# aleCombi/Hedgehog.jl

Measured on AMD Instinct MI355X. Metric: MC path-steps/sec (Heston Euler-Maruyama, 1e6 paths x 252 steps per GPU), higher is better.
Workload: dtype f64

## Files before the change

hedgehog.jl_amd/_ffi.py:

```python
from __future__ import annotations

import ctypes as C
import os

HH_MAX_PARTIALS = 8
HH_LSM_PHASE_POW, HH_LSM_PHASE_INIT, HH_LSM_PHASE_STEP = 1, 2, 3
HH_TILE_PATHS = 256
HH_ACC_LEN = 16
HH_MAX_MODELS = 16
HH_ACC_SUM, HH_ACC_SUMSQ, HH_ACC_DSUM, HH_ACC_NPATHS = 0, 1, 2, 10

HH_LOGNORMAL, HH_HESTON = 0, 1
HH_EULER_MARUYAMA, HH_EXACT_LAW, HH_BROADIE_KAYA = 0, 1, 2
HH_NOISE_GENERATE, HH_NOISE_REPLAY = 0, 1
HH_REPLAY_TILE_MAJOR, HH_REPLAY_PATH_MAJOR = 0, 1
HH_PATH_SPOT, HH_PATH_LOG = 0, 1
HH_PAYOFF_VANILLA, HH_PAYOFF_ASIAN_ARITH, HH_PAYOFF_ASIAN_GEOM = 0, 1, 2
HH_PAYOFF_BARRIER, HH_PAYOFF_DIGITAL_CASH, HH_PAYOFF_DIGITAL_ASSET = 3, 4, 5
HH_BARRIER_UP_OUT, HH_BARRIER_UP_IN, HH_BARRIER_DOWN_OUT, HH_BARRIER_DOWN_IN = 0, 1, 2, 3
HH_STAT_SUM_S, HH_STAT_SUM_X, HH_STAT_MAX_S, HH_STAT_MIN_S, HH_STAT_S_T = 0, 1, 2, 3, 4
HH_PAYOFF_LOOKBACK_FLOAT, HH_PAYOFF_LOOKBACK_FIXED = 6, 7
HH_STAT_CMAX_S, HH_STAT_CMIN_S = 5, 6
HH_EXTREMES_MONITORED, HH_EXTREMES_BRIDGE = 0, 1
HH_PATH_STATS = 5
HH_PATH_STATS_BRIDGE = 7
HH_MAX_PATH_PAYOFFS = 1024
HH_JUMP_MAX_MEAN = 64.0
HH_JUMP_MAX_COUNT = 255

HH_OK, HH_ERR_INVALID, HH_ERR_UNSUPPORTED, HH_ERR_HIP, HH_ERR_NOMEM, HH_ERR_RCCL, HH_ERR_DEVICE_TIMEOUT = 0, -1, -2, -3, -4, -5, -6
HH_MGPU_AUTO, HH_MGPU_HOST_SUM, HH_MGPU_RCCL = 0, 1, 2
HH_MGPU_REDUCE_HOST, HH_MGPU_REDUCE_RCCL = 0, 1
HH_MGPU_OPT_ENQUEUE = 1
HH_MGPU_ENQUEUE_SERIAL, HH_MGPU_ENQUEUE_THREADS = 0, 1

_dp = C.POINTER(C.c_double)


class hh_model(C.Structure):
    _fields_ = [(n, C.c_double) for n in
                ("S0", "V0", "kappa", "theta", "sigma", "rho", "r_drift", "discount", "T", "strike",
                 "cp")] + \
               [(n, _dp) for n in
                ("dS0", "dV0", "dkappa", "dtheta", "dsigma", "dr_drift", "ddiscount", "dstrike")]


class hh_config(C.Structure):
    _fields_ = [
        ("dynamics", C.c_int32), ("strategy", C.c_int32), ("antithetic", C.c_int32),
        ("em_split", C.c_int32), ("compat_sqrt_alpha", C.c_int32), ("noise_mode", C.c_int32),
        ("replay_layout", C.c_int32), ("seeds_on_device", C.c_int32),
        ("replay_on_device", C.c_int32), ("terminal_on_device", C.c_int32),
        ("n_steps", C.c_uint32), ("n_partials", C.c_uint32),
        ("n_paths", C.c_uint64), ("path_offset", C.c_uint64),
        ("seeds", C.c_void_p), ("replay", C.c_void_p),
        ("bk_n_sigma", C.c_double), ("bk_cf_tol", C.c_double), ("bk_atol", C.c_double),
        ("bk_moment_h", C.c_double),
        ("bk_newton_maxiter", C.c_int32), ("bk_bisect_maxiter", C.c_int32),
        ("bk_root_form", C.c_int32), ("bk_bracket_form", C.c_int32), ("bk_caps", C.c_int32), ("reserved0", C.c_int32),
        ("seeds_len", C.c_uint64), ("replay_len", C.c_uint64),
    ]


class hh_result(C.Structure):
    _fields_ = [
        ("price", C.c_double), ("std_error", C.c_double),
        ("sum_payoff", C.c_double), ("sumsq_payoff", C.c_double),
        ("dprice", C.c_double * HH_MAX_PARTIALS),
        ("n_paths_done", C.c_uint64),
        ("bk_newton_fail", C.c_uint64), ("bk_bisect_fallback", C.c_uint64),
        ("bk_maxguess_fallback", C.c_uint64), ("bk_cf_terms", C.c_uint64),
        ("kernel_ms", C.c_double), ("total_ms", C.c_double),
    ]


class hh_lsm_result(C.Structure):
    _fields_ = [("price", C.c_double), ("std_error", C.c_double), ("n_paths_total", C.c_uint64),
                ("rows_regressed", C.c_uint32), ("rows_skipped", C.c_uint32),
                ("kernel_ms", C.c_double), ("total_ms", C.c_double),
                ("form", C.c_int32), ("persistent_fallbacks", C.c_int32)]


class hh_path_payoff(C.Structure):
    _fields_ = [("kind", C.c_int32), ("barrier_type", C.c_int32), ("strike", C.c_double), ("cp", C.c_double),
                ("barrier", C.c_double), ("rebate", C.c_double), ("cash", C.c_double)]


class hh_jump(C.Structure):
    _fields_ = [("lambda_", C.c_double), ("mu_j", C.c_double), ("sigma_j", C.c_double)]


HH_BK_ROOT_SECANT, HH_BK_ROOT_ORDER2 = 0, 1
HH_BK_BRACKET_MIDPOINT, HH_BK_BRACKET_ROOTS = 0, 1
HH_BK_CAPS_AS_WRITTEN, HH_BK_CAPS_ROOTS_DEFAULT = 0, 1
HH_OPT_LSM_FORM = 1
HH_OPT_BK_TERM_CACHE = 2
HH_OPT_GRID_FORM = 3
HH_OPT_LSM_SPIN_TICKS = 4
HH_OPT_FUSE_REDUCE = 5
HH_OPT_GRID_ORDER = 6
HH_OPT_FINISH_SPIN_TICKS = 7
HH_OPT_FINISH_TILE_FIRST = 8
HH_GRID_FORM_PER_DATE, HH_GRID_FORM_BATCHED = 0, 1
HH_CM_GRAD_LEN = 8
HH_LSM_FORM_PER_DATE, HH_LSM_FORM_PERSISTENT, HH_LSM_FORM_AUTO = 0, 1, 2
HH_CRR_MAX_STEPS, HH_CRR_FORM_A_MAX_STEPS = 32768, 2047
HH_CRR_EUROPEAN, HH_CRR_AMERICAN_FORWARD, HH_CRR_AMERICAN_SPOT = 0, 1, 2
HH_FD_MAX_SPACE, HH_FD_MAX_TIME, HH_FD_FORM_A_MAX_SPACE = 4096, 65536, 1024
HH_FD_EUROPEAN, HH_FD_AMERICAN = 0, 1


class HedgehogMCError(RuntimeError):
    def __init__(self, code: int, msg: str):
        super().__init__(f"hedgehog_mc error {code}: {msg}")
        self.code = code


LIB_PATH = os.environ.get("HEDGEHOG_MC_LIB") or os.path.join(
    os.path.dirname(os.path.abspath(__file__)), "lib", "libhedgehog_mc.so")

_vp = C.c_void_p
SYMBOLS = [
    ("hh_abi_version", C.c_int, []),
    ("hh_ctx_create", C.c_int, [C.POINTER(_vp), C.c_int]),
    ("hh_ctx_destroy", None, [_vp]),
    ("hh_ctx_set_stream", C.c_int, [_vp, _vp]),
    ("hh_ctx_reset_stream", C.c_int, [_vp]),
    ("hh_last_error", C.c_char_p, [_vp]),
    ("hh_ctx_set_option", C.c_int, [_vp, C.c_int32, C.c_int64]),
    ("hh_ctx_check_last", C.c_int, [_vp]),
    ("hh_mc_solve", C.c_int, [_vp, C.POINTER(hh_model), C.POINTER(hh_config), C.POINTER(hh_result), _vp]),
    ("hh_mc_accumulate", C.c_int, [_vp, C.POINTER(hh_model), C.POINTER(hh_config), _vp, _vp]),
    ("hh_mc_solve_multi", C.c_int, [_vp, C.POINTER(hh_model), C.c_uint32, C.POINTER(hh_config), C.POINTER(hh_result), _vp]),
    ("hh_mc_accumulate_multi", C.c_int, [_vp, C.POINTER(hh_model), C.c_uint32, C.POINTER(hh_config), _vp, _vp]),
    ("hh_mc_finalize", C.c_int, [C.POINTER(hh_model), C.POINTER(hh_config), _vp, C.POINTER(hh_result)]),
    ("hh_mc_accumulate_basket", C.c_int, [_vp, C.POINTER(hh_model), C.POINTER(hh_config), _vp, _vp, C.c_uint32, _vp, _vp]),
    ("hh_mc_solve_basket", C.c_int, [_vp, C.POINTER(hh_model), C.POINTER(hh_config), _vp, _vp, C.c_uint32, _vp, _vp]),
    ("hh_carr_madan", C.c_int, [_vp, C.POINTER(hh_model), C.c_int32, C.c_int32, C.c_double, C.c_double, C.POINTER(C.c_double)]),
    ("hh_carr_madan_basket", C.c_int, [_vp, C.POINTER(hh_model), C.c_int32, C.c_int32, C.c_double, C.c_double,
                                       _vp, _vp, _vp, _vp, _vp, C.c_uint32, _vp]),
    ("hh_carr_madan_basket_grad", C.c_int, [_vp, C.POINTER(hh_model), C.c_int32, C.c_int32, C.c_double,
                                            C.c_double, _vp, _vp, _vp, _vp, _vp, C.c_uint32, _vp, _vp]),
    ("hh_crr_solve", C.c_int, [_vp, C.c_int32, C.c_uint32, _vp, _vp, _vp, _vp, _vp, _vp, _vp, C.c_uint32, _vp, _vp]),
    ("hh_fd_solve", C.c_int, [_vp, C.c_int32, C.c_int32, C.c_int32, C.c_uint32, _vp, _vp, _vp, _vp, _vp, _vp, _vp, _vp, _vp, _vp, _vp]),
    ("hh_lsm_grid_elems", C.c_size_t, [C.c_uint64, C.c_uint32, C.c_int32]),
    ("hh_lsm_solve", C.c_int, [_vp, C.POINTER(hh_model), C.POINTER(hh_config), C.c_int32, C.c_double, C.POINTER(hh_lsm_result), _vp, _vp, _vp]),
    ("hh_lsm_solve_grid", C.c_int, [_vp, C.POINTER(hh_model), _vp, C.c_uint64, C.c_uint32, C.c_int32, C.c_double, C.POINTER(hh_lsm_result), _vp, _vp]),
    ("hh_heston_exact_grid", C.c_int, [_vp, C.POINTER(hh_model), C.POINTER(hh_config), _vp, _vp, C.c_int32, C.POINTER(hh_result)]),
    ("hh_euler_grid", C.c_int, [_vp, C.POINTER(hh_model), C.POINTER(hh_config), C.c_int32, _vp, _vp, C.c_int32, C.POINTER(hh_result)]),
    ("hh_lsm_solve_euler", C.c_int, [_vp, C.POINTER(hh_model), C.POINTER(hh_config), C.c_int32, C.c_int32, C.c_double,
                                     C.POINTER(hh_lsm_result), _vp, _vp, _vp]),
    ("hh_mc_path_stats", C.c_int, [_vp, C.POINTER(hh_model), C.POINTER(hh_config), C.c_uint32, C.c_int32, _vp, C.c_int32,
                                   C.POINTER(hh_result)]),
    ("hh_mc_solve_path", C.c_int, [_vp, C.POINTER(hh_model), C.POINTER(hh_config), C.c_uint32, C.c_int32,
                                   C.POINTER(hh_path_payoff), C.c_uint32, C.POINTER(hh_result), _vp, _vp]),
    ("hh_mc_path_stats_ex", C.c_int, [_vp, C.POINTER(hh_model), C.POINTER(hh_config), C.c_uint32, C.c_int32, C.c_int32, _vp,
                                      C.c_int32, C.POINTER(hh_result)]),
    ("hh_mc_solve_path_ex", C.c_int, [_vp, C.POINTER(hh_model), C.POINTER(hh_config), C.c_uint32, C.c_int32, C.c_int32,
                                      C.POINTER(hh_path_payoff), C.c_uint32, C.POINTER(hh_result), _vp, _vp]),
    ("hh_mc_solve_jump", C.c_int, [_vp, C.POINTER(hh_model), C.POINTER(hh_jump), C.POINTER(hh_config), C.POINTER(hh_result),
                                   _vp]),
    ("hh_mc_solve_path_jump", C.c_int, [_vp, C.POINTER(hh_model), C.POINTER(hh_jump), C.POINTER(hh_config), C.c_uint32,
                                        C.c_int32, C.POINTER(hh_path_payoff), C.c_uint32, C.POINTER(hh_result), _vp, _vp]),
    ("hh_carr_madan_jump", C.c_int, [_vp, C.POINTER(hh_model), C.POINTER(hh_jump), C.c_double, C.c_double,
                                     _vp, _vp, _vp, _vp, _vp, C.c_uint32, _vp]),
    ("hh_lsm_shard_xchg_elems", C.c_size_t, [C.c_uint32, C.c_int32]),
    ("hh_lsm_shard_begin", C.c_int, [_vp, C.POINTER(hh_model), C.POINTER(hh_config), C.c_int32, C.c_double, _vp]),
    ("hh_lsm_shard_phase", C.c_int, [_vp, C.c_int32, C.c_uint32, _vp, _vp]),
    ("hh_lsm_shard_finish", C.c_int, [_vp, _vp, _vp, _vp, _vp, C.POINTER(C.c_uint32), C.POINTER(C.c_uint32)]),
    ("hh_lsm_finalize", C.c_int, [_vp, C.POINTER(hh_lsm_result)]),
    ("hh_lsm_debug_read", C.c_int, [_vp, C.c_uint64, C.c_uint32, C.c_int32, _vp]),
    ("hh_replay_elems", C.c_size_t, [C.c_uint64, C.c_uint32, C.c_int32]),
    ("hh_replay_pack", C.c_int, [_vp, C.c_int32, C.c_uint64, C.c_uint32, _vp, C.c_int32, _vp]),
    ("hh_wiener_fill", C.c_int, [_vp, C.c_int32, C.c_double, C.c_double, C.c_uint32, C.c_uint64, _vp, C.c_int32, _vp]),
    ("hh_seeds_fingerprint", C.c_uint64, [_vp, C.c_uint64]),
    ("hh_seeds_cache", C.c_int, [_vp, _vp, C.c_uint64, C.c_uint64, C.POINTER(_vp)]),
    ("hh_seeds_cache_stats", C.c_int, [_vp, C.POINTER(C.c_uint64), C.POINTER(C.c_uint64), C.POINTER(C.c_uint64)]),
    ("hh_device_malloc", C.c_int, [_vp, C.c_size_t, C.POINTER(_vp)]),
    ("hh_device_free", C.c_int, [_vp, _vp]),
    ("hh_memcpy_h2d", C.c_int, [_vp, _vp, _vp, C.c_size_t]),
    ("hh_memcpy_d2h", C.c_int, [_vp, _vp, _vp, C.c_size_t]),
    ("hh_ctx_synchronize", C.c_int, [_vp]),
    ("hh_ctx_enable_timing", C.c_int, [_vp, C.c_int32]),
    ("hh_ctx_read_timings", C.c_int, [_vp, _vp, C.c_int32, C.POINTER(C.c_int32)]),
    ("hh_bk_decisions", C.c_int, [_vp, C.c_uint64, _vp, _vp]),
# ... 347 lines not shown
```

hedgehog.jl_amd/csrc/hh_api.hip:

```cpp
#include <cmath>
#include <cstdarg>
#include <cstdio>
#include <cstring>
#include <mutex>
#include <vector>

#include "hh_kernels.h"

#include "hh_ctx.h"

namespace {

const char* const kNoCtx = "hedgehog_mc: no context";

int ncomp_of(int dynamics) { return dynamics == HH_HESTON ? 2 : 1; }

constexpr uint64_t kMaxPaths = (1ull << 32) - 256;
constexpr uint32_t kMaxEulerSteps = 4u * 65535u;
constexpr uint32_t kMaxGridSteps = 65534u;

static bool bk_law_ok(const hh_model* m, double dt) {
  const double s2 = m->sigma * m->sigma;
  const double d = 4.0 * m->kappa * m->theta / s2;
  if (!(d >= 1e-8 && d <= 1e6)) return false;
// ... 41 lines not shown
    if ((c->bk_root_form != HH_BK_ROOT_SECANT && c->bk_root_form != HH_BK_ROOT_ORDER2) ||
        (c->bk_bracket_form != HH_BK_BRACKET_MIDPOINT && c->bk_bracket_form != HH_BK_BRACKET_ROOTS) ||
        (c->bk_caps != HH_BK_CAPS_AS_WRITTEN && c->bk_caps != HH_BK_CAPS_ROOTS_DEFAULT))
      return fail(ctx, HH_ERR_INVALID, "bk_root_form, bk_bracket_form, bk_caps: 0 or 1 each (hedgehog_mc.h)");
    if (!bk_law_ok(m, m->T))
      return fail(ctx, HH_ERR_INVALID, "HestonBroadieKaya needs 1e-8 <= d = 4 kappa theta / sigma^2 <= 1e6 "
                                       "(Bessel order d/2 - 1 strictly above -1, tables up to order 5e5) and "
                                       "finite transition constants (|kappa T| < 700)");
  }
  const bool euler = c->strategy == HH_EULER_MARUYAMA;
  if (c->noise_mode == HH_NOISE_REPLAY) {
    if (!c->replay) return fail(ctx, HH_ERR_INVALID, "REPLAY needs a replay buffer");
    if (((uintptr_t)c->replay & 15u) != 0)
      return fail(ctx, HH_ERR_INVALID, "replay buffer must be 16-byte aligned");
    if (c->replay_len) {
      uint64_t need = c->n_paths;
      if (c->strategy == HH_BROADIE_KAYA) need = 3 * c->n_paths;
      if (euler)
        need = c->replay_layout == HH_REPLAY_PATH_MAJOR
                   ? c->n_paths * (uint64_t)c->n_steps * (uint64_t)ncomp_of(c->dynamics)
                   : (uint64_t)hh::tiles_for(c->n_paths) * c->n_steps * ncomp_of(c->dynamics) *
                         hh::kTile;
      if (c->replay_len < need)
        return fail(ctx, HH_ERR_INVALID, "replay buffer holds %llu elements, %llu needed",
                    (unsigned long long)c->replay_len, (unsigned long long)need);
    }
  } else if (c->noise_mode == HH_NOISE_GENERATE) {
    if (!c->seeds) return fail(ctx, HH_ERR_INVALID, "GENERATE needs seeds");
    const uint64_t need = euler ? c->n_paths : 1;
    if (c->seeds_len && c->seeds_len < need)
      return fail(ctx, HH_ERR_INVALID, "Number of seeds (%llu) must be >= number of trajectories (%llu)",
                  (unsigned long long)c->seeds_len, (unsigned long long)need);
  } else {
    return fail(ctx, HH_ERR_INVALID, "unknown noise_mode %d", c->noise_mode);
  }
  return HH_OK;
}

int ensure_poisoned(hh_ctx* ctx, size_t need) {
  if (need <= ctx->frecords.cap) return HH_OK;
  int rc = ensure(ctx, ctx->frecords, need);
  if (rc) return rc;
  static_assert((hh::kPoison >> 32) == (hh::kPoison & 0xffffffffull), "hipMemsetD32 writes the pattern");
  HH_HIP(ctx, hipMemsetD32Async((hipDeviceptr_t)ctx->frecords, (int)(hh::kPoison & 0xffffffffull),
                                ctx->frecords.cap * 2, ctx->stream));
  return HH_OK;
}

constexpr uint32_t kFuseAutoMaxRecords = 512, kFuseAutoMinSteps = 32;
bool fuse_for(const hh_ctx* ctx, const hh_config* c) {
  if (ctx->fuse_reduce != 2) return ctx->fuse_reduce == 1;
  return hh::sim_records(*c) <= kFuseAutoMaxRecords || (c->strategy == HH_EULER_MARUYAMA && c->n_steps >= kFuseAutoMinSteps);
}

void fused_controls(const hh_ctx* ctx, hh::DevicePtrs& p) {
  p.finish_state = ctx->finish_state;
  p.finish_spin_ticks = ctx->finish_spin_ticks;
  p.finish_tile_first = ctx->finish_tile_first;
}

int recover_finish(hh_ctx* ctx) {
  unsigned int state = 0;
  HH_HIP(ctx, hipStreamSynchronize(ctx->stream));
  HH_HIP(ctx, hipMemcpy(&state, ctx->finish_state, sizeof(state), hipMemcpyDeviceToHost));
  if (state == 0u) return HH_OK;
  if (ctx->frecords.cap)
    HH_HIP(ctx, hipMemsetD32Async((hipDeviceptr_t)ctx->frecords, (int)(hh::kPoison & 0xffffffffull),
                                  ctx->frecords.cap * 2, ctx->stream));
  HH_HIP(ctx, hipMemsetAsync(ctx->finish_state, 0, 2 * sizeof(unsigned int), ctx->stream));
  HH_HIP(ctx, hipStreamSynchronize(ctx->stream));
  const long long ticks = ctx->finish_spin_ticks < 0 ? (long long)hh::kFinishSpinTicksDefault : ctx->finish_spin_ticks;
  return fail(ctx, HH_ERR_DEVICE_TIMEOUT,
              "the record reduction inside a simulation kernel gave up: a workgroup's record had not arrived after %lld "
              "ticks of the 100 MHz clock (a queue preempted for that long, or a workgroup that died); the sums of that "
              "solve, and of solves queued behind it, are lost — the context's record buffer has been reset and the "
              "context can be used again", ticks);
}

int finalize_failed(hh_ctx* ctx, int rc) {
  const int rf = recover_finish(ctx);
  return rf ? rf : fail(ctx, rc, "finalize failed: the accumulator holds no trajectories");
}

size_t replay_elems(uint64_t n_paths, uint32_t n_steps, int dynamics) {
  return (size_t)hh::tiles_for(n_paths) * n_steps * ncomp_of(dynamics) * hh::kTile;
}

int solve_times(hh_ctx* ctx, const WallClock& clock, double* kernel_ms, double* total_ms) {
  float ms = 0.f;
  HH_HIP(ctx, hipEventElapsedTime(&ms, ctx->ev0, ctx->ev1));
  *kernel_ms = ms;
  *total_ms = clock.ms();
  return HH_OK;
}

void payoff_moments(const double* acc, double n, double* mean, double* var) {
  *mean = acc[HH_ACC_SUM] / n;
  *var = n > 1.0 ? (acc[HH_ACC_SUMSQ] - n * *mean * *mean) / (n - 1.0) : 0.0;
  if (!(*var > 0.0)) *var = 0.0;
}

}

extern "C" {

int hh_abi_version(void) { return HH_ABI_VERSION; }

int hh_ctx_create(hh_ctx** out, int device_id) {
  if (!out) return HH_ERR_INVALID;
  *out = nullptr;
  int n = 0;
  if (hipGetDeviceCount(&n) != hipSuccess || n <= 0) return HH_ERR_HIP;
  if (device_id < 0 || device_id >= n) return HH_ERR_INVALID;
  hh_ctx* ctx = new (std::nothrow) hh_ctx();
  if (!ctx) return HH_ERR_NOMEM;
  ctx->device = device_id;
  if (hipSetDevice(device_id) != hipSuccess ||
      hipStreamCreateWithFlags(&ctx->own_stream, hipStreamNonBlocking) != hipSuccess ||
      hipEventCreate(&ctx->ev0) != hipSuccess || hipEventCreate(&ctx->ev1) != hipSuccess ||
      hipEventCreateWithFlags(&ctx->ev_switch, hipEventDisableTiming) != hipSuccess ||
      hipEventCreateWithFlags(&ctx->ev_stage, hipEventDisableTiming) != hipSuccess ||
      hipMalloc((void**)&ctx->accum, HH_ACC_LEN * sizeof(double)) != hipSuccess ||
      hipMalloc((void**)&ctx->finish_state, 2 * sizeof(unsigned int)) != hipSuccess ||
      hipMemset(ctx->finish_state, 0, 2 * sizeof(unsigned int)) != hipSuccess ||
      hipHostMalloc((void**)&ctx->accum_host, (HH_ACC_LEN + 8) * sizeof(double), hipHostMallocDefault) !=
          hipSuccess) {
    hh_ctx_destroy(ctx);
    return HH_ERR_HIP;
  }
  ctx->stream = ctx->own_stream;
  *out = ctx;
  return HH_OK;
}

void hh_ctx_destroy(hh_ctx* ctx) {
  if (!ctx) return;
  (void)hipSetDevice(ctx->device);
  if (ctx->own_stream) (void)hipStreamSynchronize(ctx->own_stream);
  (void)hipDeviceSynchronize();
  for (auto& e : ctx->seed_cache)
    if (e.dev) (void)hipFree(e.dev);
  if (ctx->accum) (void)hipFree(ctx->accum);
  if (ctx->finish_state) (void)hipFree(ctx->finish_state);
  if (ctx->accum_host) (void)hipHostFree(ctx->accum_host);
  for (auto& pr : ctx->tev)
    for (auto& e : pr)
      if (e) (void)hipEventDestroy(e);
  if (ctx->ev_switch) (void)hipEventDestroy(ctx->ev_switch);
  if (ctx->ev_stage) (void)hipEventDestroy(ctx->ev_stage);
  if (ctx->ev0) (void)hipEventDestroy(ctx->ev0);
  if (ctx->ev1) (void)hipEventDestroy(ctx->ev1);
  if (ctx->own_stream) (void)hipStreamDestroy(ctx->own_stream);
  delete ctx;
}

static int switch_stream(hh_ctx* ctx, hipStream_t next) {
  if (next == ctx->stream) return HH_OK;
  HH_HIP(ctx, hipSetDevice(ctx->device));
  HH_HIP(ctx, hipEventRecord(ctx->ev_switch, ctx->stream));
  HH_HIP(ctx, hipStreamWaitEvent(next, ctx->ev_switch, 0));
  ctx->stream = next;
  return HH_OK;
}

int hh_ctx_set_stream(hh_ctx* ctx, void* hip_stream) {
  if (!ctx) return HH_ERR_INVALID;
  std::lock_guard<std::recursive_mutex> lock__(ctx->mu);
  return switch_stream(ctx, (hipStream_t)hip_stream);
}

int hh_ctx_reset_stream(hh_ctx* ctx) {
  if (!ctx) return HH_ERR_INVALID;
  std::lock_guard<std::recursive_mutex> lock__(ctx->mu);
  return switch_stream(ctx, ctx->own_stream);
}

const char* hh_last_error(const hh_ctx* ctx) { return ctx ? ctx->err : kNoCtx; }

int hh_ctx_set_option(hh_ctx* ctx, int32_t option, int64_t value) {
  if (!ctx) return HH_ERR_INVALID;
  std::lock_guard<std::recursive_mutex> lock__(ctx->mu);
  switch (option) {
    case HH_OPT_LSM_FORM:
      if (value != HH_LSM_FORM_PER_DATE && value != HH_LSM_FORM_PERSISTENT && value != HH_LSM_FORM_AUTO)
        return fail(ctx, HH_ERR_INVALID, "HH_OPT_LSM_FORM: 0 (launch per date), 1 (one launch) or 2 (auto)");
      ctx->lsm_form = (int)value;
      return HH_OK;
    case HH_OPT_BK_TERM_CACHE:
      if (value < 8 || value > 1024)
        return fail(ctx, HH_ERR_INVALID, "HH_OPT_BK_TERM_CACHE: 8 .. 1024 series terms per trajectory");
      ctx->bk_term_cache = (int)value;
      return HH_OK;
    case HH_OPT_LSM_SPIN_TICKS:
      if (value < -1) return fail(ctx, HH_ERR_INVALID, "HH_OPT_LSM_SPIN_TICKS: ticks of the 100 MHz clock, 0 = give up at once, -1 = default");
      ctx->lsm_spin_ticks = value;
      return HH_OK;
    case HH_OPT_GRID_FORM:
      if (value != HH_GRID_FORM_PER_DATE && value != HH_GRID_FORM_BATCHED)
        return fail(ctx, HH_ERR_INVALID, "HH_OPT_GRID_FORM: 0 (one chain per date) or 1 (dates batched)");
      ctx->grid_form = (int)value;
      return HH_OK;
    case HH_OPT_GRID_ORDER:
      if (value != 0 && value != 1)
        return fail(ctx, HH_ERR_INVALID, "HH_OPT_GRID_ORDER: 0 (a chain's pairs in their natural order) or 1 (sorted by their Bessel arguments)");
      ctx->grid_order = (int)value;
      return HH_OK;
    case HH_OPT_FINISH_SPIN_TICKS:
      if (value < -1) return fail(ctx, HH_ERR_INVALID, "HH_OPT_FINISH_SPIN_TICKS: ticks of the 100 MHz clock, 0 = give up at once, -1 = default");
      ctx->finish_spin_ticks = value;
      return HH_OK;
    case HH_OPT_FINISH_TILE_FIRST:
      if (value != 0 && value != 1) return fail(ctx, HH_ERR_INVALID, "HH_OPT_FINISH_TILE_FIRST: 0 (the last tile's workgroup adds the records) or 1 (the first one's)");
      ctx->finish_tile_first = (int)value;
      return HH_OK;
    case HH_OPT_FUSE_REDUCE:
      if (value < 0 || value > 2)
        return fail(ctx, HH_ERR_INVALID, "HH_OPT_FUSE_REDUCE: 0 (a second kernel reduces the records), 1 (the simulation kernel does) or 2 (by size)");
      ctx->fuse_reduce = (int)value;
      return HH_OK;
    default:
      return fail(ctx, HH_ERR_INVALID, "unknown option %d", option);
  }
}

int hh_ctx_synchronize(hh_ctx* ctx) {
  if (!ctx) return HH_ERR_INVALID;
  std::lock_guard<std::recursive_mutex> lock__(ctx->mu);
  HH_HIP(ctx, hipSetDevice(ctx->device));
  HH_HIP(ctx, hipStreamSynchronize(ctx->stream));
  return HH_OK;
}

size_t hh_replay_elems(uint64_t n_paths, uint32_t n_steps, int32_t dynamics) {
  return replay_elems(n_paths, n_steps, dynamics);
}

int hh_replay_pack(hh_ctx* ctx, int32_t dynamics, uint64_t n_paths, uint32_t n_steps,
                   const double* src, int32_t src_on_device, double* dst) {
  if (!ctx) return HH_ERR_INVALID;
  std::lock_guard<std::recursive_mutex> lock__(ctx->mu);
  if (!src || !dst || n_paths == 0 || n_steps == 0 || n_paths > kMaxPaths || n_steps > kMaxEulerSteps)
    return fail(ctx, HH_ERR_INVALID, "hh_replay_pack: bad arguments");
  HH_HIP(ctx, hipSetDevice(ctx->device));
  const int nc = ncomp_of(dynamics);
  const double* src_dev = src;
  if (!src_on_device) {
    const size_t n = (size_t)n_paths * n_steps * nc;
    const int rc = stage_host(ctx, ctx->replay_src, n, src, n, &src_dev);
    if (rc) return rc;
  }
  HH_HIP(ctx, hh::launch_replay_pack(nc, n_paths, n_steps, src_dev, dst, ctx->stream));
  return release_host_operands(ctx);
}

int hh_wiener_fill(hh_ctx* ctx, int32_t dynamics, double rho, double T, uint32_t n_steps,
                   uint64_t n_paths, const uint64_t* seeds, int32_t seeds_on_device, double* dst) {
  if (!ctx) return HH_ERR_INVALID;
  std::lock_guard<std::recursive_mutex> lock__(ctx->mu);
  if (!seeds || !dst || n_paths == 0 || n_steps == 0 || !(T > 0.0) || !(std::fabs(rho) <= 1.0) ||
      n_paths > kMaxPaths || n_steps > kMaxEulerSteps)
    return fail(ctx, HH_ERR_INVALID, "hh_wiener_fill: bad arguments");
  HH_HIP(ctx, hipSetDevice(ctx->device));
  const uint64_t* seeds_dev = seeds;
  if (!seeds_on_device) {
    const int rc = stage_host(ctx, ctx->seeds, (size_t)n_paths, seeds, (size_t)n_paths, &seeds_dev);
    if (rc) return rc;
  }
  const double dt = T / (double)n_steps;
  HH_HIP(ctx, hh::launch_wiener_fill(dynamics, rho, std::sqrt(dt), n_steps, n_paths, seeds_dev, dst,
                                     ctx->stream));
  return release_host_operands(ctx);
}

static int stage_noise(hh_ctx* ctx, const hh_config* c, hh::DevicePtrs& p, bool tile_major_only) {
  int rc = HH_OK;
  const bool bk = c->strategy == HH_BROADIE_KAYA;
  if (c->noise_mode == HH_NOISE_GENERATE) {
    const size_t need = (c->strategy == HH_EULER_MARUYAMA) ? (size_t)c->n_paths : 1;
    if (c->seeds_on_device)
      p.seeds = c->seeds;
    else if ((rc = stage_host(ctx, ctx->seeds, need, c->seeds, need, &p.seeds)))
      return rc;
  } else if (bk) {
    const size_t n3 = (size_t)3 * c->n_paths;
    if (c->replay_on_device)
      p.replay = c->replay;
    else if ((rc = stage_host(ctx, ctx->replay, n3, c->replay, n3, &p.replay)))
      return rc;
  } else {
    const uint32_t steps = (c->strategy == HH_EULER_MARUYAMA) ? c->n_steps : 1;
    const int dyn = (c->strategy == HH_EULER_MARUYAMA) ? c->dynamics : HH_LOGNORMAL;
    const size_t tile_elems = replay_elems(c->n_paths, steps, dyn);
    if (c->replay_layout == HH_REPLAY_PATH_MAJOR && c->strategy == HH_EULER_MARUYAMA && !tile_major_only &&
        hh::replay_direct_path_major(steps, ncomp_of(dyn))) {
      const size_t n = (size_t)c->n_paths * steps * ncomp_of(dyn);
      if (c->replay_on_device)
        p.replay = c->replay;
      else if ((rc = stage_host(ctx, ctx->replay_src, n, c->replay, n, &p.replay)))
        return rc;
      p.replay_path_major = true;
    } else if (c->replay_layout == HH_REPLAY_PATH_MAJOR) {
      rc = ensure(ctx, ctx->replay, tile_elems);
      if (rc) return rc;
      rc = hh_replay_pack(ctx, dyn, c->n_paths, steps, c->replay, c->replay_on_device, ctx->replay);
      if (rc) return rc;
      p.replay = ctx->replay;
    } else if (c->replay_layout == HH_REPLAY_TILE_MAJOR) {
      if (c->replay_on_device) {
        p.replay = c->replay;
      } else {
        const size_t host_elems =
            (c->strategy == HH_EULER_MARUYAMA) ? tile_elems : (size_t)c->n_paths;
        rc = stage_host(ctx, ctx->replay, tile_elems, c->replay, host_elems, &p.replay);
        if (rc) return rc;
      }
    } else {
      return fail(ctx, HH_ERR_INVALID, "unknown replay_layout %d", c->replay_layout);
    }
  }

  return HH_OK;
}

static int run_simulation(hh_ctx* ctx, const hh_model* m, const hh_config* c, double* terminal,
                          bool need_terminal_dev, double** terminal_dev_out, double* accum_dev = nullptr,
                          bool* reduced = nullptr) {
  int rc = HH_OK;
  const uint32_t n_tiles = hh::tiles_for(c->n_paths);
  const bool bk = c->strategy == HH_BROADIE_KAYA;
  rc = ensure(ctx, ctx->records, (size_t)(bk ? hh::bk_record_count(c->n_paths) : n_tiles) * hh::kRecStride);
  if (rc) return rc;

  hh::DevicePtrs p{};
  p.records = ctx->records;
  const bool fuse = accum_dev && !bk && fuse_for(ctx, c);
  if (fuse) {
    if ((rc = ensure_poisoned(ctx, (size_t)n_tiles * hh::kRecStride))) return rc;
    p.records = ctx->frecords;
    p.accum = accum_dev;
    fused_controls(ctx, p);
  }
  if (reduced) *reduced = fuse || bk;
  if (bk) {
    rc = ensure_bk_scratch(ctx, hh::bk_scratch_bytes(c->n_paths, ctx->bk_term_cache));
    if (rc) return rc;
    p.accum = accum_dev ? accum_dev : ctx->accum;
    p.bk_scratch = ctx->bk_scratch;
    p.bk_table_key = &ctx->bk_table_key;
    p.bk_term_cache = ctx->bk_term_cache;
    ctx->bk_last_n = c->n_paths;
    ctx->bk_last_cache = ctx->bk_term_cache;
  }

  if ((rc = stage_noise(ctx, c, p, false))) return rc;

  const size_t n_term = (size_t)c->n_paths * (c->antithetic ? 2 : 1);
  if (terminal && c->terminal_on_device) {
    p.terminal = terminal;
  } else if (terminal || need_terminal_dev) {
    rc = ensure(ctx, ctx->terminal, n_term);
    if (rc) return rc;
    p.terminal = ctx->terminal;
  }
  const int n_active = c->n_partials ? hh::count_active_partials(*m, *c) : 0;
  if (need_terminal_dev && n_active) {
    rc = ensure(ctx, ctx->terminal_d, n_term * (size_t)hh::pad_partials((uint32_t)n_active));
    if (rc) return rc;
    p.terminal_d = ctx->terminal_d;
  }
  if (terminal_dev_out) *terminal_dev_out = p.terminal;

  if (ctx->timing) HH_HIP(ctx, hipEventRecord(ctx->tev[ctx->t_count % hh_ctx::kTimingSlots][0], ctx->stream));
  if (c->strategy == HH_BROADIE_KAYA)
    HH_HIP(ctx, hh::launch_bk(*m, *c, p, ctx->stream));
  else
    HH_HIP(ctx, hh::launch_simulation(*m, *c, p, ctx->stream));
  return HH_OK;
}

static int end_timing(hh_ctx* ctx) {
  if (ctx->timing) {
    HH_HIP(ctx, hipEventRecord(ctx->tev[ctx->t_count % hh_ctx::kTimingSlots][1], ctx->stream));
    ++ctx->t_count;
  }
  return HH_OK;
}

static int copy_back_terminal(hh_ctx* ctx, const hh_config* c, double* terminal) {
  if (terminal && !c->terminal_on_device) {
    const size_t n_term = (size_t)c->n_paths * (c->antithetic ? 2 : 1);
    HH_HIP(ctx, hipMemcpyAsync(terminal, ctx->terminal, n_term * sizeof(double),
                               hipMemcpyDeviceToHost, ctx->stream));
    HH_HIP(ctx, hipStreamSynchronize(ctx->stream));
  }
  return HH_OK;
}

int hh_mc_accumulate(hh_ctx* ctx, const hh_model* m, const hh_config* c, double* accum_dev,
                     double* terminal) {
  if (!ctx) return HH_ERR_INVALID;
  std::lock_guard<std::recursive_mutex> lock__(ctx->mu);
  int rc = validate(ctx, m, c);
  if (rc) return rc;
  if (!accum_dev) return fail(ctx, HH_ERR_INVALID, "accum_dev is NULL");
  HH_HIP(ctx, hipSetDevice(ctx->device));
  bool reduced = false;
  rc = run_simulation(ctx, m, c, terminal, false, nullptr, accum_dev, &reduced);
  if (rc) return rc;
  if (!reduced)
    HH_HIP(ctx, hh::launch_reduce_records(ctx->records, hh::sim_records(*c), (double)c->n_paths, accum_dev, ctx->stream, 1, m, c));
  if ((rc = end_timing(ctx))) return rc;
  if ((rc = release_host_operands(ctx))) return rc;
  return copy_back_terminal(ctx, c, terminal);
}

static int next_pass(int remaining) {
  if (remaining <= hh::kMaxModelsPerPass) return remaining;
  return remaining == hh::kMaxModelsPerPass + 1 ? hh::kMaxModelsPerPass - 1 : hh::kMaxModelsPerPass;
}

int hh_mc_accumulate_multi(hh_ctx* ctx, const hh_model* models, uint32_t n_models, const hh_config* c,
                           double* accum_dev, double* const* terminals) {
  if (!ctx) return HH_ERR_INVALID;
  std::lock_guard<std::recursive_mutex> lock__(ctx->mu);
  if (!models || n_models == 0 || n_models > HH_MAX_MODELS)
    return fail(ctx, HH_ERR_INVALID, "hh_mc_accumulate_multi: 1 .. %d models", HH_MAX_MODELS);
  if (!accum_dev) return fail(ctx, HH_ERR_INVALID, "accum_dev is NULL");
  int rc;
  for (uint32_t k = 0; k < n_models; ++k)
    if ((rc = validate(ctx, &models[k], c))) return rc;
  if (c->n_partials)
    return fail(ctx, HH_ERR_UNSUPPORTED, "several models in one pass carry no dual partials (n_partials must be 0)");
  if (n_models == 1) return hh_mc_accumulate(ctx, models, c, accum_dev, terminals ? terminals[0] : nullptr);
  HH_HIP(ctx, hipSetDevice(ctx->device));
  if (c->strategy == HH_BROADIE_KAYA) {
    const uint32_t count = hh::bk_record_count(c->n_paths);
    if ((rc = ensure(ctx, ctx->records, 2 * (size_t)count * hh::kRecStride))) return rc;
    std::vector<int> leader(n_models, -1);
    for (uint32_t k = 0; k < n_models; ++k)
      for (uint32_t j = 0; j < k; ++j)
        if (leader[j] < 0 && hh::bk_same_chain(models[j], models[k])) {
          leader[k] = (int)j;
          break;
        }
    for (uint32_t k = 0; k < n_models; ++k) {
      if (leader[k] >= 0) continue;
      if ((rc = hh_mc_accumulate(ctx, &models[k], c, accum_dev + (size_t)k * HH_ACC_LEN, terminals ? terminals[k] : nullptr)))
        return rc;
      for (uint32_t f = k + 1; f < n_models; ++f) {
        if (leader[f] != (int)k) continue;
        double* terminal = terminals ? terminals[f] : nullptr;
        hh::DevicePtrs p{};
        p.records = ctx->records + (size_t)count * hh::kRecStride;
        p.bk_scratch = ctx->bk_scratch;
        p.bk_term_cache = ctx->bk_term_cache;
        if (terminal && c->terminal_on_device) {
          p.terminal = terminal;
        } else if (terminal) {
          if ((rc = ensure(ctx, ctx->terminal, (size_t)c->n_paths))) return rc;
          p.terminal = ctx->terminal;
        }
        if (ctx->timing) HH_HIP(ctx, hipEventRecord(ctx->tev[ctx->t_count % hh_ctx::kTimingSlots][0], ctx->stream));
        HH_HIP(ctx, hh::launch_bk_refinish(models[f], *c, p, ctx->records, ctx->stream));
        HH_HIP(ctx, hh::launch_reduce_records(p.records, count, (double)c->n_paths, accum_dev + (size_t)f * HH_ACC_LEN,
                                              ctx->stream, 1, &models[f], c, false,
                                              hh::bk_live_records(ctx->bk_scratch, c->n_paths)));
        if ((rc = end_timing(ctx))) return rc;
        if ((rc = copy_back_terminal(ctx, c, terminal))) return rc;
      }
    }
    return HH_OK;
  }
  const uint32_t n_tiles = hh::tiles_for(c->n_paths);
  const size_t rec_elems = (size_t)n_tiles * hh::kRecStride;
  const bool fuse = fuse_for(ctx, c);
  if (fuse) rc = ensure_poisoned(ctx, (size_t)n_models * rec_elems);
  else rc = ensure(ctx, ctx->records, (size_t)n_models * rec_elems);
  if (rc) return rc;
  hh::DevicePtrs base{};
  if (fuse) fused_controls(ctx, base);
  if ((rc = stage_noise(ctx, c, base, true))) return rc;
  const size_t n_term = (size_t)c->n_paths * (c->antithetic ? 2 : 1);
  bool any_host_terminal = false;
  if (terminals && !c->terminal_on_device) {
    for (uint32_t k = 0; k < n_models; ++k) any_host_terminal = any_host_terminal || terminals[k] != nullptr;
    if (any_host_terminal && (rc = ensure(ctx, ctx->terminal, (size_t)n_models * n_term))) return rc;
  }
  std::vector<hh::DevicePtrs> p(n_models, base);
  for (uint32_t k = 0; k < n_models; ++k) {
    p[k].records = (fuse ? ctx->frecords : ctx->records) + (size_t)k * rec_elems;
    p[k].accum = fuse ? accum_dev + (size_t)k * HH_ACC_LEN : nullptr;
    double* t = terminals ? terminals[k] : nullptr;
    p[k].terminal = !t ? nullptr : c->terminal_on_device ? t : ctx->terminal + (size_t)k * n_term;
  }
  if (ctx->timing) HH_HIP(ctx, hipEventRecord(ctx->tev[ctx->t_count % hh_ctx::kTimingSlots][0], ctx->stream));
  for (uint32_t k0 = 0; k0 < n_models;) {
    const int take = next_pass((int)(n_models - k0));
    HH_HIP(ctx, hh::launch_simulation_multi(models + k0, take, *c, p.data() + k0, ctx->stream));
    if (!fuse)
      for (int k = 0; k < take; ++k)
        HH_HIP(ctx, hh::launch_reduce_records(p[k0 + k].records, hh::sim_records(*c), (double)c->n_paths,
                                              accum_dev + (size_t)(k0 + k) * HH_ACC_LEN, ctx->stream, 1, &models[k0 + k], c));
    k0 += (uint32_t)take;
  }
  if ((rc = end_timing(ctx))) return rc;
  if ((rc = release_host_operands(ctx))) return rc;
  if (any_host_terminal) {
    for (uint32_t k = 0; k < n_models; ++k)
      if (terminals[k])
        HH_HIP(ctx, hipMemcpyAsync(terminals[k], p[k].terminal, n_term * sizeof(double), hipMemcpyDeviceToHost, ctx->stream));
    HH_HIP(ctx, hipStreamSynchronize(ctx->stream));
  }
  return HH_OK;
}

int hh_mc_solve_multi(hh_ctx* ctx, const hh_model* models, uint32_t n_models, const hh_config* c, hh_result* out,
                      double* const* terminals) {
  if (!ctx) return HH_ERR_INVALID;
  std::lock_guard<std::recursive_mutex> lock__(ctx->mu);
  if (!out || !models || n_models == 0 || n_models > HH_MAX_MODELS)
    return fail(ctx, HH_ERR_INVALID, "hh_mc_solve_multi: 1 .. %d models and their results", HH_MAX_MODELS);
  const WallClock clock;
  HH_HIP(ctx, hipSetDevice(ctx->device));
  const size_t n_acc = (size_t)n_models * HH_ACC_LEN;
  int rc = ensure(ctx, ctx->basket_accum, n_acc);
  if (rc) return rc;
  HH_HIP(ctx, hipEventRecord(ctx->ev0, ctx->stream));
  if ((rc = hh_mc_accumulate_multi(ctx, models, n_models, c, ctx->basket_accum, terminals))) return rc;
  HH_HIP(ctx, hipEventRecord(ctx->ev1, ctx->stream));
  double host[HH_MAX_MODELS * HH_ACC_LEN];
  HH_HIP(ctx, hipMemcpyAsync(host, ctx->basket_accum, n_acc * sizeof(double), hipMemcpyDeviceToHost, ctx->stream));
  HH_HIP(ctx, hipStreamSynchronize(ctx->stream));
  double kernel_ms, total_ms;
  if ((rc = solve_times(ctx, clock, &kernel_ms, &total_ms))) return rc;
  rc = finalize_results(models, 1, c, host, n_models, kernel_ms, total_ms, out);
  return rc ? finalize_failed(ctx, rc) : HH_OK;
}

int hh_mc_accumulate_basket(hh_ctx* ctx, const hh_model* m, const hh_config* c,
                            const double* strikes, const double* cps, uint32_t n_payoffs,
                            double* accum_dev, double* terminal) {
  if (!ctx) return HH_ERR_INVALID;
  std::lock_guard<std::recursive_mutex> lock__(ctx->mu);
  int rc = validate(ctx, m, c);
  if (rc) return rc;
  if (!accum_dev || !strikes || !cps || n_payoffs == 0 || n_payoffs > 65535)
    return fail(ctx, HH_ERR_INVALID, "hh_mc_accumulate_basket: bad arguments");
  for (uint32_t k = 0; k < n_payoffs; ++k)
    if (cps[k] != 1.0 && cps[k] != -1.0) return fail(ctx, HH_ERR_INVALID, "cp must be +1 or -1");
  if (m->dstrike)
    return fail(ctx, HH_ERR_UNSUPPORTED, "strike partials are not carried through a basket");
  HH_HIP(ctx, hipSetDevice(ctx->device));
  double* term_dev = nullptr;
  rc = run_simulation(ctx, m, c, terminal, true, &term_dev);
  if (rc) return rc;

  hh::BasketArgs b{};
  b.n_paths = c->n_paths;
  b.n_chunks = hh::basket_chunks(c->n_paths);
  b.antithetic = c->antithetic;
  std::vector<double> payoffs(strikes, strikes + n_payoffs);
  payoffs.insert(payoffs.end(), cps, cps + n_payoffs);
  const double* payoffs_dev = nullptr;
  rc = stage_host(ctx, ctx->payoffs, payoffs.size(), payoffs.data(), payoffs.size(), &payoffs_dev);
  if (rc) return rc;
  rc = ensure(ctx, ctx->basket_records, (size_t)n_payoffs * b.n_chunks * hh::kRecStride);
  if (rc) return rc;
  b.terminal = term_dev;
  const int n_active = c->n_partials ? hh::count_active_partials(*m, *c) : 0;
  b.terminal_d = n_active ? ctx->terminal_d : nullptr;
  b.strikes = payoffs_dev;
  b.cps = payoffs_dev + n_payoffs;
  b.records = ctx->basket_records;
  HH_HIP(ctx, hh::launch_basket_payoffs(b, n_payoffs, (uint32_t)n_active, ctx->stream));
  HH_HIP(ctx, hh::launch_reduce_records(ctx->basket_records, b.n_chunks, (double)c->n_paths,
                                        accum_dev, ctx->stream, n_payoffs, m, c, true));
  if (c->strategy == HH_BROADIE_KAYA)
    HH_HIP(ctx, hh::launch_copy_bk_counters(ctx->accum, accum_dev, n_payoffs, ctx->stream));
  if ((rc = end_timing(ctx))) return rc;
  if ((rc = release_host_operands(ctx))) return rc;
  return copy_back_terminal(ctx, c, terminal);
}

int hh_mc_solve_basket(hh_ctx* ctx, const hh_model* m, const hh_config* c, const double* strikes,
                       const double* cps, uint32_t n_payoffs, hh_result* out, double* terminal) {
  if (!ctx) return HH_ERR_INVALID;
  std::lock_guard<std::recursive_mutex> lock__(ctx->mu);
  if (!out) return fail(ctx, HH_ERR_INVALID, "result is NULL");
  const WallClock clock;
  HH_HIP(ctx, hipSetDevice(ctx->device));
  const size_t n_acc = (size_t)n_payoffs * HH_ACC_LEN;
  int rc = ensure(ctx, ctx->basket_accum, n_acc);
  if (rc) return rc;
  HH_HIP(ctx, hipEventRecord(ctx->ev0, ctx->stream));
  rc = hh_mc_accumulate_basket(ctx, m, c, strikes, cps, n_payoffs, ctx->basket_accum, terminal);
  if (rc) return rc;
  HH_HIP(ctx, hipEventRecord(ctx->ev1, ctx->stream));
  std::vector<double> host(n_acc);
  HH_HIP(ctx, hipMemcpyAsync(host.data(), ctx->basket_accum, n_acc * sizeof(double),
                             hipMemcpyDeviceToHost, ctx->stream));
  HH_HIP(ctx, hipStreamSynchronize(ctx->stream));
  double kernel_ms, total_ms;
  if ((rc = solve_times(ctx, clock, &kernel_ms, &total_ms))) return rc;
  rc = finalize_results(m, 0, c, host.data(), n_payoffs, kernel_ms, total_ms, out);
  return rc ? finalize_failed(ctx, rc) : HH_OK;
}

int hh_mc_finalize(const hh_model* m, const hh_config* c, const double* acc, hh_result* out) {
  if (!m || !c || !acc || !out) return HH_ERR_INVALID;
  const double n = acc[HH_ACC_NPATHS];
  if (!(n >= 1.0)) return HH_ERR_INVALID;
  double mean, var;
  payoff_moments(acc, n, &mean, &var);
  out->sum_payoff = acc[HH_ACC_SUM];
  out->sumsq_payoff = acc[HH_ACC_SUMSQ];
  out->price = m->discount * mean;
  out->std_error = m->discount * std::sqrt(var / n);
  for (uint32_t k = 0; k < HH_MAX_PARTIALS; ++k) {
    double d = 0.0;
    if (k < c->n_partials) {
      const double dD = m->ddiscount ? m->ddiscount[k] : 0.0;
      d = dD * mean + m->discount * (acc[HH_ACC_DSUM + k] / n);
    }
    out->dprice[k] = d;
  }
  out->n_paths_done = (uint64_t)n;
  out->bk_newton_fail = (uint64_t)acc[HH_ACC_BK_NEWTON_FAIL];
  out->bk_bisect_fallback = (uint64_t)acc[HH_ACC_BK_BISECT];
  out->bk_maxguess_fallback = (uint64_t)acc[HH_ACC_BK_MAXGUESS];
  out->bk_cf_terms = (uint64_t)acc[HH_ACC_BK_CF_TERMS];
  return HH_OK;
}

int hh_mc_solve(hh_ctx* ctx, const hh_model* m, const hh_config* c, hh_result* out,
                double* terminal) {
  if (!ctx) return HH_ERR_INVALID;
  std::lock_guard<std::recursive_mutex> lock__(ctx->mu);
  if (!out) return fail(ctx, HH_ERR_INVALID, "result is NULL");
  const WallClock clock;
  std::memset(out, 0, sizeof(*out));
  HH_HIP(ctx, hipSetDevice(ctx->device));
  HH_HIP(ctx, hipEventRecord(ctx->ev0, ctx->stream));
  int rc = hh_mc_accumulate(ctx, m, c, ctx->accum, terminal);
  if (rc) return rc;
  HH_HIP(ctx, hipEventRecord(ctx->ev1, ctx->stream));
  HH_HIP(ctx, hipMemcpyAsync(ctx->accum_host, ctx->accum, HH_ACC_LEN * sizeof(double),
                             hipMemcpyDeviceToHost, ctx->stream));
  HH_HIP(ctx, hipStreamSynchronize(ctx->stream));
  rc = hh_mc_finalize(m, c, ctx->accum_host, out);
  if (rc) return finalize_failed(ctx, rc);
  return solve_times(ctx, clock, &out->kernel_ms, &out->total_ms);
}

int hh_ctx_check_last(hh_ctx* ctx) {
  if (!ctx) return HH_ERR_INVALID;
  std::lock_guard<std::recursive_mutex> lock__(ctx->mu);
  HH_HIP(ctx, hipSetDevice(ctx->device));
  return recover_finish(ctx);
}

int hh_bk_decisions(hh_ctx* ctx, uint64_t n_paths, uint32_t* decisions, uint32_t* series_len) {
  if (!ctx) return HH_ERR_INVALID;
  std::lock_guard<std::recursive_mutex> lock__(ctx->mu);
  if (!ctx->bk_scratch || ctx->bk_last_n == 0 || n_paths != ctx->bk_last_n)
    return fail(ctx, HH_ERR_INVALID, "hh_bk_decisions: the last Broadie-Kaya solve of this context had %llu trajectories",
                (unsigned long long)ctx->bk_last_n);
  HH_HIP(ctx, hipSetDevice(ctx->device));
  const uint32_t *dec = nullptr, *len = nullptr;
  hh::bk_diag_ptrs(ctx->bk_scratch, n_paths, ctx->bk_last_cache, &dec, &len);
  if (decisions)
    HH_HIP(ctx, hipMemcpyAsync(decisions, dec, n_paths * sizeof(uint32_t), hipMemcpyDeviceToHost, ctx->stream));
  if (series_len)
    HH_HIP(ctx, hipMemcpyAsync(series_len, len, n_paths * sizeof(uint32_t), hipMemcpyDeviceToHost, ctx->stream));
  HH_HIP(ctx, hipStreamSynchronize(ctx->stream));
  return HH_OK;
}

#define HH_CM_BOUND_MSG "%s: bound/alpha must be <= 196608 (1024 sub-panels of half-width 0.75 alpha per lane)"
static_assert(hh::kCarrMadanMaxSubpanels * 192 == 196608, "HH_CM_BOUND_MSG names the limit");

int hh_carr_madan(hh_ctx* ctx, const hh_model* m, int32_t dynamics, int32_t compat_sqrt_alpha,
                  double alpha, double bound, double* price_out) {
  if (!ctx) return HH_ERR_INVALID;
  std::lock_guard<std::recursive_mutex> lock__(ctx->mu);
  if (!m || !price_out) return fail(ctx, HH_ERR_INVALID, "hh_carr_madan: NULL argument");
  if (dynamics != HH_LOGNORMAL && dynamics != HH_HESTON)
    return fail(ctx, HH_ERR_INVALID, "unknown dynamics %d", dynamics);
  if (!(m->S0 > 0.0) || !(m->strike > 0.0) || !(m->T > 0.0) || !(alpha > 0.0) || !(bound > 0.0) ||
      (m->cp != 1.0 && m->cp != -1.0) || (dynamics == HH_HESTON && m->sigma == 0.0))
    return fail(ctx, HH_ERR_INVALID, "hh_carr_madan: bad scalars");
  if (!hh::carr_madan_subpanels(alpha, bound)) return fail(ctx, HH_ERR_INVALID, HH_CM_BOUND_MSG, "hh_carr_madan");
  HH_HIP(ctx, hipSetDevice(ctx->device));
  HH_HIP(ctx, hh::launch_carr_madan(*m, dynamics, compat_sqrt_alpha, alpha, bound, ctx->accum,
                                    ctx->stream));
  HH_HIP(ctx, hipMemcpyAsync(ctx->accum_host, ctx->accum, sizeof(double), hipMemcpyDeviceToHost,
                             ctx->stream));
  HH_HIP(ctx, hipStreamSynchronize(ctx->stream));
  const double call = ctx->accum_host[0];
  *price_out = m->cp > 0.0 ? call : call - m->S0 + m->strike * m->discount;
  return HH_OK;
}

static int cm_upload_payoffs(hh_ctx* ctx, const char* who, const double* strikes, const double* cps, const double* Ts,
                             const double* r_drifts, const double* discounts, size_t n, size_t out_len,
                             std::vector<double>& host) {
  for (size_t k = 0; k < n; ++k) {
    if (!(strikes[k] > 0.0) || !(Ts[k] > 0.0) || (cps[k] != 1.0 && cps[k] != -1.0) ||
        !std::isfinite(r_drifts[k]) || !(discounts[k] > 0.0))
      return fail(ctx, HH_ERR_INVALID, "%s: payoff %zu: strike, T, discount > 0, cp = +-1", who, k);
    host[k] = std::log(strikes[k]);
    host[n + k] = Ts[k];
    host[2 * n + k] = r_drifts[k];
    host[3 * n + k] = discounts[k];
  }
  HH_HIP(ctx, hipSetDevice(ctx->device));
  int rc = ensure(ctx, ctx->payoffs, 4 * n + out_len);
  if (rc) return rc;
  HH_HIP(ctx, hipMemcpyAsync(ctx->payoffs, host.data(), 4 * n * sizeof(double), hipMemcpyHostToDevice,
                             ctx->stream));
  return HH_OK;
}

int hh_carr_madan_basket(hh_ctx* ctx, const hh_model* m, int32_t dynamics, int32_t compat_sqrt_alpha,
                         double alpha, double bound, const double* strikes, const double* cps,
                         const double* Ts, const double* r_drifts, const double* discounts,
                         uint32_t n_payoffs, double* prices_out) {
  if (!ctx) return HH_ERR_INVALID;
  std::lock_guard<std::recursive_mutex> lock__(ctx->mu);
  if (!m || !strikes || !cps || !Ts || !r_drifts || !discounts || !prices_out)
    return fail(ctx, HH_ERR_INVALID, "hh_carr_madan_basket: NULL argument");
  if (dynamics != HH_LOGNORMAL && dynamics != HH_HESTON)
    return fail(ctx, HH_ERR_INVALID, "unknown dynamics %d", dynamics);
  if (n_payoffs == 0 || n_payoffs > (1u << 20))
    return fail(ctx, HH_ERR_INVALID, "hh_carr_madan_basket: 1 .. 2^20 payoffs per call");
// ... 885 lines not shown
```

hedgehog.jl_amd/csrc/hh_bk.hip:

```cpp
#include <algorithm>
#include <atomic>
#include <cmath>

#include "hh_bessel.h"
#include "hh_kernels.h"
#include "hh_math.h"
#include "hh_reduce.h"
#include "hh_rng.h"

namespace hh {

namespace {

constexpr double kPi = kBesselPi;
constexpr double kTwoPi = kBesselTwoPi, kInvTwoPi = 0.15915494309189533577;
constexpr double kInvPi = 0.31830988618379067154, kTwoOverPi = 0.63661977236758134308;

#ifndef HH_BK_COMPLEX_SETUP
#define HH_BK_COMPLEX_SETUP 0
#endif
#ifndef HH_BK_SERIAL_LADDER
#define HH_BK_SERIAL_LADDER 0
#endif

// ... 971 lines not shown
    if (stage == kLadderLo) {
      fa = f;
      x = xb;
      stage = kLadderHi;
      continue;
    }
    if (stage == kLadderHi) {
      fb = f;
      if (fa * fb > 0.0) {
        acc[4] += 1.0;
        dec |= kDecMaxGuess;
        break;
      }
      acc[3] += 1.0;
      dec |= kDecBisect;
      x = roots_bisect ? roots_middle(xa, xb) : 0.5 * (xa + xb);
      if (cap_bisect <= 0 || (roots_bisect && !(xa < x && x < xb))) break;
      stage = kBisect;
      continue;
    }
    ++iters;
    bool stop;
    if (roots_bisect) {
      if (f == 0.0) {
        out_set = true;
      } else if (sign_of(fa) * sign_of(f) < 0) {
        xb = x;
        fb = f;
      } else {
        xa = x;
        fa = f;
      }
      const double mid = roots_middle(xa, xb);
      stop = out_set || (int)iters >= cap_bisect || !(xa < mid && mid < xb);
      if (!out_set) x = stop ? mid : mid;
    } else {
      if (f == 0.0) {
        xa = xb = x;
      } else if ((f < 0.0) == (fa < 0.0)) {
        xa = x;
        fa = f;
      } else {
        xb = x;
      }
      x = 0.5 * (xa + xb);
      stop = f == 0.0 || xb - xa <= p.atol || (int)iters >= cap_bisect;
    }
    if (stop) {
      dec |= (iters & 0xffu) << kDecItersShift;
      break;
    }
  }
  if (roots_bisect && (dec & kDecBisect) && !out_set) x = fabs(fa) < fabs(fb) ? xa : xb;
  const double IV = x;
  p.diag[path] = dec;
  p.diag[p.draw_stride + path] = (uint32_t)s.cache.j_stop;
  acc[5] += n_terms;
  const double pay = bk_finish_path(p, path, IV);
  acc[0] += pay;
  acc[1] = fma(pay, pay, acc[1]);
}

template <class Fn>
__device__ __forceinline__ void for_long_tiles(const unsigned long long* __restrict__ long_mask, uint32_t n_tiles,
                                               uint32_t b, Fn&& fn) {
  __shared__ unsigned char hit[kTile];
  for (uint32_t t0 = b; t0 < n_tiles; t0 += (uint32_t)kHeavyGrid * kTile) {
    const uint32_t t = t0 + threadIdx.x * (uint32_t)kHeavyGrid;
    unsigned long long any = 0ull;
    if (t < n_tiles) {
#pragma unroll
      for (int w = 0; w < kTile / 64; ++w) any |= long_mask[(size_t)t * (kTile / 64) + w];
    }
    __syncthreads();
    hit[threadIdx.x] = any != 0ull;
    __syncthreads();
    for (uint32_t i = 0; i < (uint32_t)kTile; ++i)
      if (hit[i]) fn(t0 + i * (uint32_t)kHeavyGrid);
  }
}

__global__ __launch_bounds__(kTile) void bk_tail_kernel(const BkArgs* __restrict__ args, const BkTables* __restrict__ tabs,
                                                        uint32_t n_tiles, double n_paths, double* __restrict__ accum,
                                                        uint32_t* __restrict__ cnt, const double* __restrict__ records) {
  const uint32_t b = blockIdx.x, tid = threadIdx.x;
  __shared__ double sm[257];
  const uint32_t n_long_v = __hip_atomic_load(cnt, __ATOMIC_RELAXED, __HIP_MEMORY_SCOPE_AGENT);
  double out = 0.0;
  if (b < (uint32_t)kRecStride) out = sum_slot(records, n_tiles, (int)b, sm);
  const uint32_t n_long = (uint32_t)__builtin_amdgcn_readfirstlane((int)n_long_v);
  uint32_t n_rec = n_tiles;
  if (n_long != 0u) {
    const BkArgs& p = *args;
    double acc[6] = {0, 0, 0, 0, 0, 0};
    for_long_tiles(p.long_mask, n_tiles, b, [&](uint32_t tile) {
      const uint64_t path = (uint64_t)tile * kTile + tid;
      if ((p.long_mask[(size_t)tile * (kTile / 64) + (tid >> 6)] >> (tid & 63u)) & 1ull)
        tail_whole_trajectory(p, tabs->t, tabs->coef, path, acc);
    });
    bk_store_record(acc, p.records + (size_t)(n_tiles + b) * kRecStride);
    __syncthreads();
    if (tid == 0) {
      __builtin_amdgcn_fence(__ATOMIC_RELEASE, "agent");
      asm volatile("s_waitcnt vmcnt(0)" ::: "memory");
      __hip_atomic_fetch_add(cnt + 2, 1u, __ATOMIC_RELAXED, __HIP_MEMORY_SCOPE_AGENT);
    }
    if (b >= (uint32_t)kRecStride) return;
    if (tid == 0) {
      while (__hip_atomic_load(cnt + 2, __ATOMIC_RELAXED, __HIP_MEMORY_SCOPE_AGENT) != (uint32_t)kHeavyGrid)
        __builtin_amdgcn_s_sleep(8);
      __builtin_amdgcn_fence(__ATOMIC_ACQUIRE, "agent");
      asm volatile("s_waitcnt vmcnt(0)" ::: "memory");
      if (__hip_atomic_fetch_add(cnt + 3, 1u, __ATOMIC_RELAXED, __HIP_MEMORY_SCOPE_AGENT) == (uint32_t)kRecStride - 1u) {
        __hip_atomic_store(cnt, 0u, __ATOMIC_RELAXED, __HIP_MEMORY_SCOPE_AGENT);
        __hip_atomic_store(cnt + 2, 0u, __ATOMIC_RELAXED, __HIP_MEMORY_SCOPE_AGENT);
        __hip_atomic_store(cnt + 3, 0u, __ATOMIC_RELAXED, __HIP_MEMORY_SCOPE_AGENT);
      }
    }
    __syncthreads();
    n_rec = n_tiles + (uint32_t)kHeavyGrid;
    out = sum_slot(records, n_rec, (int)b, sm);
  } else if (b >= (uint32_t)kRecStride) {
    return;
  }
  if (tid == 0) {
    accum[b] = b == (uint32_t)HH_ACC_NPATHS ? n_paths : out;
    if (b == 0u) cnt[1] = n_rec;
  }
}

__global__ __launch_bounds__(kTile) void bk_refinish_kernel(const BkArgs p, const double* __restrict__ rec0, uint32_t n_tiles) {
  const uint32_t b = blockIdx.x, tid = threadIdx.x;
  if (b >= p.counters[1]) return;
  double acc[6] = {0, 0, 0, 0, 0, 0};
  if (b < n_tiles) {
    const uint64_t path = (uint64_t)b * kTile + tid;
    const bool left = (p.long_mask[(size_t)b * (kTile / 64) + (tid >> 6)] >> (tid & 63u)) & 1ull;
    if (path < p.n_paths && !left) {
      const double pay = bk_finish_path(p, path, p.iv_keep[path]);
      acc[0] = pay;
      acc[1] = pay * pay;
    }
  } else {
    for_long_tiles(p.long_mask, n_tiles, b - n_tiles, [&](uint32_t tile) {
      const uint64_t path = (uint64_t)tile * kTile + tid;
      if ((p.long_mask[(size_t)tile * (kTile / 64) + (tid >> 6)] >> (tid & 63u)) & 1ull) {
        const double pay = bk_finish_path(p, path, p.iv_keep[path]);
        acc[0] += pay;
        acc[1] = fma(pay, pay, acc[1]);
      }
    });
  }
  double* rec = p.records + (size_t)b * kRecStride;
  bk_store_record(acc, rec);
  if (tid == 0) {
    const double* r0 = rec0 + (size_t)b * kRecStride;
    rec[HH_ACC_BK_NEWTON_FAIL] = r0[HH_ACC_BK_NEWTON_FAIL];
    rec[HH_ACC_BK_BISECT] = r0[HH_ACC_BK_BISECT];
    rec[HH_ACC_BK_MAXGUESS] = r0[HH_ACC_BK_MAXGUESS];
    rec[HH_ACC_BK_CF_TERMS] = r0[HH_ACC_BK_CF_TERMS];
  }
}

__global__ __launch_bounds__(64) void bk_tables_kernel(const BkBessel t, BkTables* __restrict__ dst, double kappa,
                                                        double sigma2, double T, double eta_k, double zeta_k) {
  for (int j = (int)threadIdx.x; j <= kCoefTerms; j += 64) dst->coef[j] = kTwoOverPi / (double)j;
  if (threadIdx.x != 0) return;
  dst->zero = chf_zero(kappa, sigma2, T, eta_k, zeta_k);
  const double* src = reinterpret_cast<const double*>(&t);
  double* out = reinterpret_cast<double*>(dst->t);
  static_assert(sizeof(BkBessel) == sizeof(dst->t), "the Bessel tables of BkTables");
#pragma unroll
  for (size_t i = 0; i < sizeof(BkBessel) / sizeof(double); ++i) out[i] = src[i];
}

__global__ __launch_bounds__(256) void fill_rows_kernel(double* __restrict__ spot0,
                                                        double* __restrict__ var0, uint64_t n,
                                                        double S0, double V0) {
  const uint64_t i = (uint64_t)blockIdx.x * 256 + threadIdx.x;
  if (i < n) {
    spot0[i] = S0;
    var0[i] = V0;
  }
}

constexpr int kSortWaves = kTile / 64;
static_assert(kSortRun % 64 == 0, "whole rounds of a wave");

__global__ __launch_bounds__(kTile) void grid_sort_count_kernel(const uint8_t* __restrict__ keys, uint32_t n, uint32_t n_runs,
                                                                uint32_t* __restrict__ counts) {
  __shared__ uint32_t hist[kSortWaves][256];
  const uint32_t wave = threadIdx.x >> 6, lane = threadIdx.x & 63u, run = blockIdx.x * kSortWaves + wave;
  for (uint32_t d = lane; d < 256u; d += 64u) hist[wave][d] = 0u;
  __syncthreads();
  if (run < n_runs) {
    const uint32_t base = run * (uint32_t)kSortRun;
    constexpr int kRounds = kSortRun / 64;
    uint32_t key[kRounds];
#pragma unroll
    for (int r = 0; r < kRounds; ++r) {
      const uint32_t i = base + (uint32_t)r * 64u + lane;
      key[r] = i < n ? (uint32_t)keys[i] : 256u;
    }
#pragma unroll
    for (int r = 0; r < kRounds; ++r)
      if (key[r] < 256u) atomicAdd(&hist[wave][key[r]], 1u);
  }
  __syncthreads();
  if (run < n_runs)
// ... 123 lines not shown
  a.kappa = m.kappa; a.theta = m.theta; a.sigma = m.sigma; a.sigma2 = m.sigma * m.sigma; a.inv_sigma2 = 1.0 / a.sigma2;
  a.rho = m.rho; a.V0 = m.V0; a.T = m.T; a.logS0 = log(m.S0); a.r = m.r_drift;
  a.strike = m.strike; a.cp = m.cp;
  const double em1 = -expm1(-m.kappa * m.T);
  a.d = 4.0 * m.kappa * m.theta / a.sigma2;
  a.lam_num = 4.0 * m.kappa * exp(-m.kappa * m.T);
  a.lam_den = a.sigma2 * em1;
  a.cscale = a.sigma2 * em1 / (4.0 * m.kappa);
  a.nu = 0.5 * a.d - 1.0;
  a.zeta_k = em1 / m.kappa;
  a.eta_k = m.kappa * (1.0 + exp(-m.kappa * m.T)) / em1;
  a.nuk_factor = 4.0 * m.kappa * exp(-0.5 * m.kappa * m.T) / a.sigma2 / em1;
  if (!(a.d > 0.0) || !std::isfinite(a.d) || !(a.lam_num * m.V0 / a.lam_den >= 0.0))
    return (int)hipErrorInvalidValue;
  a.n_int = a.nu >= 1.0 ? (int)floor(a.nu) : 0;
  a.n_sigma = c.bk_n_sigma > 0.0 ? c.bk_n_sigma : 5.0;
  a.cf_tol = c.bk_cf_tol > 0.0 ? c.bk_cf_tol : 1e-3;
  a.atol = c.bk_atol > 0.0 ? c.bk_atol : 1e-4;
  a.moment_h = c.bk_moment_h > 0.0 ? c.bk_moment_h : 1e-2;
  a.newton_maxiter = c.bk_newton_maxiter > 0 ? c.bk_newton_maxiter : 10;
  a.bisect_maxiter = c.bk_bisect_maxiter > 0 ? c.bk_bisect_maxiter : 100;
  a.root_form = c.bk_root_form;
  a.bracket_form = c.bk_bracket_form;
  a.caps = c.bk_caps;
  a.n_paths = n_chain;
  a.path_offset = c.path_offset;
  a.seeds = ptr.seeds;
  a.terminal = ptr.terminal;
  a.records = ptr.records;
  const BkScratch at = bk_scratch_at(n_chain, ptr.bk_term_cache);
  unsigned char* base = reinterpret_cast<unsigned char*>(ptr.bk_scratch);
  a.long_mask = reinterpret_cast<unsigned long long*>(base + at.long_mask);
  L.n_tiles = at.n_tiles;
  a.slot_busy = reinterpret_cast<uint32_t*>(base + at.slot_lines);
  a.counters = reinterpret_cast<uint32_t*>(base + at.counters);
  a.args_dev = base + at.args;
  L.tabs_dev = reinterpret_cast<BkTables*>(base + at.tables);
  a.tabs_dev = L.tabs_dev;
  a.n_tiles = at.n_tiles;
  a.cache_cap = at.cache_cap;
  a.phi_cache = reinterpret_cast<double*>(base + at.phi_cache);
  a.cache_stride = at.cache_columns;
  a.static_slots = at.n_tiles <= (uint32_t)kSlots ? 1u : 0u;
  a.draws = reinterpret_cast<double*>(base + at.draws);
  a.iv_store = reinterpret_cast<double*>(base + at.iv);
  a.diag = reinterpret_cast<uint32_t*>(base + at.diag);
  a.draw_stride = at.lanes;
  return 0;
}

int bk_tables(const BkArgs& a, const BkLayout& L, const DevicePtrs& ptr, hipStream_t s, bool upload_tables) {
  if (ptr.bk_table_key)
    upload_tables = !(ptr.bk_table_key->where == L.tabs_dev && ptr.bk_table_key->nu == a.nu &&
                      ptr.bk_table_key->kappa == a.kappa && ptr.bk_table_key->sigma2 == a.sigma2 &&
                      ptr.bk_table_key->T == a.T);
  if (upload_tables) {
    (void)hipMemsetAsync(a.slot_busy, 0, bk_scratch_at(a.n_paths, 0).zeroed_bytes, s);
    BkBessel tabs;
    if (!bessel_table(a.nu, tabs.t[0]) || !bessel_table(a.nu - a.n_int, tabs.t[1]))
      return (int)hipErrorInvalidValue;
    hipLaunchKernelGGL(bk_tables_kernel, dim3(1), dim3(64), 0, s, tabs, L.tabs_dev, a.kappa, a.sigma2, a.T, a.eta_k,
                       a.zeta_k);
    if (ptr.bk_table_key) *ptr.bk_table_key = BkTableKey{L.tabs_dev, a.nu, a.kappa, a.sigma2, a.T};
  }
  return 0;
}

uint32_t cf_resident_workgroups() {
  static std::atomic<uint32_t> cache[64];
  int dev = 0;
  if (hipGetDevice(&dev) != hipSuccess || dev < 0 || dev >= 64) return 0u;
  uint32_t v = cache[dev].load(std::memory_order_relaxed);
  if (v == 0u) {
    int cus = 0, per_cu = 0;
    if (hipDeviceGetAttribute(&cus, hipDeviceAttributeMultiprocessorCount, dev) != hipSuccess ||
        hipOccupancyMaxActiveBlocksPerMultiprocessor(&per_cu, bk_cf_kernel<0, 1>, kTile, 0) != hipSuccess || cus <= 0 || per_cu <= 0)
      return 0u;
    v = (uint32_t)cus * (uint32_t)per_cu;
    cache[dev].store(v, std::memory_order_relaxed);
  }
  return v;
}

void bk_chain(const BkArgs& a0, const BkLayout& L, hipStream_t s, double* accum, double n_acc, int draw = 0) {
  BkArgs a = a0;
  const uint32_t resident = cf_resident_workgroups();
  a.drain_tile = resident != 0u && L.n_tiles > resident ? L.n_tiles - resident : 0xffffffffu;
  const dim3 b(kTile), g(L.n_tiles);
  const BkTables* tabs = static_cast<const BkTables*>(L.tabs_dev);
  if (a.order)
    hipLaunchKernelGGL(bk_cf_kernel<1>, g, b, 0, s, a, tabs);
  else if (draw == 1)
    hipLaunchKernelGGL((bk_cf_kernel<0, 1>), g, b, 0, s, a, tabs);
  else if (draw == 2)
    hipLaunchKernelGGL((bk_cf_kernel<0, 2>), g, b, 0, s, a, tabs);
  else
    hipLaunchKernelGGL(bk_cf_kernel<0>, g, b, 0, s, a, tabs);
  hipLaunchKernelGGL(bk_tail_kernel, dim3(kHeavyGrid), b, 0, s, static_cast<const BkArgs*>(a.args_dev), tabs, L.n_tiles,
                     n_acc, accum, a.counters, static_cast<const double*>(a.records));
}

}

int launch_bk(const hh_model& m, const hh_config& c, const DevicePtrs& ptr, hipStream_t s,
              const BkTransition* tr, bool upload_tables) {
  if (!ptr.accum) return (int)hipErrorInvalidValue;
  BkArgs a{};
  BkLayout L{};
  if (tr) {
    a.in_spot = tr->in_spot; a.in_var = tr->in_var;
    a.out_spot = tr->out_spot; a.out_var = tr->out_var;
    a.step = tr->step;
  }
  int rc = bk_prepare(m, c, ptr, c.n_paths, a, L);
  if (rc) return rc;
  a.replay = c.noise_mode == HH_NOISE_REPLAY ? ptr.replay : nullptr;
  if (!tr) a.iv_keep = a.iv_store;
  if ((rc = bk_tables(a, L, ptr, s, upload_tables))) return rc;
  int draw = a.replay ? 2 : 1;
  if (a.in_var) {
    if (a.replay) return (int)hipErrorInvalidValue;
    hipLaunchKernelGGL(bk_draw_kernel, dim3(L.n_tiles), dim3(kTile), 0, s, a);
    draw = 0;
  }
  bk_chain(a, L, s, ptr.accum, (double)c.n_paths, draw);
  return (int)hipGetLastError();
}

bool bk_same_chain(const hh_model& a, const hh_model& b) {
  return a.kappa == b.kappa && a.theta == b.theta && a.sigma == b.sigma && a.V0 == b.V0 && a.T == b.T;
}

int launch_bk_refinish(const hh_model& m, const hh_config& c, const DevicePtrs& ptr, const double* rec0, hipStream_t s) {
  BkArgs a{};
  BkLayout L{};
  const int rc = bk_prepare(m, c, ptr, c.n_paths, a, L);
  if (rc) return rc;
  a.iv_keep = a.iv_store;
  hipLaunchKernelGGL(bk_refinish_kernel, dim3(L.n_tiles + (uint32_t)kHeavyGrid), dim3(kTile), 0, s, a, rec0, L.n_tiles);
  return (int)hipGetLastError();
}

uint32_t bk_grid_dates_per_chain(uint64_t n_paths, uint32_t n_steps) {
  const uint64_t pairs_max = (uint64_t)1 << 22;
  const uint64_t per = n_paths ? pairs_max / n_paths : 1;
  if (per <= 1) return 1;
  const uint64_t chains = (n_steps + per - 1) / per;
  return (uint32_t)((n_steps + chains - 1) / chains);
}

void bk_diag_ptrs(const void* scratch, uint64_t n_paths, int term_cache, const uint32_t** decisions,
                  const uint32_t** series_len) {
  const BkScratch at = bk_scratch_at(n_paths, term_cache);
  const uint32_t* diag = reinterpret_cast<const uint32_t*>(static_cast<const unsigned char*>(scratch) + at.diag);
  *decisions = diag;
  *series_len = diag + at.lanes;
}

size_t bk_grid_sort_bytes(uint64_t n_chain) { return BkSortScratch(n_chain).total; }

int launch_bk_grid(const hh_model& m, const hh_config& c, const DevicePtrs& ptr, hipStream_t s,
                   double* spot_rows, double* var_rows, uint32_t k0, uint32_t n_dates, bool upload_tables) {
  if (!ptr.accum) return (int)hipErrorInvalidValue;
  BkArgs a{};
  BkLayout L{};
  const uint64_t n_row = c.n_paths, n_chain = n_row * n_dates;
  int rc = bk_prepare(m, c, ptr, n_chain, a, L);
  if (rc) return rc;
  a.in_var = var_rows;
  a.step = k0;
  a.iv_out = a.iv_store;
  if ((rc = bk_tables(a, L, ptr, s, upload_tables))) return rc;
  const dim3 rows(tiles_for(n_row)), b(kTile);
  const bool ordered = ptr.bk_sort && n_chain >= kGridOrderMinPairs && n_chain < (1ull << 31);
  const BkSortScratch sort(n_chain);
  unsigned char* sort_base = static_cast<unsigned char*>(ptr.bk_sort);
  uint32_t* perm = reinterpret_cast<uint32_t*>(sort_base + sort.perm);
  uint32_t* counts = reinterpret_cast<uint32_t*>(sort_base + sort.counts);
  uint32_t* totals = reinterpret_cast<uint32_t*>(sort_base + sort.totals);
  uint8_t* keys = sort_base + sort.keys;
  hipLaunchKernelGGL(bk_draw_grid_kernel, rows, b, 0, s, a, n_row, k0, n_dates, var_rows, ordered ? keys : nullptr);
  if (ordered) {
    const dim3 sort_grid((sort.n_runs + kSortWaves - 1) / kSortWaves);
    hipLaunchKernelGGL(grid_sort_count_kernel, sort_grid, b, 0, s, static_cast<const uint8_t*>(keys), (uint32_t)n_chain,
                       sort.n_runs, counts);
    hipLaunchKernelGGL(grid_sort_scan_kernel, dim3(256), b, 0, s, counts, sort.n_runs, totals);
    hipLaunchKernelGGL(grid_sort_scatter_kernel, sort_grid, b, 0, s, static_cast<const uint8_t*>(keys), (uint32_t)n_chain,
                       sort.n_runs, static_cast<const uint32_t*>(counts), static_cast<const uint32_t*>(totals), perm);
    BkArgs o = a;
    o.order = perm;
    bk_chain(o, L, s, ptr.accum, (double)n_chain);
  } else {
    bk_chain(a, L, s, ptr.accum, (double)n_chain);
  }
  hipLaunchKernelGGL(bk_grid_spots_kernel, rows, b, 0, s, a, n_row, n_dates,
                     static_cast<const double*>(var_rows), spot_rows);
  return (int)hipGetLastError();
}

}
```

hedgehog.jl_amd/csrc/hh_ctx.h:

```cpp
#pragma once
#include <chrono>
#include <cstdarg>
#include <cstdio>
#include <cstring>
#include <mutex>

#include "hh_kernels.h"

template <class T>
struct DevBuf {
  T* p = nullptr;
  size_t cap = 0;
  DevBuf() = default;
  DevBuf(const DevBuf&) = delete;
  DevBuf& operator=(const DevBuf&) = delete;
  ~DevBuf() { if (p) (void)hipFree(p); }
  operator T*() const { return p; }
};

struct hh_ctx {
  int device = 0;
  hipStream_t own_stream = nullptr;
  hipStream_t stream = nullptr;
  hipEvent_t ev0 = nullptr, ev1 = nullptr, ev_switch = nullptr;
  hipEvent_t ev_stage = nullptr;
  bool staged_host = false;
  DevBuf<double> records;
  DevBuf<uint64_t> seeds;
  DevBuf<double> replay;
  DevBuf<double> replay_src;
  DevBuf<double> terminal;
  DevBuf<double> terminal_d;
  DevBuf<double> payoffs;
  DevBuf<double> basket_records;
  DevBuf<double> basket_accum;
  DevBuf<unsigned char> bk_scratch;
  hh::BkTableKey bk_table_key{};
  DevBuf<double> lsm_grid;
  DevBuf<double> heston_var;
  DevBuf<double> path_stats;
  DevBuf<double> path_values;
  DevBuf<hh_path_payoff> path_payoffs;
  DevBuf<double> lsm_val;
  DevBuf<int32_t> lsm_tau;
  DevBuf<double> lsm_scratch;
  struct {
    bool active = false;
    hh_model m{};
    uint64_t ntot = 0;
    uint32_t n_steps = 0;
    int32_t degree = 0;
    double step_discount = 1.0;
  } shard;
  int lsm_form = hh::kLsmFormAuto;
  int bk_term_cache = 0;
  uint64_t bk_last_n = 0;
  int bk_last_cache = 0;
  int grid_form = HH_GRID_FORM_BATCHED;
  int grid_order = 1;
  DevBuf<unsigned char> bk_sort;
  uint64_t lsm_persistent_fallbacks = 0;
  long long lsm_spin_ticks = -1;
  DevBuf<double> frecords;
  int fuse_reduce = 2;
  unsigned int* finish_state = nullptr;
  long long finish_spin_ticks = -1;
  int finish_tile_first = 0;
  struct SeedEntry {
    uint64_t* dev = nullptr;
    uint64_t n = 0, fingerprint = 0, head = 0, tail = 0, stamp = 0;
  };
  static constexpr int kSeedEntries = HH_SEED_CACHE_ENTRIES;
  SeedEntry seed_cache[kSeedEntries];
  uint64_t seed_clock = 0, seed_hits = 0, seed_uploads = 0, seed_evictions = 0;
  double* accum = nullptr;
  double* accum_host = nullptr;
  static constexpr int kTimingSlots = 256;
  bool timing = false;
  hipEvent_t tev[kTimingSlots][2] = {};
  int t_count = 0;
  char err[512] = {0};
  std::recursive_mutex mu;
};

namespace {

[[maybe_unused]] int fail(hh_ctx* ctx, int code, const char* fmt, ...) {
  if (ctx) {
    va_list ap;
    va_start(ap, fmt);
    vsnprintf(ctx->err, sizeof(ctx->err), fmt, ap);
    va_end(ap);
  }
  return code;
}

#define HH_HIP(ctx, expr)                                                                   \
  do {                                                                                      \
    hipError_t e__ = (hipError_t)(expr);                                                    \
    if (e__ != hipSuccess)                                                                  \
      return fail(ctx, HH_ERR_HIP, "%s failed: %s (%s:%d)", #expr, hipGetErrorString(e__),  \
                  __FILE__, __LINE__);                                                      \
  } while (0)

template <class T>
int ensure(hh_ctx* ctx, DevBuf<T>& buf, size_t need) {
  if (need <= buf.cap) return HH_OK;
  if (buf.p) HH_HIP(ctx, hipFree(buf.p));
  buf.p = nullptr;
  buf.cap = 0;
  hipError_t e = hipMalloc((void**)&buf.p, need * sizeof(T));
  if (e != hipSuccess)
    return fail(ctx, HH_ERR_NOMEM, "hipMalloc(%zu bytes) failed: %s", need * sizeof(T),
                hipGetErrorString(e));
  buf.cap = need;
  return HH_OK;
}

[[maybe_unused]] inline int note_host_copy(hh_ctx* ctx) {
  HH_HIP(ctx, hipEventRecord(ctx->ev_stage, ctx->stream));
  ctx->staged_host = true;
  return HH_OK;
}
template <class T>
int stage_host(hh_ctx* ctx, DevBuf<T>& buf, size_t need, const T* src, size_t n, const T** dev) {
  int rc = ensure(ctx, buf, need);
  if (rc) return rc;
  HH_HIP(ctx, hipMemcpyAsync(buf, src, n * sizeof(T), hipMemcpyHostToDevice, ctx->stream));
  if ((rc = note_host_copy(ctx))) return rc;
  *dev = buf;
  return HH_OK;
}
[[maybe_unused]] inline int release_host_operands(hh_ctx* ctx) {
  if (!ctx->staged_host) return HH_OK;
  ctx->staged_host = false;
  HH_HIP(ctx, hipEventSynchronize(ctx->ev_stage));
  return HH_OK;
}

[[maybe_unused]] inline int ensure_bk_scratch(hh_ctx* ctx, size_t need) {
  const size_t before = ctx->bk_scratch.cap;
  const int rc = ensure(ctx, ctx->bk_scratch, need);
  if (ctx->bk_scratch.cap != before) ctx->bk_table_key = hh::BkTableKey{};
  return rc;
}

struct WallClock {
  std::chrono::steady_clock::time_point t0 = std::chrono::steady_clock::now();
  double ms() const { return std::chrono::duration<double, std::milli>(std::chrono::steady_clock::now() - t0).count(); }
};

[[maybe_unused]] int finalize_results(const hh_model* models, size_t model_stride, const hh_config* c,
                                      const double* acc, uint32_t k, double kernel_ms, double total_ms,
                                      hh_result* out) {
  for (uint32_t i = 0; i < k; ++i) {
    std::memset(&out[i], 0, sizeof(hh_result));
    const int rc = hh_mc_finalize(&models[i * model_stride], c, acc + (size_t)i * HH_ACC_LEN, &out[i]);
    if (rc) return rc;
    out[i].kernel_ms = kernel_ms;
    out[i].total_ms = total_ms;
  }
  return HH_OK;
}

}
```

hedgehog.jl_amd/csrc/hh_kernels.h:

```cpp
#pragma once
#include <hip/hip_runtime.h>
#include <stdint.h>

#include "../../include/hedgehog_mc.h"
#include "hh_layout.h"

namespace hh {

constexpr int kRecStride = HH_ACC_LEN;
constexpr unsigned long long kPoison = 0x7FF8C0DE7FF8C0DEull;
constexpr unsigned long long kFinishSpinTicksDefault = 500000000ull;
constexpr int kRecItmS = 11;

template <int P>
struct DualT {
  double v;
  double d[P > 0 ? P : 1];
};

constexpr int kMaxBasis = 4;
enum { kBasisV0 = 0, kBasisKappa = 1, kBasisTheta = 2, kBasisSigma = 3 };
struct PartialMap {
  int sim;
  int n;
  int n_active;
  int basis[kMaxBasis];
  double w[HH_MAX_PARTIALS][kMaxBasis];
  double xdT[HH_MAX_PARTIALS];
  double dK[HH_MAX_PARTIALS];
};
template <int P>
struct SimArgs {
  DualT<P> x0;
  DualT<P> v0;
  DualT<P> kappa, theta, sigma;
  DualT<P> r;
  DualT<P> gdrift;
  DualT<P> strike;
  DualT<P> law_mu, law_sd;
  double dt, sqrt_dt, rho, rho_c, cp;
  uint64_t n_paths;
  uint64_t path_offset;
  uint32_t n_steps;
  uint32_t n_tiles;
  uint32_t tail_from;
  const uint64_t* seeds;
  const double* replay;
  double* terminal;
  double* terminal_d;
  double* records;
  double* accum;
  double acc_n_paths;
  unsigned int* finish_state;
  unsigned long long finish_spin_ticks;
  uint32_t reducer_tile;
  PartialMap map;
};

struct DevicePtrs {
  const uint64_t* seeds;
  const double* replay;
  double* terminal;
  double* terminal_d;
  double* records;
  double* accum;
  unsigned int* finish_state;
  long long finish_spin_ticks = -1;
  int finish_tile_first = 0;
  void* bk_scratch;
  struct BkTableKey* bk_table_key;
  int bk_term_cache;
  void* bk_sort;
  bool replay_path_major;
};
inline bool replay_direct_path_major(uint32_t n_steps, int ncomp) { return ((uint64_t)n_steps * ncomp) % 2 == 0; }
struct BkTableKey {
  const void* where;
  double nu;
  double kappa, sigma2, T;
};

constexpr int kBasketChunk = 4096;
struct BasketArgs {
  const double* terminal;
  const double* terminal_d;
  const double* strikes;
  const double* cps;
  uint64_t n_paths;
  uint32_t n_chunks;
  int antithetic;
  double* records;
};
inline uint32_t basket_chunks(uint64_t n_paths) {
  return (uint32_t)((n_paths + kBasketChunk - 1) / kBasketChunk);
}

constexpr int kExactPairs = 8, kExactPairsHuge = 64;
constexpr int kExactPairsSmall = 4;
int exact_pairs_per_lane(uint64_t n_paths);
inline uint32_t exact_records(uint64_t n_paths) {
  const uint64_t per = 512ull * (uint64_t)exact_pairs_per_lane(n_paths);
  return (uint32_t)((n_paths + per - 1) / per);
}
inline uint32_t sim_records(const hh_config& c) {
  return c.strategy == HH_EXACT_LAW ? exact_records(c.n_paths) : tiles_for(c.n_paths);
}
inline int pad_partials(uint32_t p) { return p <= 4 ? (int)p : 4; }

int launch_simulation(const hh_model& m, const hh_config& c, const DevicePtrs& p, hipStream_t s);
int launch_simulation_multi(const hh_model* models, int n_models, const hh_config& c, const DevicePtrs* p,
                            hipStream_t s);
constexpr int kMaxModelsPerPass = 4;
SimArgs<0> make_args0(const hh_model& m, const hh_config& c, const DevicePtrs& p);
struct BkTransition {
  const double* in_spot;
  const double* in_var;
  double* out_spot;
  double* out_var;
  uint32_t step;
};
bool bk_same_chain(const hh_model& a, const hh_model& b);
int launch_bk_refinish(const hh_model& m, const hh_config& c, const DevicePtrs& p, const double* rec0, hipStream_t s);
int launch_bk(const hh_model& m, const hh_config& c, const DevicePtrs& p, hipStream_t s,
              const BkTransition* tr = nullptr, bool upload_tables = true);
int launch_bk_grid(const hh_model& m, const hh_config& c, const DevicePtrs& p, hipStream_t s,
                   double* spot_rows, double* var_rows, uint32_t k0, uint32_t n_dates, bool upload_tables);
uint32_t bk_grid_dates_per_chain(uint64_t n_paths, uint32_t n_steps);
size_t bk_grid_sort_bytes(uint64_t n_chain);
size_t bk_scratch_bytes(uint64_t n_paths, int term_cache = 0);
void bk_diag_ptrs(const void* scratch, uint64_t n_paths, int term_cache, const uint32_t** decisions,
                  const uint32_t** series_len);
uint32_t bk_record_count(uint64_t n_paths);
const uint32_t* bk_live_records(const void* scratch, uint64_t n_paths);
int launch_copy_bk_counters(const double* src, double* accum, uint32_t n_groups, hipStream_t s);
int launch_fill_rows(double* spot0, double* var0, uint64_t n, double S0, double V0, hipStream_t s);
int launch_reduce_records(const double* records, uint32_t n_records, double n_paths, double* accum,
                          hipStream_t s, uint32_t n_groups = 1, const hh_model* m = nullptr,
                          const hh_config* c = nullptr, bool basket = false,
                          const uint32_t* n_records_dev = nullptr);
int count_active_partials(const hh_model& m, const hh_config& c);
int launch_basket_payoffs(const BasketArgs& b, uint32_t n_payoffs, uint32_t n_active_partials,
                          hipStream_t s);
constexpr uint32_t kCarrMadanMaxSubpanels = 1024;
uint32_t carr_madan_subpanels(double alpha, double bound);
int launch_carr_madan(const hh_model& m, int dynamics, int compat_sqrt_alpha, double alpha,
                      double bound, double* out_dev, hipStream_t s);
int launch_carr_madan_grad(const hh_model& m, int dynamics, int compat_sqrt_alpha, double alpha,
                           double bound, const double* per_payoff_dev, uint32_t n_payoffs,
                           double* out_dev, hipStream_t s);
int launch_carr_madan_basket(const hh_model& m, int dynamics, int compat_sqrt_alpha, double alpha,
                             double bound, const double* per_payoff_dev, uint32_t n_payoffs,
                             double* out_dev, hipStream_t s);
struct CrrTree {
  double F, K, cp, u, p, q, disc;
  int32_t style;
  uint32_t row;
};
int launch_crr(const CrrTree* trees_dev, const double* spot_factors_dev, int steps, uint32_t n_trees,
               double* out_dev, hipStream_t s);
struct FdOption {
  double S0, K, cp, r, T;
  double h, x0;
  double lo, di, up;
  int32_t style;
  int32_t pad_;
};
int launch_fd(const FdOption* opts_dev, int space_steps, int time_steps, int rannacher_steps, uint32_t n_options,
              double* out_dev, hipStream_t s);
uint32_t lsm_chunks(uint64_t ntot);
size_t lsm_scratch_doubles(uint64_t ntot, uint32_t n_steps, int degree);
enum { kLsmPhaseStats = 0, kLsmPhasePow = 1, kLsmPhaseInit = 2, kLsmPhaseStep = 3, kLsmPhaseFinal = 4 };
int launch_lsm_phase(int phase, uint32_t t, const double* grid, uint64_t ntot, uint32_t n_steps,
                     double strike, double cp, double step_discount, int degree, int32_t* tau,
                     double* val, double* scratch, double* records, const double* vec_in,
                     double* vec_out, hipStream_t s);
int launch_gbm_grid(const uint64_t* seeds_dev, uint64_t n_paths, uint32_t n_steps, double S0,
                    double r, double sigma, double T, int anti, double* grid, hipStream_t s);
int launch_euler_grid(const hh_model& m, const hh_config& c, const uint64_t* seeds_dev, bool log_state,
                      double* grid, double* var_grid, hipStream_t s);
int launch_path_stats(const hh_model& m, const hh_config& c, const uint64_t* seeds_dev, uint32_t monitor_every,
                      bool include_start, bool bridge, double* stats, hipStream_t s);
struct PathPayoffArgs {
  const double* stats;
  const hh_path_payoff* payoffs;
  double* values;
  double* records;
  double n_mon;
  uint64_t n_paths;
  uint32_t n_chunks;
  int antithetic;
  int extremes;
};
int launch_path_payoffs(const PathPayoffArgs& b, uint32_t n_payoffs, hipStream_t s);
double merton_compensator(const hh_jump& jump);
constexpr int kMertonPerLane = 8;
inline uint32_t merton_records(uint64_t n_paths) {
  const uint64_t per = (uint64_t)kTile * kMertonPerLane;
  return (uint32_t)((n_paths + per - 1) / per);
}
int launch_merton_exact(const hh_model& m, const hh_config& c, const hh_jump& jump, const DevicePtrs& p, hipStream_t s);
int launch_jump_stats(const hh_model& m, const hh_config& c, const hh_jump& jump, const uint64_t* seeds_dev,
                      uint32_t monitor_every, bool include_start, double* stats, hipStream_t s);
int launch_carr_madan_jump(const hh_model& m, const hh_jump& jump, double alpha, double bound,
                           const double* per_payoff_dev, uint32_t n_payoffs, double* out_dev, hipStream_t s);
enum { kLsmFormPerDate = 0, kLsmFormPersistent = 1, kLsmFormAuto = 2 };
int launch_lsm(const double* grid, uint64_t ntot, uint32_t n_steps, double strike, double cp,
               double step_discount, int degree, int32_t* tau, double* val, double* scratch,
               double* records, hipStream_t s, int form, int* form_used,
               unsigned long long spin_ticks = 100000000ull );
const unsigned int* lsm_persistent_status(const double* scratch, const LsmScratch& at);
int launch_wiener_fill(int dynamics, double rho, double sqrt_dt, uint32_t n_steps, uint64_t n_paths,
                       const uint64_t* seeds_dev, double* dst, hipStream_t s);
int launch_replay_pack(int ncomp, uint64_t n_paths, uint32_t n_steps, const double* src_dev,
                       double* dst_dev, hipStream_t s);

}
```

hedgehog.jl_amd/csrc/hh_kernels.hip:

```cpp
#include <type_traits>

#include "hh_sim.h"

namespace hh {



constexpr int kReplayChunk = 4;
constexpr int kReplayMaxWaves = 2;
constexpr int kReplayMaxWavesDual = 3;
constexpr int kReplayMaxWavesAnti = 8;

constexpr int replay_max_waves(bool replay, bool anti, int p) {
  return !replay ? 8 : anti ? kReplayMaxWavesAnti : p > 0 ? kReplayMaxWavesDual : kReplayMaxWaves;
}
template <class M, int P, bool REPLAY, bool ANTI>
__global__ __launch_bounds__(kTile)
__attribute__((amdgpu_waves_per_eu(1, replay_max_waves(REPLAY, ANTI, P)))) void euler_kernel(const SimArgs<P> a) {
  constexpr int NC = M::NCOMP;
  using State = typename M::State;

  const uint32_t tile = blockIdx.x;
  const uint32_t tid = threadIdx.x;
  const uint64_t path = (uint64_t)tile * kTile + tid;
// ... 188 lines not shown
      if constexpr (ANTI) M::step(sa, a, -d.x, -d.y);
    } else {
      M::step(st, a, d.x, 0.0);
      if constexpr (ANTI) M::step(sa, a, -d.x, 0.0);
      M::step(st, a, d.y, 0.0);
      if constexpr (ANTI) M::step(sa, a, -d.y, 0.0);
    }
  };

  if (n_chunks > 0) issue(0, true);
  for (int k = 0; k < n_chunks; ++k) {
    V2 d[NP];
#pragma unroll
    for (int j = 0; j < NP; ++j)
      d[j] = *reinterpret_cast<const V2*>(my_img + (((uint32_t)j ^ sw) << 4));
    asm volatile("s_waitcnt lgkmcnt(0)" ::: "memory");
    __builtin_amdgcn_sched_barrier(0);
    const bool full = k >= 1 && k <= k_full_end;
    if (k + 1 < n_chunks) issue(k + 1, !(k + 1 <= k_full_end));
    if (full) {
#pragma unroll
      for (int j = 0; j < NP; ++j) advance(d[j]);
    } else {
#pragma unroll
      for (int j = 0; j < NP; ++j) {
        const int t = NP * k - o + j;
        if (t >= 0 && t < T) advance(d[j]);
      }
    }
  }

  double acc[4 + P];
#pragma unroll
  for (int i = 0; i < 4 + P; ++i) acc[i] = 0.0;
  finish_path<P, ANTI>(st, sa, a, path, acc);
  block_reduce_publish<4 + P, kTile / 64, 2>(acc, a.records + (size_t)tile * kRecStride, a.accum != nullptr, a.map.n > 0);
  if (a.accum && reduces_records(tile, a)) finish_records<kTile, P>(a);
}


template <int P>
struct ExactState {
  DualT<P> x;
};

template <int P, bool REPLAY, bool ANTI, int PAIRS>
__global__ __launch_bounds__(kTile) void exact_gbm_kernel(const SimArgs<P> a) {
  const uint32_t chunk = blockIdx.x;
  const uint32_t tid = threadIdx.x;

  double acc[4 + P];
#pragma unroll
  for (int i = 0; i < 4 + P; ++i) acc[i] = 0.0;

#pragma unroll 2
  for (int jp = 0; jp < PAIRS; ++jp) {
    const uint64_t path0 = ((uint64_t)chunk * PAIRS + jp) * (2 * kTile) + (uint64_t)tid * 2;
    double z[2];
    exact_pair_normals<REPLAY>(a, path0, z);
#pragma unroll
    for (int j = 0; j < 2; ++j) {
      ExactState<P> st, sa;
      st.x.v = fma(a.law_sd.v, z[j], a.law_mu.v);
      if constexpr (ANTI) sa.x.v = 2 * a.law_mu.v - st.x.v;
      if constexpr (P > 0) {
#pragma unroll
        for (int k = 0; k < P; ++k) {
          st.x.d[k] = fma(a.law_sd.d[k], z[j], a.law_mu.d[k]);
          if constexpr (ANTI) sa.x.d[k] = 2 * a.law_mu.d[k] - st.x.d[k];
        }
      }
      finish_path<P, ANTI>(st, sa, a, path0 + j, acc);
    }
  }
  block_reduce_publish<4 + P, kTile / 64, 2>(acc, a.records + (size_t)chunk * kRecStride, a.accum != nullptr, a.map.n > 0);
  if (a.accum && reduces_records(chunk, a)) finish_records<kTile, P>(a);
}


__global__ __launch_bounds__(256) void reduce_records_kernel(const double* __restrict__ rec,
                                                              uint32_t n, double n_paths,
                                                              double* __restrict__ accum,
                                                              const PartialMap map,
                                                              const uint32_t* __restrict__ n_dev) {
  __shared__ double sm[257];
  const int slot = blockIdx.x;
  rec += (size_t)blockIdx.y * n * kRecStride;
  if (n_dev) n = min(n, *n_dev);
  accum += (size_t)blockIdx.y * kRecStride;
  double out;
  const int k = slot - HH_ACC_DSUM;
  if (map.n > 0 && k >= 0 && k < HH_MAX_PARTIALS) {
    out = 0.0;
    if (k < map.n) {
      for (int j = 0; j < map.n_active; ++j)
        if (map.w[k][j] != 0.0) out = fma(map.w[k][j], sum_slot(rec, n, HH_ACC_DSUM + j, sm), out);
      if (map.xdT[k] != 0.0) out = fma(map.xdT[k], sum_slot(rec, n, kRecItmS, sm), out);
      if (map.dK[k] != 0.0) out -= map.dK[k] * sum_slot(rec, n, kRecItmS + 1, sm);
    }
  } else if (map.sim && (slot == kRecItmS || slot == kRecItmS + 1)) {
    out = 0.0;
  } else {
    out = sum_slot(rec, n, slot, sm);
  }
  if (threadIdx.x == 0) accum[slot] = (slot == HH_ACC_NPATHS) ? n_paths : out;
}


constexpr int kFillSteps = 16;

template <int NC>
__global__ __launch_bounds__(kTile) void wiener_fill_kernel(double rho, double rho_c,
                                                            double sqrt_dt, uint32_t n_steps,
                                                            uint64_t n_paths,
                                                            const uint64_t* __restrict__ seeds,
                                                            double* __restrict__ dst) {
  const uint32_t tile = blockIdx.x;
  const uint32_t s0 = blockIdx.y * kFillSteps;
  const uint64_t path = (uint64_t)tile * kTile + threadIdx.x;
  const bool live = path < n_paths;
  const uint64_t key = live ? seeds[path] : 0ull;
  double* out = dst + (size_t)tile * n_steps * NC * kTile + threadIdx.x;
  for (uint32_t s = s0; s < s0 + kFillSteps && s < n_steps; ++s) {
    double z1, z2;
    if constexpr (NC == 2) {
      normal_pair(key, s, 0u, 0u, kDomEuler, z1, z2);
      const double d1 = sqrt_dt * z1;
      const double d2 = sqrt_dt * fma(rho, z1, rho_c * z2);
      out[((size_t)s * 2 + 0) * kTile] = live ? d1 : 0.0;
      out[((size_t)s * 2 + 1) * kTile] = live ? d2 : 0.0;
    } else {
      normal_pair(key, s >> 1, 0u, 0u, kDomEuler, z1, z2);
      const double d = sqrt_dt * ((s & 1u) ? z2 : z1);
      out[(size_t)s * kTile] = live ? d : 0.0;
    }
  }
}

constexpr int kPackSteps = 4;

template <int NC>
__global__ __launch_bounds__(256) void replay_pack_kernel(uint64_t n_paths, uint32_t n_steps,
                                                          const double* __restrict__ src,
                                                          double* __restrict__ dst) {
  constexpr int COLS = kPackSteps * NC;
  __shared__ double sm[kTile][COLS + 1];
  const uint32_t tile = blockIdx.x;
  const uint32_t s0 = blockIdx.y * kPackSteps;
  const int tid = threadIdx.x;
  const int col = tid % COLS, row0 = tid / COLS;
  constexpr int ROWS_PER_IT = 256 / COLS;
  for (int row = row0; row < kTile; row += ROWS_PER_IT) {
    const uint64_t path = (uint64_t)tile * kTile + row;
    const uint32_t s = s0 + col / NC;
    double v = 0.0;
    if (path < n_paths && s < n_steps) v = src[((size_t)path * n_steps + s0) * NC + col];
    sm[row][col] = v;
  }
  __syncthreads();
  double* out = dst + (size_t)tile * n_steps * NC * kTile + tid;
  for (int c = 0; c < COLS; ++c) {
    const uint32_t s = s0 + c / NC;
    if (s < n_steps) out[((size_t)s * NC + (c % NC)) * kTile] = sm[tid][c];
  }
}


static inline double seed_of(const double* p, uint32_t k, uint32_t n) {
  return (p && k < n) ? p[k] : 0.0;
}

static const double* basis_seeds(const hh_model& m, int b) {
  return b == kBasisV0 ? m.dV0 : b == kBasisKappa ? m.dkappa : b == kBasisTheta ? m.dtheta : m.dsigma;
}

static PartialMap classify_partials(const hh_model& m, const hh_config& c) {
  PartialMap pm{};
  const uint32_t np = c.n_partials < HH_MAX_PARTIALS ? c.n_partials : HH_MAX_PARTIALS;
  pm.n = (int)np;
  const bool euler = c.strategy == HH_EULER_MARUYAMA;
  const bool heston = c.dynamics == HH_HESTON;
  const double dt = m.T / (double)(c.n_steps ? c.n_steps : 1);
  const double sqT = sqrt(m.T), tmul = c.compat_sqrt_alpha ? sqT : m.T;
  for (int b = 0; b < kMaxBasis; ++b) {
    if (b != kBasisSigma && !(heston && euler)) continue;
    bool used = false;
    for (uint32_t k = 0; k < np; ++k) used = used || seed_of(basis_seeds(m, b), k, np) != 0.0;
    if (used) pm.basis[pm.n_active++] = b;
  }
  for (uint32_t k = 0; k < np; ++k) {
    for (int j = 0; j < pm.n_active; ++j) pm.w[k][j] = seed_of(basis_seeds(m, pm.basis[j]), k, np);
    pm.dK[k] = seed_of(m.dstrike, k, np);
    const double dr = seed_of(m.dr_drift, k, np);
    double xd = seed_of(m.dS0, k, np) / m.S0;
    if (euler) {
      if (dr != 0.0)
        for (uint32_t s = 0; s < c.n_steps; ++s) xd = fma(dt, dr, xd);
    } else {
      xd = xd + dr * tmul;
    }
    pm.xdT[k] = xd;
  }
  return pm;
}

int exact_pairs_per_lane(uint64_t n_paths) {
  return n_paths >= (uint64_t)2048 * 512 * kExactPairsHuge ? kExactPairsHuge
         : n_paths >= (uint64_t)2048 * 512 * kExactPairs   ? kExactPairs
                                                           : kExactPairsSmall;
}

int count_active_partials(const hh_model& m, const hh_config& c) {
  return classify_partials(m, c).n_active;
}

template <int P>
static SimArgs<P> make_args(const hh_model& m, const hh_config& c, const DevicePtrs& p,
                            const PartialMap& pm) {
  SimArgs<P> a{};
  const double sig2h = 0.5 * m.sigma * m.sigma;
  a.x0.v = log(m.S0);
  a.v0.v = m.V0;
  a.kappa.v = m.kappa;
  a.theta.v = m.theta;
  a.sigma.v = m.sigma;
  a.r.v = m.r_drift;
  a.gdrift.v = m.r_drift - sig2h;
  a.strike.v = m.strike;
  const double sqT = sqrt(m.T);
  const double tmul = c.compat_sqrt_alpha ? sqT : m.T;
  a.law_mu.v = a.x0.v + a.gdrift.v * tmul;
  a.law_sd.v = m.sigma * sqT;
  for (int j = 0; j < P && j < pm.n_active; ++j) {
    const int b = pm.basis[j];
    const double dsig = b == kBasisSigma ? 1.0 : 0.0;
    a.v0.d[j] = b == kBasisV0 ? 1.0 : 0.0;
    a.kappa.d[j] = b == kBasisKappa ? 1.0 : 0.0;
    a.theta.d[j] = b == kBasisTheta ? 1.0 : 0.0;
    a.sigma.d[j] = dsig;
    a.gdrift.d[j] = -m.sigma * dsig;
    a.law_mu.d[j] = a.gdrift.d[j] * tmul;
    a.law_sd.d[j] = dsig * sqT;
  }
  a.dt = m.T / (double)(c.n_steps ? c.n_steps : 1);
  a.sqrt_dt = sqrt(a.dt);
  a.rho = m.rho;
  a.rho_c = sqrt(1.0 - m.rho * m.rho);
  a.cp = m.cp;
  a.n_paths = c.n_paths;
  a.path_offset = c.path_offset;
  a.n_steps = c.n_steps;
  a.n_tiles = sim_records(c);
  a.seeds = p.seeds;
  a.replay = p.replay;
  a.terminal = p.terminal;
  a.terminal_d = p.terminal_d;
  a.records = p.records;
  a.accum = p.accum;
  a.acc_n_paths = (double)c.n_paths;
  a.finish_state = p.finish_state;
  a.finish_spin_ticks = p.finish_spin_ticks < 0 ? kFinishSpinTicksDefault : (unsigned long long)p.finish_spin_ticks;
  a.reducer_tile = p.finish_tile_first ? 0u : a.n_tiles - 1u;
  a.map = pm;
  return a;
}

SimArgs<0> make_args0(const hh_model& m, const hh_config& c, const DevicePtrs& p) {
  hh_config c0 = c;
  c0.n_partials = 0;
  return make_args<0>(m, c0, p, classify_partials(m, c0));
}

template <class M, int P, bool REPLAY, bool ANTI>
static int launch_euler_t(const SimArgs<P>& a, hipStream_t s) {
  hipLaunchKernelGGL((euler_kernel<M, P, REPLAY, ANTI>), dim3(a.n_tiles), dim3(kTile), 0, s, a);
  return (int)hipGetLastError();
}

template <class M, int P>
static int launch_euler_pm(const SimArgs<P>& a, bool anti, hipStream_t s) {
  auto kernel = anti ? euler_pm_kernel<M, P, true> : euler_pm_kernel<M, P, false>;
  hipLaunchKernelGGL(kernel, dim3(a.n_tiles), dim3(kTile), 0, s, a);
  return (int)hipGetLastError();
}

template <class M, int P>
static int launch_euler_m(const SimArgs<P>& a, bool replay, bool anti, hipStream_t s, bool path_major = false) {
  if (replay && path_major) return launch_euler_pm<M, P>(a, anti, s);
  if (replay) return anti ? launch_euler_t<M, P, true, true>(a, s) : launch_euler_t<M, P, true, false>(a, s);
  return anti ? launch_euler_t<M, P, false, true>(a, s) : launch_euler_t<M, P, false, false>(a, s);
}

template <int P>
static int launch_sim_p(const hh_model& m, const hh_config& c, const DevicePtrs& p,
                        const PartialMap& pm, hipStream_t s) {
  const SimArgs<P> a = make_args<P>(m, c, p, pm);
  const bool anti = c.antithetic != 0;
  const bool replay = c.noise_mode == HH_NOISE_REPLAY;
  if (c.strategy == HH_EXACT_LAW) {
    auto pick = [&](auto replay_c, auto anti_c) {
      constexpr bool R = decltype(replay_c)::value, A = decltype(anti_c)::value;
      const int pairs = exact_pairs_per_lane(c.n_paths);
      return pairs == kExactPairsHuge ? exact_gbm_kernel<P, R, A, kExactPairsHuge>
             : pairs == kExactPairs   ? exact_gbm_kernel<P, R, A, kExactPairs>
                                      : exact_gbm_kernel<P, R, A, kExactPairsSmall>;
    };
    using T = std::true_type;
    using F = std::false_type;
    auto kernel = replay ? (anti ? pick(T{}, T{}) : pick(T{}, F{})) : (anti ? pick(F{}, T{}) : pick(F{}, F{}));
    hipLaunchKernelGGL(kernel, dim3(a.n_tiles), dim3(kTile), 0, s, a);
    return (int)hipGetLastError();
  }
  const bool direct = replay && p.replay_path_major;
  if (c.dynamics == HH_LOGNORMAL) return launch_euler_m<GbmModel<P>, P>(a, replay, anti, s, direct);
  if (c.em_split) return launch_euler_m<HestonModel<P, true>, P>(a, replay, anti, s, direct);
  return launch_euler_m<HestonModel<P, false>, P>(a, replay, anti, s, direct);
}

int launch_simulation(const hh_model& m, const hh_config& c, const DevicePtrs& p, hipStream_t s) {
  const PartialMap pm = classify_partials(m, c);
  switch (pad_partials((uint32_t)pm.n_active)) {
    case 0: return launch_sim_p<0>(m, c, p, pm, s);
    case 1: return launch_sim_p<1>(m, c, p, pm, s);
    case 2: return launch_sim_p<2>(m, c, p, pm, s);
    case 3: return launch_sim_p<3>(m, c, p, pm, s);
    default: return launch_sim_p<4>(m, c, p, pm, s);
  }
}

int launch_reduce_records(const double* records, uint32_t n_records, double n_paths, double* accum,
                          hipStream_t s, uint32_t n_groups, const hh_model* m, const hh_config* c,
                          bool basket, const uint32_t* n_records_dev) {
  PartialMap pm{};
  if (m && c && (basket || c->strategy != HH_BROADIE_KAYA)) {
    if (c->n_partials) pm = classify_partials(*m, *c);
    pm.sim = 1;
    if (basket)
      for (double& d : pm.dK) d = 0.0;
  }
  hipLaunchKernelGGL(reduce_records_kernel, dim3(kRecStride, n_groups), dim3(256), 0, s, records,
                     n_records, n_paths, accum, pm, n_records_dev);
  return (int)hipGetLastError();
}


constexpr int kBasketKB = 4;

template <int P>
__global__ __launch_bounds__(256) void basket_payoff_kernel(const BasketArgs b, const uint32_t n_payoffs) {
  const uint32_t per_xcd = (b.n_chunks + 7u) / 8u;
  const uint32_t xcd = blockIdx.x & 7u, idx = blockIdx.x >> 3;
  const uint32_t grp = idx / per_xcd, chunk = (idx % per_xcd) * 8u + xcd;
  if (chunk >= b.n_chunks) return;
  const uint32_t k0 = grp * kBasketKB;
  double strike[kBasketKB], cp[kBasketKB];
#pragma unroll
  for (int g = 0; g < kBasketKB; ++g) {
    const uint32_t k = min(k0 + g, n_payoffs - 1);
    strike[g] = b.strikes[k];
    cp[g] = b.cps[k];
  }
  const uint64_t n_total = b.antithetic ? 2 * b.n_paths : b.n_paths;
  double acc[kBasketKB][4 + P];
#pragma unroll
  for (int g = 0; g < kBasketKB; ++g)
#pragma unroll
    for (int i = 0; i < 4 + P; ++i) acc[g][i] = 0.0;
  const uint64_t i0 = (uint64_t)chunk * kBasketChunk;
  for (uint32_t j = threadIdx.x; j < (uint32_t)kBasketChunk; j += 256) {
    const uint64_t i = i0 + j;
    if (i >= b.n_paths) break;
    const double S = b.terminal[i];
    double Sa = 0.0, d[P > 0 ? P : 1], da[P > 0 ? P : 1];
    if constexpr (P > 0) {
#pragma unroll
      for (int q = 0; q < P; ++q) d[q] = b.terminal_d[(uint64_t)q * n_total + i];
    }
    if (b.antithetic) {
      Sa = b.terminal[b.n_paths + i];
      if constexpr (P > 0) {
#pragma unroll
        for (int q = 0; q < P; ++q) da[q] = b.terminal_d[(uint64_t)q * n_total + b.n_paths + i];
      }
    }
#pragma unroll
    for (int g = 0; g < kBasketKB; ++g) {
      const double m = cp[g] * (S - strike[g]);
      const bool itm = m > 0.0;
      double p = itm ? m : 0.0;
      double wS = itm ? cp[g] * S : 0.0, wN = itm ? cp[g] : 0.0;
      double pd[P > 0 ? P : 1];
      if constexpr (P > 0) {
#pragma unroll
        for (int q = 0; q < P; ++q) pd[q] = itm ? cp[g] * d[q] : 0.0;
      }
      if (b.antithetic) {
        const double ma = cp[g] * (Sa - strike[g]);
        const bool itma = ma > 0.0;
        p = (p + (itma ? ma : 0.0)) / 2;
        wS = (wS + (itma ? cp[g] * Sa : 0.0)) / 2;
        wN = (wN + (itma ? cp[g] : 0.0)) / 2;
        if constexpr (P > 0) {
#pragma unroll
          for (int q = 0; q < P; ++q) pd[q] = (pd[q] + (itma ? cp[g] * da[q] : 0.0)) / 2;
        }
      }
      acc[g][0] += p;
      acc[g][1] = fma(p, p, acc[g][1]);
      if constexpr (P > 0) {
#pragma unroll
        for (int q = 0; q < P; ++q) acc[g][2 + q] += pd[q];
      }
      acc[g][2 + P] += wS;
      acc[g][3 + P] += wN;
    }
  }
#pragma unroll
  for (int g = 0; g < kBasketKB; ++g) {
    if (k0 + g >= n_payoffs) break;
    if (g) __syncthreads();
    block_reduce_store<4 + P, 4, 2>(acc[g], b.records + ((size_t)(k0 + g) * b.n_chunks + chunk) * kRecStride);
  }
}

// ... 56 lines not shown
```

hedgehog.jl_amd/csrc/hh_layout.h:

```cpp
#pragma once
#include "../../include/hedgehog_mc.h"

namespace hh {

constexpr int kTile = HH_TILE_PATHS;
inline uint32_t tiles_for(uint64_t n_paths) { return (uint32_t)((n_paths + kTile - 1) / kTile); }

struct LayoutCursor {
  size_t at = 0;
  size_t take(size_t n, size_t a = 1) {
    at = ((at + a - 1) & ~(a - 1)) + n;
    return at - n;
  }
};


constexpr int kLsmWg = 512;
constexpr int kLsmQSmall = 1024 / kLsmWg, kLsmQLarge = 8192 / kLsmWg;
constexpr uint64_t kLsmQ1Max = 1ull << 18;
constexpr int kLsmMaxResident = 256;
constexpr int kLsmRing = 16;
constexpr int kLsmStampSlots = 8;

inline int lsm_q(uint64_t ntot) {
  int q = kLsmQSmall;
  for (uint64_t cap = kLsmQ1Max; q < kLsmQLarge && ntot > cap; cap <<= 1) q <<= 1;
  return q;
}
inline uint32_t lsm_nch(uint64_t ntot) {
  const uint64_t per = (uint64_t)kLsmWg * lsm_q(ntot);
  return (uint32_t)((ntot + per - 1) / per);
}

struct LsmScratch {
  size_t sync, ring, rec_stats, rowstat, rec_pow, P, recB, disc_pow, counters, stamps, total;
  uint32_t rows, nch;
  int q;
  LsmScratch(uint64_t ntot, uint32_t n_steps, int degree) : rows(n_steps + 1), nch(lsm_nch(ntot)), q(lsm_q(ntot)) {
    const size_t r = rows, ch = nch, nv = 2 * (size_t)degree + 1;
    LayoutCursor c;
    sync = c.take(2);
    ring = c.take((size_t)kLsmRing * kLsmMaxResident * 32 * 2);
    rec_stats = c.take(r * ch * 3);
    rowstat = c.take(r * 3);
    rec_pow = c.take(r * ch * nv);
    P = c.take(r * nv);
    recB = c.take(r * ch * (degree + 1));
    disc_pow = c.take(r);
    counters = c.take(2);
    stamps = c.take(kLsmStampSlots);
    total = c.at;
  }
};


struct PathStatsLayout {
  size_t n_total, total;
  constexpr PathStatsLayout(uint64_t n_paths, bool antithetic, int rows = HH_PATH_STATS)
      : n_total((size_t)n_paths * (antithetic ? 2 : 1)), total((size_t)rows * n_total) {}
  constexpr size_t row(int stat) const { return (size_t)stat * n_total; }
};


constexpr int kSlots = 1536;
constexpr int kHeavyGrid = 64;
static_assert(kHeavyGrid <= kSlots, "the tail kernel's workgroup b uses slot b");
constexpr int kXcds = 8, kSlotLineWords = 16, kSlotLineBytes = 8 * kSlotLineWords;
constexpr int kBkTermCacheDefault = 256;
constexpr int kSortRun = 1024;

struct BkScratch {
  size_t long_mask, slot_lines, counters, args, tables, phi_cache, draws, iv, diag, total;
  size_t zeroed_bytes;
  size_t cache_columns, lanes;
  int cache_cap;
  uint32_t n_tiles;
  BkScratch(uint64_t n_chain, int term_cache, size_t sizeof_args, size_t sizeof_tables)
      : cache_cap(term_cache > 0 ? term_cache : kBkTermCacheDefault), n_tiles(tiles_for(n_chain)) {
    const size_t slots = n_tiles < (uint32_t)kHeavyGrid ? kHeavyGrid : n_tiles < (uint32_t)kSlots ? n_tiles : kSlots;
    cache_columns = slots * kTile;
    lanes = (size_t)n_tiles * kTile;
    LayoutCursor c;
    long_mask = c.take((size_t)n_tiles * (kTile / 64) * sizeof(uint64_t));
    slot_lines = c.take(kXcds * kSlotLineBytes, kSlotLineBytes);
    counters = c.take(kSlotLineBytes);
    zeroed_bytes = c.at - slot_lines;
    args = c.take(sizeof_args, 256);
    tables = c.take(sizeof_tables, 256);
    phi_cache = c.take(cache_columns * (size_t)cache_cap * sizeof(double), 256);
    draws = c.take(4 * lanes * sizeof(double));
    iv = c.take(lanes * sizeof(double));
    diag = c.take(2 * lanes * sizeof(uint32_t));
    total = c.at;
  }
};

// ... 16 lines not shown
```

hedgehog.jl_amd/csrc/hh_mgpu.hip:

```cpp
#include <dlfcn.h>

#include <array>
#include <atomic>
#include <chrono>
#include <condition_variable>
#include <cstdlib>
#include <cstring>
#include <functional>
#include <memory>
#include <thread>
#include <vector>

#include "hh_ctx.h"

namespace {

typedef struct ncclComm* rccl_comm_t;
constexpr int kNcclSuccess = 0, kNcclSum = 0, kNcclDouble = 8;

struct RcclApi {
  void* lib = nullptr;
  int (*CommInitAll)(rccl_comm_t*, int, const int*) = nullptr;
  int (*CommDestroy)(rccl_comm_t) = nullptr;
  int (*CommAbort)(rccl_comm_t) = nullptr;
  int (*GetVersion)(int*) = nullptr;
  char path[512] = {0};
  int from_env = 0;
  int (*AllReduce)(const void*, void*, size_t, int, int, rccl_comm_t, hipStream_t) = nullptr;
  int (*GroupStart)() = nullptr;
  int (*GroupEnd)() = nullptr;
  const char* (*GetErrorString)(int) = nullptr;
  char why[256] = {0};
  bool ok = false;
};

RcclApi& rccl() {
  static RcclApi api;
  static std::once_flag once;
  std::call_once(once, [] {
    const char* env = std::getenv("HEDGEHOG_MC_RCCL");
    if (env && *env) {
      api.lib = dlopen(env, RTLD_NOW | RTLD_LOCAL);
      api.from_env = api.lib != nullptr;
    }
    const char* loaded[] = {"librccl.so", "librccl.so.1"};
    for (const char* n : loaded)
      if (!api.lib) api.lib = dlopen(n, RTLD_NOW | RTLD_LOCAL | RTLD_NOLOAD);
    const char* names[] = {"librccl.so.1", "librccl.so", "/opt/rocm/lib/librccl.so.1"};
    for (const char* n : names)
      if (!api.lib) api.lib = dlopen(n, RTLD_NOW | RTLD_LOCAL);
    if (!api.lib) {
      snprintf(api.why, sizeof(api.why), "librccl not found (%s)", dlerror());
      return;
    }
    api.CommInitAll = (decltype(api.CommInitAll))dlsym(api.lib, "ncclCommInitAll");
    api.CommDestroy = (decltype(api.CommDestroy))dlsym(api.lib, "ncclCommDestroy");
    api.CommAbort = (decltype(api.CommAbort))dlsym(api.lib, "ncclCommAbort");
    api.AllReduce = (decltype(api.AllReduce))dlsym(api.lib, "ncclAllReduce");
    api.GroupStart = (decltype(api.GroupStart))dlsym(api.lib, "ncclGroupStart");
    api.GroupEnd = (decltype(api.GroupEnd))dlsym(api.lib, "ncclGroupEnd");
    api.GetErrorString = (decltype(api.GetErrorString))dlsym(api.lib, "ncclGetErrorString");
    api.GetVersion = (decltype(api.GetVersion))dlsym(api.lib, "ncclGetVersion");
    Dl_info info{};
    if (api.AllReduce && dladdr((void*)api.AllReduce, &info) && info.dli_fname)
      snprintf(api.path, sizeof(api.path), "%s", info.dli_fname);
    api.ok = api.CommInitAll && api.CommDestroy && api.CommAbort && api.AllReduce && api.GroupStart &&
             api.GroupEnd && api.GetErrorString;
    if (!api.ok) snprintf(api.why, sizeof(api.why), "librccl lacks an expected symbol");
  });
  return api;
}

}

struct hh_worker {
  std::thread th;
  std::mutex m;
  std::condition_variable cv;
  std::atomic<uint64_t> posted{0}, finished{0};
  std::atomic<int> parked{0}, stop{0};
  int rc = 0;
};

struct hh_mgpu {
  int n = 0;
  int flags = HH_MGPU_AUTO;
  int mode = HH_MGPU_REDUCE_HOST;
  bool rccl_lost = false;
  bool stuck = false;
  std::vector<int> devices;
  std::vector<hh_ctx*> ctx;
  std::vector<double*> acc, red;
  std::vector<size_t> acc_cap;
  std::vector<rccl_comm_t> comms;
  double* host = nullptr;
  size_t host_cap = 0;
  std::vector<double*> xchg;
  std::vector<size_t> xchg_cap;
  int enqueue = HH_MGPU_ENQUEUE_THREADS;
  std::vector<std::unique_ptr<hh_worker>> workers;
  const std::function<int(int)>* job = nullptr;
  std::vector<int> rcs;
  std::vector<std::array<char, 320>> derr;
  std::vector<double> enq_us;
  double enq_phase_us = 0.0;
  std::vector<hipEvent_t> pre;
  std::vector<hipEvent_t> fence;
  struct Retired {
    int device;
    hipStream_t s;
  };
  std::vector<Retired> retired;
  char err[512] = {0};
  std::mutex mu;
};

namespace {

using clk = std::chrono::steady_clock;
inline double us_since(clk::time_point t0) {
  return std::chrono::duration<double, std::micro>(clk::now() - t0).count();
}
inline void cpu_relax() {
#if defined(__x86_64__) && !defined(__HIP_DEVICE_COMPILE__)
  __builtin_ia32_pause();
#endif
}

int mfail(hh_mgpu* mg, int code, const char* fmt, ...) {
  if (mg) {
    va_list ap;
    va_start(ap, fmt);
    vsnprintf(mg->err, sizeof(mg->err), fmt, ap);
    va_end(ap);
  }
  return code;
}

int mfinalize_failed(hh_mgpu* mg, int rc) {
  for (int g = 0; g < mg->n; ++g)
    if (hh_ctx_check_last(mg->ctx[g]) == HH_ERR_DEVICE_TIMEOUT)
      rc = mfail(mg, HH_ERR_DEVICE_TIMEOUT, "device %d: %s", g, hh_last_error(mg->ctx[g]));
  return rc == HH_ERR_DEVICE_TIMEOUT ? rc : mfail(mg, rc, "finalize failed: the accumulator holds no trajectories");
}

#define HH_MHIP(mg, expr)                                                                     \
  do {                                                                                        \
    hipError_t e__ = (hipError_t)(expr);                                                      \
    if (e__ != hipSuccess)                                                                    \
      return mfail(mg, HH_ERR_HIP, "%s failed: %s (%s:%d)", #expr, hipGetErrorString(e__),    \
                   __FILE__, __LINE__);                                                       \
  } while (0)

#define HH_DHIP(mg, g, expr)                                                                       \
  do {                                                                                             \
    hipError_t e__ = (hipError_t)(expr);                                                           \
    if (e__ != hipSuccess) {                                                                       \
      snprintf(mg->derr[g].data(), mg->derr[g].size(), "%s failed: %s (%s:%d)", #expr,             \
               hipGetErrorString(e__), __FILE__, __LINE__);                                        \
      return HH_ERR_HIP;                                                                           \
    }                                                                                              \
  } while (0)

void shard_range(uint64_t n_paths, int n_dev, int g, bool tile_aligned, uint64_t* start, uint64_t* stop) {
  uint64_t per = (n_paths + (uint64_t)n_dev - 1) / (uint64_t)n_dev;
  if (tile_aligned) per = (per + hh::kTile - 1) / hh::kTile * hh::kTile;
  const uint64_t a = std::min(n_paths, (uint64_t)g * per);
  *start = a;
  *stop = std::min(n_paths, a + per);
}


constexpr double kSpinWindowUs = 150.0;

void worker_main(hh_mgpu* mg, int g) {
  hh_worker& w = *mg->workers[g - 1];
  (void)hipSetDevice(mg->devices[g]);
  uint64_t seen = 0;
  for (;;) {
    const auto idle0 = clk::now();
    while (w.posted.load() == seen && !w.stop.load()) {
      if (us_since(idle0) < kSpinWindowUs) {
// ... 98 lines not shown
    mg->host_cap = n_acc * (size_t)mg->n;
  }
  return HH_OK;
}

int drain(hh_mgpu* mg, int rc) {
  for (int g = 0; g < mg->n; ++g) {
    (void)hipSetDevice(mg->devices[g]);
    (void)hipStreamSynchronize(mg->ctx[g]->stream);
    mg->ctx[g]->shard.active = false;
  }
  return rc;
}
#define HH_MHIP_DRAIN(mg, expr)                                                                       \
  do {                                                                                                \
    hipError_t e__ = (hipError_t)(expr);                                                              \
    if (e__ != hipSuccess)                                                                            \
      return drain(mg, mfail(mg, HH_ERR_HIP, "%s failed: %s (%s:%d)", #expr, hipGetErrorString(e__), \
                             __FILE__, __LINE__));                                                    \
  } while (0)


int all_reduce_group(hh_mgpu* mg, double* const* send, double* const* recv, size_t n) {
  RcclApi& api = rccl();
  int e = api.GroupStart();
  for (int g = 0; g < mg->n && e == kNcclSuccess; ++g)
    e = api.AllReduce(send[g], recv[g], n, kNcclDouble, kNcclSum, mg->comms[g], mg->ctx[g]->stream);
  const int e2 = api.GroupEnd();
  return e == kNcclSuccess ? e2 : e;
}

bool rccl_give_up(hh_mgpu* mg) {
  RcclApi& api = rccl();
  for (rccl_comm_t c : mg->comms)
    if (c) (void)api.CommAbort(c);
  mg->comms.clear();
  mg->mode = HH_MGPU_REDUCE_HOST;
  mg->rccl_lost = true;
  bool all_moved = true;
  for (int g = 0; g < mg->n; ++g) {
    hh_ctx* c = mg->ctx[g];
    std::lock_guard<std::recursive_mutex> lock__(c->mu);
    c->shard.active = false;
    hipStream_t fresh = nullptr;
    (void)hipSetDevice(mg->devices[g]);
    if (c->stream != c->own_stream || hipStreamCreateWithFlags(&fresh, hipStreamNonBlocking) != hipSuccess) {
      all_moved = false;
      continue;
    }
    if (mg->fence[g]) (void)hipStreamWaitEvent(fresh, mg->fence[g], 0);
    mg->retired.push_back({mg->devices[g], c->own_stream});
    c->own_stream = c->stream = fresh;
  }
  mg->stuck = mg->stuck || !all_moved;
  return all_moved;
}

void wait_fences(hh_mgpu* mg) {
  for (int g = 0; g < mg->n; ++g)
    if (mg->fence[g]) {
      (void)hipSetDevice(mg->devices[g]);
      (void)hipEventSynchronize(mg->fence[g]);
    }
}

struct Basket {
  const double *strikes, *cps;
  uint32_t n_payoffs;
  uint32_t n_models = 0;
};

int run_shards(hh_mgpu* mg, const hh_model* m, const hh_config* cfgs, const Basket* basket,
               double* const* terminals, double* kernel_ms) {
  const bool multi = basket && basket->n_models > 0;
  const size_t n_acc = (size_t)HH_ACC_LEN * (multi ? basket->n_models : basket ? basket->n_payoffs : 1u);
  if (mg->stuck)
    return mfail(mg, HH_ERR_RCCL, "a collective failed and a shard could not be moved off the stream it was enqueued on "
                                  "(a stream lent with hh_ctx_set_stream, or no new stream): create a new context");
  if (mg->flags == HH_MGPU_RCCL && mg->rccl_lost)
    return drain(mg, mfail(mg, HH_ERR_RCCL, "the RCCL communicators of this context were aborted after a failed "
                                            "collective (HH_MGPU_RCCL does not fall back): create a new one"));
  int rc = ensure_acc(mg, n_acc);
  if (rc) return drain(mg, rc);
  const auto t_enq = clk::now();
  rc = for_each_device(mg, [&](int g) -> int {
    const auto t0 = clk::now();
    hh_ctx* c = mg->ctx[g];
    HH_DHIP(mg, g, hipSetDevice(mg->devices[g]));
    HH_DHIP(mg, g, hipEventRecord(c->ev0, c->stream));
    if (cfgs[g].n_paths == 0) {
      HH_DHIP(mg, g, hipMemsetAsync(mg->acc[g], 0, n_acc * sizeof(double), c->stream));
    } else {
      double* term = terminals ? terminals[g] : nullptr;
      const int r = multi    ? hh_mc_accumulate_multi(c, m, basket->n_models, &cfgs[g], mg->acc[g], nullptr)
                    : basket ? hh_mc_accumulate_basket(c, m, &cfgs[g], basket->strikes, basket->cps,
                                                       basket->n_payoffs, mg->acc[g], term)
                             : hh_mc_accumulate(c, m, &cfgs[g], mg->acc[g], term);
      if (r) {
        snprintf(mg->derr[g].data(), mg->derr[g].size(), "%s", hh_last_error(c));
        return r;
      }
    }
    HH_DHIP(mg, g, hipEventRecord(c->ev1, c->stream));
    mg->fence[g] = c->ev1;
    mg->enq_us[g] = us_since(t0);
    return HH_OK;
  });
  mg->enq_phase_us = us_since(t_enq);
  if (rc) return drain(mg, rc);
  bool reduced = false;
  if (mg->mode == HH_MGPU_REDUCE_RCCL) {
    const int e = all_reduce_group(mg, mg->acc.data(), mg->red.data(), n_acc);
    if (e == kNcclSuccess) {
      HH_MHIP_DRAIN(mg, hipSetDevice(mg->devices[0]));
      HH_MHIP_DRAIN(mg, hipMemcpyAsync(mg->host, mg->red[0], n_acc * sizeof(double), hipMemcpyDeviceToHost,
                                       mg->ctx[0]->stream));
      reduced = true;
    } else {
      mfail(mg, HH_ERR_RCCL, "ncclAllReduce failed: %s — communicators aborted, accumulators are summed on the host",
            rccl().GetErrorString(e));
      const bool moved = rccl_give_up(mg);
      if (mg->flags == HH_MGPU_RCCL || !moved) {
        wait_fences(mg);
        return HH_ERR_RCCL;
      }
    }
  }
  if (!reduced) {
    for (int g = 0; g < mg->n; ++g) {
      HH_MHIP_DRAIN(mg, hipSetDevice(mg->devices[g]));
      HH_MHIP_DRAIN(mg, hipMemcpyAsync(mg->host + (size_t)g * n_acc, mg->acc[g], n_acc * sizeof(double),
                                       hipMemcpyDeviceToHost, mg->ctx[g]->stream));
    }
  }
  for (int g = 0; g < mg->n; ++g) {
    HH_MHIP_DRAIN(mg, hipSetDevice(mg->devices[g]));
    HH_MHIP_DRAIN(mg, hipStreamSynchronize(mg->ctx[g]->stream));
  }
  if (!reduced) {
    for (int g = 1; g < mg->n; ++g)
      for (size_t i = 0; i < n_acc; ++i) mg->host[i] += mg->host[(size_t)g * n_acc + i];
  }
  double worst = 0.0;
  for (int g = 0; g < mg->n; ++g) {
    float ms = 0.f;
    HH_MHIP(mg, hipSetDevice(mg->devices[g]));
    HH_MHIP(mg, hipEventElapsedTime(&ms, mg->ctx[g]->ev0, mg->ctx[g]->ev1));
    if (ms > worst) worst = ms;
  }
  *kernel_ms = worst;
  return HH_OK;
}

int ncomp(int dynamics) { return dynamics == HH_HESTON ? 2 : 1; }

}

extern "C" {

void hh_mgpu_shard_range(uint64_t n_paths, int n_devices, int g, int tile_aligned, uint64_t* start,
                         uint64_t* stop) {
  uint64_t a = 0, b = 0;
  if (n_devices > 0 && g >= 0 && g < n_devices) shard_range(n_paths, n_devices, g, tile_aligned != 0, &a, &b);
  if (start) *start = a;
  if (stop) *stop = b;
}

int hh_mgpu_create(hh_mgpu** out, const int* device_ids, int n_devices, int flags) {
  if (!out) return HH_ERR_INVALID;
  *out = nullptr;
  if (!device_ids || n_devices < 1 || n_devices > 64) return HH_ERR_INVALID;
  if (flags != HH_MGPU_AUTO && flags != HH_MGPU_HOST_SUM && flags != HH_MGPU_RCCL) return HH_ERR_INVALID;
  int n_hip = 0;
  if (hipGetDeviceCount(&n_hip) != hipSuccess || n_hip <= 0) return HH_ERR_HIP;
  for (int g = 0; g < n_devices; ++g)
    if (device_ids[g] < 0 || device_ids[g] >= n_hip) return HH_ERR_INVALID;
  hh_mgpu* mg = new (std::nothrow) hh_mgpu();
  if (!mg) return HH_ERR_NOMEM;
  mg->n = n_devices;
  mg->flags = flags;
  mg->devices.assign(device_ids, device_ids + n_devices);
  mg->ctx.assign(n_devices, nullptr);
  mg->acc.assign(n_devices, nullptr);
  mg->red.assign(n_devices, nullptr);
  mg->acc_cap.assign(n_devices, 0);
  mg->xchg.assign(n_devices, nullptr);
  mg->xchg_cap.assign(n_devices, 0);
  mg->rcs.assign(n_devices, 0);
  mg->derr.resize(n_devices);
  mg->enq_us.assign(n_devices, 0.0);
  mg->pre.assign(n_devices, nullptr);
  mg->fence.assign(n_devices, nullptr);
  for (int g = 0; g < n_devices; ++g) {
    int rc = hh_ctx_create(&mg->ctx[g], device_ids[g]);
    if (!rc && hipEventCreateWithFlags(&mg->pre[g], hipEventDisableTiming) != hipSuccess) rc = HH_ERR_HIP;
    if (rc) {
      hh_mgpu_destroy(mg);
      return rc;
    }
  }
  const bool want = flags == HH_MGPU_RCCL || (flags == HH_MGPU_AUTO && n_devices > 1);
  if (want) {
    RcclApi& api = rccl();
    int e = -1;
    if (api.ok) {
      mg->comms.assign(n_devices, nullptr);
      e = api.CommInitAll(mg->comms.data(), n_devices, device_ids);
      if (e != kNcclSuccess) {
        mg->comms.clear();
        mfail(mg, HH_ERR_RCCL, "ncclCommInitAll failed: %s — accumulators are summed on the host",
              api.GetErrorString(e));
      }
    } else {
      mfail(mg, HH_ERR_RCCL, "RCCL unavailable: %s — accumulators are summed on the host", api.why);
    }
    if (e == kNcclSuccess) {
      mg->mode = HH_MGPU_REDUCE_RCCL;
    } else if (flags == HH_MGPU_RCCL) {
      hh_mgpu_destroy(mg);
      return HH_ERR_RCCL;
    }
  }
  *out = mg;
  return HH_OK;
}

void hh_mgpu_destroy(hh_mgpu* mg) {
  if (!mg) return;
  stop_workers(mg);
  std::vector<char> busy(mg->n, mg->stuck ? 1 : 0);
  for (const auto& r : mg->retired) {
    (void)hipSetDevice(r.device);
    if (hipStreamQuery(r.s) == hipSuccess) {
      (void)hipStreamDestroy(r.s);
    } else {
      for (int g = 0; g < mg->n; ++g)
        if (mg->devices[g] == r.device) busy[g] = 1;
    }
  }
  for (int g = 0; g < mg->n; ++g) {
    if (!mg->ctx[g] || busy[g]) continue;
    (void)hipSetDevice(mg->devices[g]);
    (void)hipStreamSynchronize(mg->ctx[g]->stream);
  }
  for (rccl_comm_t c : mg->comms)
    if (c) (void)rccl().CommDestroy(c);
  for (int g = 0; g < mg->n; ++g) {
    if (busy[g]) continue;
    if (mg->pre[g]) (void)hipEventDestroy(mg->pre[g]);
    if (!mg->ctx[g]) continue;
    (void)hipSetDevice(mg->devices[g]);
    if (mg->acc[g]) (void)hipFree(mg->acc[g]);
    if (mg->red[g]) (void)hipFree(mg->red[g]);
    if (mg->xchg[g]) (void)hipFree(mg->xchg[g]);
    if (mg->ctx[g]) hh_ctx_destroy(mg->ctx[g]);
  }
  bool any_busy = false;
  for (char b : busy) any_busy = any_busy || b;
  if (mg->host && !any_busy) (void)hipHostFree(mg->host);
  delete mg;
}

const char* hh_mgpu_last_error(const hh_mgpu* mg) { return mg ? mg->err : "hedgehog_mc: no multi-GPU context"; }
int hh_mgpu_n_devices(const hh_mgpu* mg) { return mg ? mg->n : 0; }
int hh_mgpu_reduce_mode(const hh_mgpu* mg) { return mg ? mg->mode : HH_MGPU_REDUCE_HOST; }
hh_ctx* hh_mgpu_ctx(hh_mgpu* mg, int i) { return (mg && i >= 0 && i < mg->n) ? mg->ctx[i] : nullptr; }

int hh_mgpu_selftest(hh_mgpu* mg, int32_t* ranks_out, int32_t* reduce_mode_out) {
  if (!mg) return HH_ERR_INVALID;
  std::lock_guard<std::mutex> lock__(mg->mu);
  if (!ranks_out) return mfail(mg, HH_ERR_INVALID, "hh_mgpu_selftest: ranks_out is NULL");
  if (mg->stuck) return mfail(mg, HH_ERR_RCCL, "stuck context (see hh_mgpu_last_error of the failed call)");
  int rc = ensure_acc(mg, HH_ACC_LEN);
  if (rc) return rc;
  std::vector<double> ones(HH_ACC_LEN, 1.0);
  for (int g = 0; g < mg->n; ++g) {
    HH_MHIP_DRAIN(mg, hipSetDevice(mg->devices[g]));
    HH_MHIP_DRAIN(mg, hipMemcpyAsync(mg->acc[g], ones.data(), HH_ACC_LEN * sizeof(double), hipMemcpyHostToDevice,
                                     mg->ctx[g]->stream));
    HH_MHIP_DRAIN(mg, hipMemsetAsync(mg->red[g], 0, HH_ACC_LEN * sizeof(double), mg->ctx[g]->stream));
    HH_MHIP_DRAIN(mg, hipEventRecord(mg->pre[g], mg->ctx[g]->stream));
    mg->fence[g] = mg->pre[g];
  }
  for (int g = 0; g < mg->n; ++g) {
    HH_MHIP_DRAIN(mg, hipSetDevice(mg->devices[g]));
    HH_MHIP_DRAIN(mg, hipStreamSynchronize(mg->ctx[g]->stream));
  }
  double total = 0.0;
  if (mg->mode == HH_MGPU_REDUCE_RCCL) {
    const int e = all_reduce_group(mg, mg->acc.data(), mg->red.data(), HH_ACC_LEN);
    if (e != kNcclSuccess) {
      mfail(mg, HH_ERR_RCCL, "ncclAllReduce failed in the self-test: %s — communicators aborted", rccl().GetErrorString(e));
      (void)rccl_give_up(mg);
      wait_fences(mg);
      return HH_ERR_RCCL;
    }
    for (int g = 0; g < mg->n; ++g) {
      HH_MHIP_DRAIN(mg, hipSetDevice(mg->devices[g]));
      HH_MHIP_DRAIN(mg, hipMemcpyAsync(mg->host + (size_t)g * HH_ACC_LEN, mg->red[g], HH_ACC_LEN * sizeof(double),
                                       hipMemcpyDeviceToHost, mg->ctx[g]->stream));
    }
    for (int g = 0; g < mg->n; ++g) {
      HH_MHIP_DRAIN(mg, hipSetDevice(mg->devices[g]));
      HH_MHIP_DRAIN(mg, hipStreamSynchronize(mg->ctx[g]->stream));
    }
    total = mg->host[0];
    for (size_t i = 0; i < (size_t)mg->n * HH_ACC_LEN; ++i)
      if (mg->host[i] != total) {
        mfail(mg, HH_ERR_RCCL, "self-test: the ranks disagree on the all-reduced count (%g vs %g) — communicators aborted",
              mg->host[i], total);
        (void)rccl_give_up(mg);
        wait_fences(mg);
        return HH_ERR_RCCL;
      }
  } else {
    for (int g = 0; g < mg->n; ++g) {
      HH_MHIP_DRAIN(mg, hipSetDevice(mg->devices[g]));
      HH_MHIP_DRAIN(mg, hipMemcpyAsync(mg->host + (size_t)g * HH_ACC_LEN, mg->acc[g], HH_ACC_LEN * sizeof(double),
                                       hipMemcpyDeviceToHost, mg->ctx[g]->stream));
    }
    for (int g = 0; g < mg->n; ++g) {
      HH_MHIP_DRAIN(mg, hipSetDevice(mg->devices[g]));
      HH_MHIP_DRAIN(mg, hipStreamSynchronize(mg->ctx[g]->stream));
    }
    for (int g = 0; g < mg->n; ++g) total += mg->host[(size_t)g * HH_ACC_LEN];
  }
  *ranks_out = (int32_t)(total + 0.5);
  if (reduce_mode_out) *reduce_mode_out = mg->mode;
  return HH_OK;
}

int hh_mgpu_rccl_info(const hh_mgpu* mg, char* path_out, size_t cap, int32_t* version_out, int32_t* from_env_out) {
  (void)mg;
  RcclApi& api = rccl();
  if (path_out && cap) snprintf(path_out, cap, "%s", api.lib ? api.path : "");
  int v = 0;
  if (api.lib && api.GetVersion && api.GetVersion(&v) != kNcclSuccess) v = 0;
  if (version_out) *version_out = v;
  if (from_env_out) *from_env_out = api.from_env;
  return api.ok ? HH_OK : HH_ERR_RCCL;
}

int hh_mgpu_set_option(hh_mgpu* mg, int32_t option, int64_t value) {
  if (!mg) return HH_ERR_INVALID;
  std::lock_guard<std::mutex> lock__(mg->mu);
  switch (option) {
    case HH_MGPU_OPT_ENQUEUE:
      if (value != HH_MGPU_ENQUEUE_SERIAL && value != HH_MGPU_ENQUEUE_THREADS)
        return mfail(mg, HH_ERR_INVALID, "HH_MGPU_OPT_ENQUEUE: 0 (one shard after the other) or 1 (a thread per device)");
      if (value == HH_MGPU_ENQUEUE_SERIAL) stop_workers(mg);
      mg->enqueue = (int)value;
      return HH_OK;
    default:
      return mfail(mg, HH_ERR_INVALID, "unknown option %d", option);
  }
}

int hh_mgpu_enqueue_stats(hh_mgpu* mg, double* shard_us, double* phase_us) {
  if (!mg) return HH_ERR_INVALID;
  std::lock_guard<std::mutex> lock__(mg->mu);
  if (shard_us)
    for (int g = 0; g < mg->n; ++g) shard_us[g] = mg->enq_us[g];
  if (phase_us) *phase_us = mg->enq_phase_us;
  return HH_OK;
}

int hh_mgpu_solve_shards(hh_mgpu* mg, const hh_model* m, const hh_config* cfgs, hh_result* out,
                         double* const* terminals) {
  if (!mg) return HH_ERR_INVALID;
  std::lock_guard<std::mutex> lock__(mg->mu);
  if (!m || !cfgs || !out) return mfail(mg, HH_ERR_INVALID, "hh_mgpu_solve_shards: NULL argument");
  const WallClock clock;
  int first = -1;
  for (int g = 0; g < mg->n && first < 0; ++g)
    if (cfgs[g].n_paths) first = g;
  if (first < 0) return mfail(mg, HH_ERR_INVALID, "every shard is empty");
  std::memset(out, 0, sizeof(*out));
  double kernel_ms = 0.0;
  int rc = run_shards(mg, m, cfgs, nullptr, terminals, &kernel_ms);
  if (rc) return rc;
  rc = hh_mc_finalize(m, &cfgs[first], mg->host, out);
  if (rc) return mfinalize_failed(mg, rc);
  out->kernel_ms = kernel_ms;
  out->total_ms = clock.ms();
  return HH_OK;
}

struct Shards {
  std::vector<hh_config> cfg;
  std::vector<double*> terminal;
  std::vector<uint64_t> start;
};

static int cut_config(hh_mgpu* mg, const hh_config* cfg, bool want_terminal, Shards& sh) {
  if (cfg->n_paths == 0) return mfail(mg, HH_ERR_INVALID, "n_paths must be >= 1");
  if (cfg->seeds_on_device || cfg->replay_on_device || cfg->terminal_on_device)
    return mfail(mg, HH_ERR_INVALID,
                 "hh_mgpu_solve takes host buffers; device-resident shards go through hh_mgpu_solve_shards");
  const bool euler = cfg->strategy == HH_EULER_MARUYAMA;
  const bool replay = cfg->noise_mode == HH_NOISE_REPLAY;
  const bool bk = cfg->strategy == HH_BROADIE_KAYA;
  const bool tile = replay && euler && cfg->replay_layout == HH_REPLAY_TILE_MAJOR;
  if (replay && !cfg->replay) return mfail(mg, HH_ERR_INVALID, "REPLAY needs a replay buffer");
  if (replay && ((uintptr_t)cfg->replay & 15u) != 0)
    return mfail(mg, HH_ERR_INVALID, "replay buffer must be 16-byte aligned");
  if (!replay && !cfg->seeds) return mfail(mg, HH_ERR_INVALID, "GENERATE needs seeds");
  const uint64_t N = cfg->n_paths;
  const size_t per_path = euler ? (size_t)cfg->n_steps * ncomp(cfg->dynamics) : 1;
  if (replay && cfg->replay_len) {
    const uint64_t need = bk ? 3 * N : tile ? (uint64_t)hh::tiles_for(N) * hh::kTile * per_path : N * per_path;
    if (cfg->replay_len < need)
      return mfail(mg, HH_ERR_INVALID, "replay buffer holds %llu elements, %llu needed",
                   (unsigned long long)cfg->replay_len, (unsigned long long)need);
  }
  if (!replay && cfg->seeds_len && cfg->seeds_len < (euler ? N : 1))
    return mfail(mg, HH_ERR_INVALID, "Number of seeds (%llu) must be >= number of trajectories (%llu)",
                 (unsigned long long)cfg->seeds_len, (unsigned long long)(euler ? N : 1));
  sh.cfg.assign(mg->n, *cfg);
  sh.terminal.assign(mg->n, nullptr);
  sh.start.assign(mg->n, 0);
  for (int g = 0; g < mg->n; ++g) {
    uint64_t a, b;
    shard_range(N, mg->n, g, tile, &a, &b);
    hh_config& c = sh.cfg[g];
    hh_ctx* x = mg->ctx[g];
    sh.start[g] = a;
    c.n_paths = b - a;
    c.path_offset = cfg->path_offset + a;
    c.seeds_len = c.replay_len = 0;
    if (c.n_paths == 0) continue;
    if (!replay && euler) c.seeds = cfg->seeds + a;
    if (replay && !bk) c.replay = cfg->replay + a * per_path;
    HH_MHIP(mg, hipSetDevice(mg->devices[g]));
    if (replay && bk) {
// ... 263 lines not shown
```

hedgehog.jl_amd/csrc/hh_reduce.h:

```cpp
#pragma once
#include <hip/hip_runtime.h>

#include "hh_kernels.h"

namespace hh {

__device__ __forceinline__ double tree256(const double* __restrict__ p) {
  const int l = threadIdx.x & 63;
  double a = p[l] + p[l + 128];
  const double b = p[l + 64] + p[l + 192];
  a += b;
#pragma unroll
  for (int off = 32; off > 0; off >>= 1) a += __shfl_down(a, off, 64);
  return __shfl(a, 0, 64);
}

__device__ __forceinline__ double sum_slot(const double* __restrict__ rec, uint32_t n, int slot,
                                           double* sm) {
  const int tid = threadIdx.x;
  double t = 0.0;
  for (uint32_t b = tid; b < n; b += 256 * 16) {
    double v[16];
#pragma unroll
    for (int u = 0; u < 16; ++u) {
      const uint32_t i = b + 256u * u;
      v[u] = i < n ? rec[(size_t)i * kRecStride + slot] : 0.0;
    }
#pragma unroll
    for (int u = 0; u < 16; ++u) t += v[u];
  }
  __syncthreads();
  sm[tid] = t;
  __syncthreads();
  double r = 0.0;
  if (tid < 64) r = tree256(sm);
  if (tid == 0) sm[256] = r;
  __syncthreads();
  return sm[256];
}

}
```

hedgehog.jl_amd/csrc/hh_sim.h:

```cpp
#pragma once
#include <type_traits>

#include "hh_kernels.h"
#include "hh_reduce.h"
#include "hh_rng.h"

namespace hh {


__device__ __forceinline__ double sqrt_clipped(double w) {
  const double y = __builtin_fmin(__builtin_amdgcn_rsq(w), 0x1p1000);
  double g = w * y, h = 0.5 * y;
  const double r = fma(-h, g, 0.5);
  g = fma(g, r, g);
  h = fma(h, r, h);
  g = fma(fma(-g, g, w), h, g);
  return fma(fma(-g, g, w), h, g);
}

template <int P, bool SPLIT>
struct HestonModel {
  static constexpr int NCOMP = 2;
  struct State {
    DualT<P> x, v;
// ... 333 lines not shown
#pragma unroll
          for (int q = 0; q < NS; ++q) {
            v[q][u] = i < n ? load_through(rec + (size_t)i * kRecStride + slot_of(q)) : 0.0;
            there = there && !is_poison(v[q][u]);
          }
        }
        if (there || give || !keep_waiting(since, give, gave_up, spin_ticks, state)) break;
      }
#pragma unroll
      for (int q = 0; q < NS; ++q)
#pragma unroll
        for (int u = 0; u < kB; ++u) t[q] += v[q][u];
    }
#pragma unroll
    for (int q = 0; q < NS; ++q) sm[q * 256 + vt] = t[q];
  }
}

template <int NT, int P, class Args>
__device__ __forceinline__ void finish_records(const Args& a) {
  double* __restrict__ records = a.records;
  double* __restrict__ accum = a.accum;
  const uint32_t n_rec = a.n_tiles;
  const double n_paths = a.acc_n_paths;
  const PartialMap* map = &a.map;
  const unsigned long long spin_ticks = a.finish_spin_ticks;
  __shared__ double sm[4 * 256];
  __shared__ unsigned int gave_up;
  const unsigned int state_in_flight = scalar_load_begin(a.finish_state);
  if (threadIdx.x == 0) gave_up = 0u;
  __syncthreads();
  const bool itm = map->n > 0;
  const double poison = __longlong_as_double((long long)kPoison);
  const auto wsrc = __builtin_amdgcn_make_buffer_rsrc(records, 0, (int)(n_rec * (uint32_t)(kRecStride * 8)), 0x00020000);
  const unsigned int ph = (unsigned int)(kPoison >> 32), pl = (unsigned int)kPoison;
  partial_pairs<NT>(records, n_rec, sm, &gave_up, spin_ticks, a.finish_state);
  if (itm) partial_slots<NT, 2>(records, n_rec, [](int q) { return kRecItmS + q; }, sm + 512, &gave_up, spin_ticks, a.finish_state);
  for (uint32_t i = threadIdx.x; i < n_rec; i += NT) {
    __builtin_amdgcn_raw_buffer_store_b128(u32x4{pl, ph, pl, ph}, wsrc, (int)(i * (uint32_t)(kRecStride * 8)), 0, 16);
    if (itm) {
      store_through(records + (size_t)i * kRecStride + kRecItmS, poison);
      store_through(records + (size_t)i * kRecStride + kRecItmS + 1, poison);
    }
  }
  __syncthreads();
  double s[4] = {0.0, 0.0, 0.0, 0.0}, d[P > 0 ? P : 1];
  if (threadIdx.x < 64) {
    s[0] = tree256(sm);
    s[1] = tree256(sm + 256);
    if (itm) {
      s[2] = tree256(sm + 512);
      s[3] = tree256(sm + 768);
    }
  }
  if constexpr (P > 0) {
    __syncthreads();
    partial_slots<NT, P>(records, n_rec, [](int q) { return HH_ACC_DSUM + q; }, sm, &gave_up, spin_ticks, a.finish_state);
    for (uint32_t i = threadIdx.x; i < n_rec; i += NT) {
#pragma unroll
      for (int j = 0; j < P; ++j) store_through(records + (size_t)i * kRecStride + HH_ACC_DSUM + j, poison);
    }
    __syncthreads();
    if (threadIdx.x < 64) {
#pragma unroll
      for (int j = 0; j < P; ++j) d[j] = tree256(sm + j * 256);
    }
  }
  if (threadIdx.x < (unsigned)kRecStride) {
    const int slot = threadIdx.x;
    double out = slot == HH_ACC_SUM ? s[0] : slot == HH_ACC_SUMSQ ? s[1] : 0.0;
    const int k = slot - HH_ACC_DSUM;
    if (k >= 0 && k < map->n) {
      out = 0.0;
      if constexpr (P > 0) {
#pragma unroll
        for (int j = 0; j < P; ++j)
          if (j < map->n_active && map->w[k][j] != 0.0) out = fma(map->w[k][j], d[j], out);
      }
      if (map->xdT[k] != 0.0) out = fma(map->xdT[k], s[2], out);
      if (map->dK[k] != 0.0) out -= map->dK[k] * s[3];
    }
    if (slot == HH_ACC_NPATHS) out = n_paths;
    const bool dirty = scalar_load_end(state_in_flight) != 0u;
    accum[slot] = (gave_up || dirty) ? __longlong_as_double(0x7FF8000000000000ll) : out;
    if (slot == 0 && gave_up) __hip_atomic_store(a.finish_state, 1u, __ATOMIC_RELAXED, __HIP_MEMORY_SCOPE_AGENT);
  }
}


__device__ __forceinline__ double stream_load(const double* p) { return __builtin_nontemporal_load(p); }

}
```

include/hedgehog_mc.h:

```cpp
#ifndef HEDGEHOG_MC_H
#define HEDGEHOG_MC_H

#include <stddef.h>
#include <stdint.h>

#ifdef __cplusplus
extern "C" {
#endif

#define HH_ABI_VERSION 6
#define HH_MAX_PARTIALS 8
#define HH_TILE_PATHS 256
#define HH_ACC_LEN 16
#define HH_MAX_MODELS 16

#define HH_ACC_SUM 0
#define HH_ACC_SUMSQ 1
#define HH_ACC_DSUM 2
#define HH_ACC_NPATHS 10
#define HH_ACC_BK_NEWTON_FAIL 11
#define HH_ACC_BK_BISECT 12
#define HH_ACC_BK_MAXGUESS 13
#define HH_ACC_BK_CF_TERMS 14

enum hh_status {
  HH_OK = 0,
  HH_ERR_INVALID = -1,
  HH_ERR_UNSUPPORTED = -2,
  HH_ERR_HIP = -3,
  HH_ERR_NOMEM = -4,
  HH_ERR_RCCL = -5,
  HH_ERR_DEVICE_TIMEOUT = -6
};

enum hh_dynamics { HH_LOGNORMAL = 0, HH_HESTON = 1 };
enum hh_strategy { HH_EULER_MARUYAMA = 0, HH_EXACT_LAW = 1, HH_BROADIE_KAYA = 2 };
enum hh_noise_mode { HH_NOISE_GENERATE = 0, HH_NOISE_REPLAY = 1 };
enum hh_replay_layout { HH_REPLAY_TILE_MAJOR = 0, HH_REPLAY_PATH_MAJOR = 1 };

enum hh_bk_root_form { HH_BK_ROOT_SECANT = 0,
                       HH_BK_ROOT_ORDER2 = 1 };
enum hh_bk_bracket_form { HH_BK_BRACKET_MIDPOINT = 0,
                          HH_BK_BRACKET_ROOTS = 1 };
enum hh_bk_caps { HH_BK_CAPS_AS_WRITTEN = 0,
                  HH_BK_CAPS_ROOTS_DEFAULT = 1 };

typedef struct hh_ctx hh_ctx;

typedef struct hh_model {
  double S0, V0, kappa, theta, sigma, rho;
  double r_drift, discount, T, strike, cp;
  const double *dS0, *dV0, *dkappa, *dtheta, *dsigma, *dr_drift, *ddiscount, *dstrike;
} hh_model;

typedef struct hh_config {
  int32_t dynamics;
  int32_t strategy;
  int32_t antithetic;
  int32_t em_split;
  int32_t compat_sqrt_alpha;
  int32_t noise_mode;
  int32_t replay_layout;
  int32_t seeds_on_device;
  int32_t replay_on_device;
  int32_t terminal_on_device;
  uint32_t n_steps;
  uint32_t n_partials;
  uint64_t n_paths;
  uint64_t path_offset;
  const uint64_t* seeds;
  const double* replay;
  double bk_n_sigma;
  double bk_cf_tol;
  double bk_atol;
  double bk_moment_h;
  int32_t bk_newton_maxiter;
  int32_t bk_bisect_maxiter;
  int32_t bk_root_form;
  int32_t bk_bracket_form;
  int32_t bk_caps;
  int32_t reserved0;
  uint64_t seeds_len;
  uint64_t replay_len;
} hh_config;

typedef struct hh_result {
  double price;
  double std_error;
  double sum_payoff, sumsq_payoff;
  double dprice[HH_MAX_PARTIALS];
  uint64_t n_paths_done;
  uint64_t bk_newton_fail, bk_bisect_fallback, bk_maxguess_fallback, bk_cf_terms;
  double kernel_ms;
  double total_ms;
} hh_result;

int hh_abi_version(void);

int hh_ctx_create(hh_ctx** out, int device_id);
void hh_ctx_destroy(hh_ctx* ctx);
int hh_ctx_set_stream(hh_ctx* ctx, void* hip_stream);
int hh_ctx_reset_stream(hh_ctx* ctx);
const char* hh_last_error(const hh_ctx* ctx);
enum hh_option { HH_OPT_LSM_FORM = 1, HH_OPT_BK_TERM_CACHE = 2, HH_OPT_GRID_FORM = 3, HH_OPT_LSM_SPIN_TICKS = 4,
                 HH_OPT_FUSE_REDUCE = 5, HH_OPT_GRID_ORDER = 6, HH_OPT_FINISH_SPIN_TICKS = 7,
                 HH_OPT_FINISH_TILE_FIRST = 8 };
enum hh_grid_form { HH_GRID_FORM_PER_DATE = 0, HH_GRID_FORM_BATCHED = 1 };
enum hh_lsm_form { HH_LSM_FORM_PER_DATE = 0, HH_LSM_FORM_PERSISTENT = 1, HH_LSM_FORM_AUTO = 2 };
int hh_ctx_set_option(hh_ctx* ctx, int32_t option, int64_t value);
int hh_ctx_check_last(hh_ctx* ctx);

int hh_mc_solve(hh_ctx* ctx, const hh_model* model, const hh_config* cfg, hh_result* out,
                double* terminal);

int hh_mc_accumulate(hh_ctx* ctx, const hh_model* model, const hh_config* cfg, double* accum_dev,
                     double* terminal);
int hh_mc_finalize(const hh_model* model, const hh_config* cfg, const double* accum_host,
                   hh_result* out);

int hh_mc_solve_multi(hh_ctx* ctx, const hh_model* models, uint32_t n_models, const hh_config* cfg,
                      hh_result* out, double* const* terminals);
int hh_mc_accumulate_multi(hh_ctx* ctx, const hh_model* models, uint32_t n_models, const hh_config* cfg,
                           double* accum_dev, double* const* terminals);

int hh_bk_decisions(hh_ctx* ctx, uint64_t n_paths, uint32_t* decisions, uint32_t* series_len);

typedef struct hh_mgpu hh_mgpu;
enum hh_mgpu_flags { HH_MGPU_AUTO = 0, HH_MGPU_HOST_SUM = 1, HH_MGPU_RCCL = 2 };
enum hh_mgpu_reduce { HH_MGPU_REDUCE_HOST = 0, HH_MGPU_REDUCE_RCCL = 1 };
int hh_mgpu_create(hh_mgpu** out, const int* device_ids, int n_devices, int flags);
void hh_mgpu_destroy(hh_mgpu* mg);
const char* hh_mgpu_last_error(const hh_mgpu* mg);
int hh_mgpu_n_devices(const hh_mgpu* mg);
int hh_mgpu_reduce_mode(const hh_mgpu* mg);
int hh_mgpu_selftest(hh_mgpu* mg, int32_t* ranks_out, int32_t* reduce_mode_out );
int hh_mgpu_rccl_info(const hh_mgpu* mg, char* path_out, size_t cap, int32_t* version_out, int32_t* from_env_out);
enum hh_mgpu_option { HH_MGPU_OPT_ENQUEUE = 1 };
enum hh_mgpu_enqueue { HH_MGPU_ENQUEUE_SERIAL = 0, HH_MGPU_ENQUEUE_THREADS = 1  };
int hh_mgpu_set_option(hh_mgpu* mg, int32_t option, int64_t value);
int hh_mgpu_enqueue_stats(hh_mgpu* mg, double* shard_us, double* phase_us);
hh_ctx* hh_mgpu_ctx(hh_mgpu* mg, int i);
void hh_mgpu_shard_range(uint64_t n_paths, int n_devices, int g, int tile_aligned, uint64_t* start,
                         uint64_t* stop);
int hh_mgpu_solve(hh_mgpu* mg, const hh_model* model, const hh_config* cfg, hh_result* out,
                  double* terminal);
int hh_mgpu_solve_shards(hh_mgpu* mg, const hh_model* model, const hh_config* shard_cfgs ,
                         hh_result* out, double* const* terminals );
int hh_mgpu_solve_basket(hh_mgpu* mg, const hh_model* model, const hh_config* cfg, const double* strikes,
                         const double* cps, uint32_t n_payoffs, hh_result* out );
int hh_mgpu_solve_multi(hh_mgpu* mg, const hh_model* models, uint32_t n_models, const hh_config* cfg,
                        hh_result* out );


int hh_mc_accumulate_basket(hh_ctx* ctx, const hh_model* model, const hh_config* cfg,
                            const double* strikes, const double* cps, uint32_t n_payoffs,
                            double* accum_dev, double* terminal);
int hh_mc_solve_basket(hh_ctx* ctx, const hh_model* model, const hh_config* cfg,
                       const double* strikes, const double* cps, uint32_t n_payoffs,
                       hh_result* out , double* terminal);

int hh_carr_madan(hh_ctx* ctx, const hh_model* model, int32_t dynamics, int32_t compat_sqrt_alpha,
                  double alpha, double bound, double* price_out);
int hh_carr_madan_basket(hh_ctx* ctx, const hh_model* model, int32_t dynamics,
                         int32_t compat_sqrt_alpha, double alpha, double bound, const double* strikes,
                         const double* cps, const double* Ts, const double* r_drifts,
                         const double* discounts, uint32_t n_payoffs, double* prices_out);
enum hh_cm_grad { HH_CM_GRAD_S0 = 0, HH_CM_GRAD_V0, HH_CM_GRAD_KAPPA, HH_CM_GRAD_THETA, HH_CM_GRAD_SIGMA,
                  HH_CM_GRAD_RHO, HH_CM_GRAD_R_DRIFT, HH_CM_GRAD_DISCOUNT, HH_CM_GRAD_LEN };
int hh_carr_madan_basket_grad(hh_ctx* ctx, const hh_model* model, int32_t dynamics,
                              int32_t compat_sqrt_alpha, double alpha, double bound,
                              const double* strikes, const double* cps, const double* Ts,
                              const double* r_drifts, const double* discounts, uint32_t n_payoffs,
                              double* prices_out, double* grad_out);

#define HH_CRR_MAX_STEPS 32768
#define HH_CRR_FORM_A_MAX_STEPS 2047
enum hh_crr_style { HH_CRR_EUROPEAN = 0, HH_CRR_AMERICAN_FORWARD = 1, HH_CRR_AMERICAN_SPOT = 2 };
int hh_crr_solve(hh_ctx* ctx, int32_t steps, uint32_t n_trees, const double* forwards, const double* strikes,
                 const double* cps, const double* ups, const double* discounts, const int32_t* styles,
                 const double* spot_factors, uint32_t n_spot_rows, const uint32_t* spot_row_of_tree,
                 double* prices_out);

#define HH_FD_MAX_SPACE 4096
#define HH_FD_MAX_TIME 65536
#define HH_FD_FORM_A_MAX_SPACE 1024
enum hh_fd_style { HH_FD_EUROPEAN = 0, HH_FD_AMERICAN = 1 };
int hh_fd_solve(hh_ctx* ctx, int32_t space_steps, int32_t time_steps, int32_t rannacher_steps, uint32_t n_options,
                const double* spots, const double* strikes, const double* cps, const double* sigmas,
                const double* rates, const double* expiries, const double* half_widths, const int32_t* styles,
                double* prices_out, double* deltas_out, double* gammas_out);

typedef struct hh_lsm_result {
  double price, std_error;
  uint64_t n_paths_total;
  uint32_t rows_regressed, rows_skipped;
  double kernel_ms, total_ms;
  int32_t form;
  int32_t persistent_fallbacks;
} hh_lsm_result;
size_t hh_lsm_grid_elems(uint64_t n_paths, uint32_t n_steps, int32_t antithetic);
int hh_lsm_solve(hh_ctx* ctx, const hh_model* model, const hh_config* cfg, int32_t degree,
                 double step_discount, hh_lsm_result* out, int32_t* stop_time, double* stop_value,
                 double* spot_grid);
int hh_lsm_solve_grid(hh_ctx* ctx, const hh_model* model, const double* spot_grid_dev,
                      uint64_t n_paths, uint32_t n_steps, int32_t degree, double step_discount,
                      hh_lsm_result* out, int32_t* stop_time, double* stop_value);

enum hh_path_state { HH_PATH_SPOT = 0, HH_PATH_LOG = 1 };
int hh_euler_grid(hh_ctx* ctx, const hh_model* model, const hh_config* cfg, int32_t path_state,
                  double* spot_grid, double* var_grid, int32_t grids_on_device, hh_result* out);
int hh_lsm_solve_euler(hh_ctx* ctx, const hh_model* model, const hh_config* cfg, int32_t path_state,
                       int32_t degree, double step_discount, hh_lsm_result* out, int32_t* stop_time,
                       double* stop_value, double* spot_grid);

enum hh_path_payoff_kind { HH_PAYOFF_VANILLA = 0, HH_PAYOFF_ASIAN_ARITH = 1, HH_PAYOFF_ASIAN_GEOM = 2,
                           HH_PAYOFF_BARRIER = 3, HH_PAYOFF_DIGITAL_CASH = 4, HH_PAYOFF_DIGITAL_ASSET = 5,
                           HH_PAYOFF_LOOKBACK_FLOAT = 6, HH_PAYOFF_LOOKBACK_FIXED = 7  };
enum hh_barrier_type { HH_BARRIER_UP_OUT = 0, HH_BARRIER_UP_IN = 1, HH_BARRIER_DOWN_OUT = 2, HH_BARRIER_DOWN_IN = 3 };
enum hh_path_stat { HH_STAT_SUM_S = 0, HH_STAT_SUM_X = 1, HH_STAT_MAX_S = 2, HH_STAT_MIN_S = 3, HH_STAT_S_T = 4,
                    HH_STAT_CMAX_S = 5, HH_STAT_CMIN_S = 6  };
// ... 76 lines not shown
```

Before: 430.8 billion.

## Deliver reduced sums directly to mapped host memory, skip D2H copy and events

```diff
diff --git a/hedgehog.jl_amd/_ffi.py b/hedgehog.jl_amd/_ffi.py
--- a/hedgehog.jl_amd/_ffi.py
+++ b/hedgehog.jl_amd/_ffi.py
@@ -32,6 +32,7 @@
 HH_MGPU_AUTO, HH_MGPU_HOST_SUM, HH_MGPU_RCCL = 0, 1, 2
 HH_MGPU_REDUCE_HOST, HH_MGPU_REDUCE_RCCL = 0, 1
 HH_MGPU_OPT_ENQUEUE = 1
+HH_MGPU_OPT_KERNEL_MS = 2
 HH_MGPU_ENQUEUE_SERIAL, HH_MGPU_ENQUEUE_THREADS = 0, 1
 
 _dp = C.POINTER(C.c_double)
@@ -101,6 +102,7 @@
 HH_OPT_GRID_ORDER = 6
 HH_OPT_FINISH_SPIN_TICKS = 7
 HH_OPT_FINISH_TILE_FIRST = 8
+HH_OPT_SOLVE_KERNEL_MS = 9
 HH_GRID_FORM_PER_DATE, HH_GRID_FORM_BATCHED = 0, 1
 HH_CM_GRAD_LEN = 8
 HH_LSM_FORM_PER_DATE, HH_LSM_FORM_PERSISTENT, HH_LSM_FORM_AUTO = 0, 1, 2
diff --git a/hedgehog.jl_amd/csrc/hh_api.hip b/hedgehog.jl_amd/csrc/hh_api.hip
--- a/hedgehog.jl_amd/csrc/hh_api.hip
+++ b/hedgehog.jl_amd/csrc/hh_api.hip
@@ -147,13 +147,19 @@
   return rf ? rf : fail(ctx, rc, "finalize failed: the accumulator holds no trajectories");
 }
 
+bool solve_is_timed(const hh_ctx* ctx) { return ctx->solve_kernel_ms != 0 || ctx->timing; }
+
+int not_delivered(hh_ctx* ctx) {
+  return fail(ctx, HH_ERR_HIP, "the solve's kernels ran and left no sums in the context's host slot");
+}
+
 size_t replay_elems(uint64_t n_paths, uint32_t n_steps, int dynamics) {
   return (size_t)hh::tiles_for(n_paths) * n_steps * ncomp_of(dynamics) * hh::kTile;
 }
 
-int solve_times(hh_ctx* ctx, const WallClock& clock, double* kernel_ms, double* total_ms) {
+int solve_times(hh_ctx* ctx, const WallClock& clock, double* kernel_ms, double* total_ms, bool timed = true) {
   float ms = 0.f;
-  HH_HIP(ctx, hipEventElapsedTime(&ms, ctx->ev0, ctx->ev1));
+  if (timed) HH_HIP(ctx, hipEventElapsedTime(&ms, ctx->ev0, ctx->ev1));
   *kernel_ms = ms;
   *total_ms = clock.ms();
   return HH_OK;
@@ -189,7 +195,10 @@
       hipMalloc((void**)&ctx->finish_state, 2 * sizeof(unsigned int)) != hipSuccess ||
       hipMemset(ctx->finish_state, 0, 2 * sizeof(unsigned int)) != hipSuccess ||
       hipHostMalloc((void**)&ctx->accum_host, (HH_ACC_LEN + 8) * sizeof(double), hipHostMallocDefault) !=
-          hipSuccess) {
+          hipSuccess ||
+      hipHostMalloc((void**)&ctx->deliver_host, hh::DeliverRing().total * sizeof(double),
+                    hipHostMallocMapped | hipHostMallocCoherent) != hipSuccess ||
+      hipHostGetDevicePointer((void**)&ctx->deliver_dev, ctx->deliver_host, 0) != hipSuccess) {
     hh_ctx_destroy(ctx);
     return HH_ERR_HIP;
   }
@@ -208,6 +217,7 @@
   if (ctx->accum) (void)hipFree(ctx->accum);
   if (ctx->finish_state) (void)hipFree(ctx->finish_state);
   if (ctx->accum_host) (void)hipHostFree(ctx->accum_host);
+  if (ctx->deliver_host) (void)hipHostFree(ctx->deliver_host);
   for (auto& pr : ctx->tev)
     for (auto& e : pr)
       if (e) (void)hipEventDestroy(e);
@@ -282,6 +292,11 @@
       if (value < 0 || value > 2)
         return fail(ctx, HH_ERR_INVALID, "HH_OPT_FUSE_REDUCE: 0 (a second kernel reduces the records), 1 (the simulation kernel does) or 2 (by size)");
       ctx->fuse_reduce = (int)value;
+      return HH_OK;
+    case HH_OPT_SOLVE_KERNEL_MS:
+      if (value != 0 && value != 1)
+        return fail(ctx, HH_ERR_INVALID, "HH_OPT_SOLVE_KERNEL_MS: 1 (hh_result::kernel_ms is measured) or 0 (no events, kernel_ms = 0)");
+      ctx->solve_kernel_ms = (int)value;
       return HH_OK;
     default:
       return fail(ctx, HH_ERR_INVALID, "unknown option %d", option);
@@ -389,7 +404,7 @@
 
 static int run_simulation(hh_ctx* ctx, const hh_model* m, const hh_config* c, double* terminal,
                           bool need_terminal_dev, double** terminal_dev_out, double* accum_dev = nullptr,
-                          bool* reduced = nullptr) {
+                          bool* reduced = nullptr, double* host_accum = nullptr) {
   int rc = HH_OK;
   const uint32_t n_tiles = hh::tiles_for(c->n_paths);
   const bool bk = c->strategy == HH_BROADIE_KAYA;
@@ -405,6 +420,7 @@
     p.accum = accum_dev;
     fused_controls(ctx, p);
   }
+  if (fuse || bk) p.host_accum = host_accum;
   if (reduced) *reduced = fuse || bk;
   if (bk) {
     rc = ensure_bk_scratch(ctx, hh::bk_scratch_bytes(c->n_paths, ctx->bk_term_cache));
@@ -463,22 +479,32 @@
 
 int hh_mc_accumulate(hh_ctx* ctx, const hh_model* m, const hh_config* c, double* accum_dev,
                      double* terminal) {
+  return hh_accumulate_delivered(ctx, m, c, accum_dev, terminal, nullptr);
+}
+
+}
+
+int hh_accumulate_delivered(hh_ctx* ctx, const hh_model* m, const hh_config* c, double* accum_dev, double* terminal,
+                            double* host_accum) {
   if (!ctx) return HH_ERR_INVALID;
   std::lock_guard<std::recursive_mutex> lock__(ctx->mu);
   int rc = validate(ctx, m, c);
   if (rc) return rc;
   if (!accum_dev) return fail(ctx, HH_ERR_INVALID, "accum_dev is NULL");
-  HH_HIP(ctx, hipSetDevice(ctx->device));
+  HH_HIP(ctx, set_device(ctx->device));
   bool reduced = false;
-  rc = run_simulation(ctx, m, c, terminal, false, nullptr, accum_dev, &reduced);
+  rc = run_simulation(ctx, m, c, terminal, false, nullptr, accum_dev, &reduced, host_accum);
   if (rc) return rc;
   if (!reduced)
-    HH_HIP(ctx, hh::launch_reduce_records(ctx->records, hh::sim_records(*c), (double)c->n_paths, accum_dev, ctx->stream, 1, m, c));
+    HH_HIP(ctx, hh::launch_reduce_records(ctx->records, hh::sim_records(*c), (double)c->n_paths, accum_dev, ctx->stream, 1, m, c,
+                                          false, nullptr, host_accum));
   if ((rc = end_timing(ctx))) return rc;
   if ((rc = release_host_operands(ctx))) return rc;
   return copy_back_terminal(ctx, c, terminal);
 }
 
+extern "C" {
+
 static int next_pass(int remaining) {
   if (remaining <= hh::kMaxModelsPerPass) return remaining;
   return remaining == hh::kMaxModelsPerPass + 1 ? hh::kMaxModelsPerPass - 1 : hh::kMaxModelsPerPass;
@@ -486,6 +512,13 @@
 
 int hh_mc_accumulate_multi(hh_ctx* ctx, const hh_model* models, uint32_t n_models, const hh_config* c,
                            double* accum_dev, double* const* terminals) {
+  return hh_accumulate_multi_delivered(ctx, models, n_models, c, accum_dev, terminals, nullptr);
+}
+
+}
+
+int hh_accumulate_multi_delivered(hh_ctx* ctx, const hh_model* models, uint32_t n_models, const hh_config* c,
+                                  double* accum_dev, double* const* terminals, double* host_accum) {
   if (!ctx) return HH_ERR_INVALID;
   std::lock_guard<std::recursive_mutex> lock__(ctx->mu);
   if (!models || n_models == 0 || n_models > HH_MAX_MODELS)
@@ -496,8 +529,9 @@
     if ((rc = validate(ctx, &models[k], c))) return rc;
   if (c->n_partials)
     return fail(ctx, HH_ERR_UNSUPPORTED, "several models in one pass carry no dual partials (n_partials must be 0)");
-  if (n_models == 1) return hh_mc_accumulate(ctx, models, c, accum_dev, terminals ? terminals[0] : nullptr);
-  HH_HIP(ctx, hipSetDevice(ctx->device));
+  if (n_models == 1) return hh_accumulate_delivered(ctx, models, c, accum_dev, terminals ? terminals[0] : nullptr, host_accum);
+  HH_HIP(ctx, set_device(ctx->device));
+  auto host_of = [&](uint32_t k) { return host_accum ? host_accum + (size_t)k * HH_ACC_LEN : nullptr; };
   if (c->strategy == HH_BROADIE_KAYA) {
     const uint32_t count = hh::bk_record_count(c->n_paths);
     if ((rc = ensure(ctx, ctx->records, 2 * (size_t)count * hh::kRecStride))) return rc;
@@ -510,7 +544,8 @@
         }
     for (uint32_t k = 0; k < n_models; ++k) {
       if (leader[k] >= 0) continue;
-      if ((rc = hh_mc_accumulate(ctx, &models[k], c, accum_dev + (size_t)k * HH_ACC_LEN, terminals ? terminals[k] : nullptr)))
+      if ((rc = hh_accumulate_delivered(ctx, &models[k], c, accum_dev + (size_t)k * HH_ACC_LEN,
+                                        terminals ? terminals[k] : nullptr, host_of(k))))
         return rc;
       for (uint32_t f = k + 1; f < n_models; ++f) {
         if (leader[f] != (int)k) continue;
@@ -529,7 +564,7 @@
         HH_HIP(ctx, hh::launch_bk_refinish(models[f], *c, p, ctx->records, ctx->stream));
         HH_HIP(ctx, hh::launch_reduce_records(p.records, count, (double)c->n_paths, accum_dev + (size_t)f * HH_ACC_LEN,
                                               ctx->stream, 1, &models[f], c, false,
-                                              hh::bk_live_records(ctx->bk_scratch, c->n_paths)));
+                                              hh::bk_live_records(ctx->bk_scratch, c->n_paths), host_of(f)));
         if ((rc = end_timing(ctx))) return rc;
         if ((rc = copy_back_terminal(ctx, c, terminal))) return rc;
       }
@@ -555,6 +590,7 @@
   for (uint32_t k = 0; k < n_models; ++k) {
     p[k].records = (fuse ? ctx->frecords : ctx->records) + (size_t)k * rec_elems;
     p[k].accum = fuse ? accum_dev + (size_t)k * HH_ACC_LEN : nullptr;
+    p[k].host_accum = fuse ? host_of(k) : nullptr;
     double* t = terminals ? terminals[k] : nullptr;
     p[k].terminal = !t ? nullptr : c->terminal_on_device ? t : ctx->terminal + (size_t)k * n_term;
   }
@@ -565,7 +601,8 @@
     if (!fuse)
       for (int k = 0; k < take; ++k)
         HH_HIP(ctx, hh::launch_reduce_records(p[k0 + k].records, hh::sim_records(*c), (double)c->n_paths,
-                                              accum_dev + (size_t)(k0 + k) * HH_ACC_LEN, ctx->stream, 1, &models[k0 + k], c));
+                                              accum_dev + (size_t)(k0 + k) * HH_ACC_LEN, ctx->stream, 1, &models[k0 + k], c,
+                                              false, nullptr, host_of(k0 + k)));
     k0 += (uint32_t)take;
   }
   if ((rc = end_timing(ctx))) return rc;
@@ -579,6 +616,8 @@
   return HH_OK;
 }
 
+extern "C" {
+
 int hh_mc_solve_multi(hh_ctx* ctx, const hh_model* models, uint32_t n_models, const hh_config* c, hh_result* out,
                       double* const* terminals) {
   if (!ctx) return HH_ERR_INVALID;
@@ -586,19 +625,20 @@
   if (!out || !models || n_models == 0 || n_models > HH_MAX_MODELS)
     return fail(ctx, HH_ERR_INVALID, "hh_mc_solve_multi: 1 .. %d models and their results", HH_MAX_MODELS);
   const WallClock clock;
-  HH_HIP(ctx, hipSetDevice(ctx->device));
+  HH_HIP(ctx, set_device(ctx->device));
   const size_t n_acc = (size_t)n_models * HH_ACC_LEN;
   int rc = ensure(ctx, ctx->basket_accum, n_acc);
   if (rc) return rc;
-  HH_HIP(ctx, hipEventRecord(ctx->ev0, ctx->stream));
-  if ((rc = hh_mc_accumulate_multi(ctx, models, n_models, c, ctx->basket_accum, terminals))) return rc;
-  HH_HIP(ctx, hipEventRecord(ctx->ev1, ctx->stream));
-  double host[HH_MAX_MODELS * HH_ACC_LEN];
-  HH_HIP(ctx, hipMemcpyAsync(host, ctx->basket_accum, n_acc * sizeof(double), hipMemcpyDeviceToHost, ctx->stream));
-  HH_HIP(ctx, hipStreamSynchronize(ctx->stream));
+  const bool timed = solve_is_timed(ctx);
+  const DeliverSlot slot = take_deliver_slot(ctx, n_models);
+  if (timed) HH_HIP(ctx, hipEventRecord(ctx->ev0, ctx->stream));
+  if ((rc = hh_accumulate_multi_delivered(ctx, models, n_models, c, ctx->basket_accum, terminals, slot.dev))) return rc;
+  if (timed) HH_HIP(ctx, hipEventRecord(ctx->ev1, ctx->stream));
+  HH_HIP(ctx, hipStreamSynchronize(ctx->stream));
+  if (!delivered(slot.host, n_models)) return not_delivered(ctx);
   double kernel_ms, total_ms;
-  if ((rc = solve_times(ctx, clock, &kernel_ms, &total_ms))) return rc;
-  rc = finalize_results(models, 1, c, host, n_models, kernel_ms, total_ms, out);
+  if ((rc = solve_times(ctx, clock, &kernel_ms, &total_ms, timed))) return rc;
+  rc = finalize_results(models, 1, c, slot.host, n_models, kernel_ms, total_ms, out);
   return rc ? finalize_failed(ctx, rc) : HH_OK;
 }
 
@@ -704,17 +744,18 @@
   if (!out) return fail(ctx, HH_ERR_INVALID, "result is NULL");
   const WallClock clock;
   std::memset(out, 0, sizeof(*out));
-  HH_HIP(ctx, hipSetDevice(ctx->device));
-  HH_HIP(ctx, hipEventRecord(ctx->ev0, ctx->stream));
-  int rc = hh_mc_accumulate(ctx, m, c, ctx->accum, terminal);
-  if (rc) return rc;
-  HH_HIP(ctx, hipEventRecord(ctx->ev1, ctx->stream));
-  HH_HIP(ctx, hipMemcpyAsync(ctx->accum_host, ctx->accum, HH_ACC_LEN * sizeof(double),
-                             hipMemcpyDeviceToHost, ctx->stream));
-  HH_HIP(ctx, hipStreamSynchronize(ctx->stream));
-  rc = hh_mc_finalize(m, c, ctx->accum_host, out);
+  HH_HIP(ctx, set_device(ctx->device));
+  const bool timed = solve_is_timed(ctx);
+  const DeliverSlot slot = take_deliver_slot(ctx, 1);
+  if (timed) HH_HIP(ctx, hipEventRecord(ctx->ev0, ctx->stream));
+  int rc = hh_accumulate_delivered(ctx, m, c, ctx->accum, terminal, slot.dev);
+  if (rc) return rc;
+  if (timed) HH_HIP(ctx, hipEventRecord(ctx->ev1, ctx->stream));
+  HH_HIP(ctx, hipStreamSynchronize(ctx->stream));
+  if (!delivered(slot.host, 1)) return not_delivered(ctx);
+  rc = hh_mc_finalize(m, c, slot.host, out);
   if (rc) return finalize_failed(ctx, rc);
-  return solve_times(ctx, clock, &out->kernel_ms, &out->total_ms);
+  return solve_times(ctx, clock, &out->kernel_ms, &out->total_ms, timed);
 }
 
 int hh_ctx_check_last(hh_ctx* ctx) {
diff --git a/hedgehog.jl_amd/csrc/hh_bk.hip b/hedgehog.jl_amd/csrc/hh_bk.hip
--- a/hedgehog.jl_amd/csrc/hh_bk.hip
+++ b/hedgehog.jl_amd/csrc/hh_bk.hip
@@ -1077,7 +1077,8 @@
 
 __global__ __launch_bounds__(kTile) void bk_tail_kernel(const BkArgs* __restrict__ args, const BkTables* __restrict__ tabs,
                                                         uint32_t n_tiles, double n_paths, double* __restrict__ accum,
-                                                        uint32_t* __restrict__ cnt, const double* __restrict__ records) {
+                                                        uint32_t* __restrict__ cnt, const double* __restrict__ records,
+                                                        double* __restrict__ host_accum) {
   const uint32_t b = blockIdx.x, tid = threadIdx.x;
   __shared__ double sm[257];
   const uint32_t n_long_v = __hip_atomic_load(cnt, __ATOMIC_RELAXED, __HIP_MEMORY_SCOPE_AGENT);
@@ -1119,7 +1120,9 @@
     return;
   }
   if (tid == 0) {
-    accum[b] = b == (uint32_t)HH_ACC_NPATHS ? n_paths : out;
+    const double sum = b == (uint32_t)HH_ACC_NPATHS ? n_paths : out;
+    accum[b] = sum;
+    if (host_accum) deliver_store(host_accum + b, sum);
     if (b == 0u) cnt[1] = n_rec;
   }
 }
@@ -1409,7 +1412,8 @@
   return v;
 }
 
-void bk_chain(const BkArgs& a0, const BkLayout& L, hipStream_t s, double* accum, double n_acc, int draw = 0) {
+void bk_chain(const BkArgs& a0, const BkLayout& L, hipStream_t s, double* accum, double n_acc, int draw = 0,
+              double* host_accum = nullptr) {
   BkArgs a = a0;
   const uint32_t resident = cf_resident_workgroups();
   a.drain_tile = resident != 0u && L.n_tiles > resident ? L.n_tiles - resident : 0xffffffffu;
@@ -1424,7 +1428,7 @@
   else
     hipLaunchKernelGGL(bk_cf_kernel<0>, g, b, 0, s, a, tabs);
   hipLaunchKernelGGL(bk_tail_kernel, dim3(kHeavyGrid), b, 0, s, static_cast<const BkArgs*>(a.args_dev), tabs, L.n_tiles,
-                     n_acc, accum, a.counters, static_cast<const double*>(a.records));
+                     n_acc, accum, a.counters, static_cast<const double*>(a.records), host_accum);
 }
 
 }
@@ -1450,7 +1454,7 @@
     hipLaunchKernelGGL(bk_draw_kernel, dim3(L.n_tiles), dim3(kTile), 0, s, a);
     draw = 0;
   }
-  bk_chain(a, L, s, ptr.accum, (double)c.n_paths, draw);
+  bk_chain(a, L, s, ptr.accum, (double)c.n_paths, draw, ptr.host_accum);
   return (int)hipGetLastError();
 }
 
diff --git a/hedgehog.jl_amd/csrc/hh_ctx.h b/hedgehog.jl_amd/csrc/hh_ctx.h
--- a/hedgehog.jl_amd/csrc/hh_ctx.h
+++ b/hedgehog.jl_amd/csrc/hh_ctx.h
@@ -75,6 +75,10 @@
   uint64_t seed_clock = 0, seed_hits = 0, seed_uploads = 0, seed_evictions = 0;
   double* accum = nullptr;
   double* accum_host = nullptr;
+  double* deliver_host = nullptr;
+  double* deliver_dev = nullptr;
+  unsigned long long deliver_turn = 0;
+  int solve_kernel_ms = 1;
   static constexpr int kTimingSlots = 256;
   bool timing = false;
   hipEvent_t tev[kTimingSlots][2] = {};
@@ -102,6 +106,32 @@
       return fail(ctx, HH_ERR_HIP, "%s failed: %s (%s:%d)", #expr, hipGetErrorString(e__),  \
                   __FILE__, __LINE__);                                                      \
   } while (0)
+
+[[maybe_unused]] inline hipError_t set_device(int device) {
+  int now = -1;
+  if (hipGetDevice(&now) == hipSuccess && now == device) return hipSuccess;
+  return hipSetDevice(device);
+}
+
+struct DeliverSlot {
+  double* host = nullptr;
+  double* dev = nullptr;
+};
+[[maybe_unused]] inline DeliverSlot take_deliver_slot(hh_ctx* ctx, uint32_t n_vec) {
+  const size_t at = hh::DeliverRing().slot(ctx->deliver_turn++);
+  DeliverSlot s{ctx->deliver_host + at, ctx->deliver_dev + at};
+  unsigned long long* w = reinterpret_cast<unsigned long long*>(s.host);
+  for (size_t i = 0; i < (size_t)n_vec * HH_ACC_LEN; ++i) w[i] = hh::kDeliverEmpty;
+  return s;
+}
+[[maybe_unused]] inline bool delivered(const double* host, uint32_t n_vec) {
+  for (uint32_t k = 0; k < n_vec; ++k) {
+    unsigned long long w;
+    std::memcpy(&w, host + (size_t)k * HH_ACC_LEN + HH_ACC_NPATHS, sizeof(w));
+    if (w == hh::kDeliverEmpty) return false;
+  }
+  return true;
+}
 
 template <class T>
 int ensure(hh_ctx* ctx, DevBuf<T>& buf, size_t need) {
@@ -164,3 +194,8 @@
 }
 
 }
+
+int hh_accumulate_delivered(hh_ctx* ctx, const hh_model* m, const hh_config* c, double* accum_dev, double* terminal,
+                            double* host_accum);
+int hh_accumulate_multi_delivered(hh_ctx* ctx, const hh_model* models, uint32_t n_models, const hh_config* c,
+                                  double* accum_dev, double* const* terminals, double* host_accum);
diff --git a/hedgehog.jl_amd/csrc/hh_kernels.h b/hedgehog.jl_amd/csrc/hh_kernels.h
--- a/hedgehog.jl_amd/csrc/hh_kernels.h
+++ b/hedgehog.jl_amd/csrc/hh_kernels.h
@@ -55,6 +55,7 @@
   unsigned long long finish_spin_ticks;
   uint32_t reducer_tile;
   PartialMap map;
+  double* host_accum;
 };
 
 struct DevicePtrs {
@@ -67,6 +68,7 @@
   unsigned int* finish_state;
   long long finish_spin_ticks = -1;
   int finish_tile_first = 0;
+  double* host_accum = nullptr;
   void* bk_scratch;
   struct BkTableKey* bk_table_key;
   int bk_term_cache;
@@ -137,7 +139,7 @@
 int launch_reduce_records(const double* records, uint32_t n_records, double n_paths, double* accum,
                           hipStream_t s, uint32_t n_groups = 1, const hh_model* m = nullptr,
                           const hh_config* c = nullptr, bool basket = false,
-                          const uint32_t* n_records_dev = nullptr);
+                          const uint32_t* n_records_dev = nullptr, double* host_accum = nullptr);
 int count_active_partials(const hh_model& m, const hh_config& c);
 int launch_basket_payoffs(const BasketArgs& b, uint32_t n_payoffs, uint32_t n_active_partials,
                           hipStream_t s);
diff --git a/hedgehog.jl_amd/csrc/hh_kernels.hip b/hedgehog.jl_amd/csrc/hh_kernels.hip
--- a/hedgehog.jl_amd/csrc/hh_kernels.hip
+++ b/hedgehog.jl_amd/csrc/hh_kernels.hip
@@ -294,7 +294,8 @@
                                                               uint32_t n, double n_paths,
                                                               double* __restrict__ accum,
                                                               const PartialMap map,
-                                                              const uint32_t* __restrict__ n_dev) {
+                                                              const uint32_t* __restrict__ n_dev,
+                                                              double* __restrict__ host_accum) {
   __shared__ double sm[257];
   const int slot = blockIdx.x;
   rec += (size_t)blockIdx.y * n * kRecStride;
@@ -315,7 +316,11 @@
   } else {
     out = sum_slot(rec, n, slot, sm);
   }
-  if (threadIdx.x == 0) accum[slot] = (slot == HH_ACC_NPATHS) ? n_paths : out;
+  if (threadIdx.x == 0) {
+    const double sum = (slot == HH_ACC_NPATHS) ? n_paths : out;
+    accum[slot] = sum;
+    if (host_accum) deliver_store(host_accum + (size_t)blockIdx.y * kRecStride + slot, sum);
+  }
 }
 
 
@@ -474,6 +479,7 @@
   a.finish_spin_ticks = p.finish_spin_ticks < 0 ? kFinishSpinTicksDefault : (unsigned long long)p.finish_spin_ticks;
   a.reducer_tile = p.finish_tile_first ? 0u : a.n_tiles - 1u;
   a.map = pm;
+  a.host_accum = p.host_accum;
   return a;
 }
 
@@ -542,7 +548,7 @@
 
 int launch_reduce_records(const double* records, uint32_t n_records, double n_paths, double* accum,
                           hipStream_t s, uint32_t n_groups, const hh_model* m, const hh_config* c,
-                          bool basket, const uint32_t* n_records_dev) {
+                          bool basket, const uint32_t* n_records_dev, double* host_accum) {
   PartialMap pm{};
   if (m && c && (basket || c->strategy != HH_BROADIE_KAYA)) {
     if (c->n_partials) pm = classify_partials(*m, *c);
@@ -551,7 +557,7 @@
       for (double& d : pm.dK) d = 0.0;
   }
   hipLaunchKernelGGL(reduce_records_kernel, dim3(kRecStride, n_groups), dim3(256), 0, s, records,
-                     n_records, n_paths, accum, pm, n_records_dev);
+                     n_records, n_paths, accum, pm, n_records_dev, host_accum);
   return (int)hipGetLastError();
 }
 
diff --git a/hedgehog.jl_amd/csrc/hh_layout.h b/hedgehog.jl_amd/csrc/hh_layout.h
--- a/hedgehog.jl_amd/csrc/hh_layout.h
+++ b/hedgehog.jl_amd/csrc/hh_layout.h
@@ -12,6 +12,15 @@
     at = ((at + a - 1) & ~(a - 1)) + n;
     return at - n;
   }
+};
+
+
+constexpr int kDeliverSlots = 4;
+constexpr unsigned long long kDeliverEmpty = 0x7FF8DE117FF8DE11ull;
+struct DeliverRing {
+  size_t slot_len, total;
+  constexpr DeliverRing() : slot_len((size_t)HH_MAX_MODELS * HH_ACC_LEN), total((size_t)kDeliverSlots * slot_len) {}
+  constexpr size_t slot(unsigned long long turn) const { return (size_t)(turn % kDeliverSlots) * slot_len; }
 };
 
 
diff --git a/hedgehog.jl_amd/csrc/hh_mgpu.hip b/hedgehog.jl_amd/csrc/hh_mgpu.hip
--- a/hedgehog.jl_amd/csrc/hh_mgpu.hip
+++ b/hedgehog.jl_amd/csrc/hh_mgpu.hip
@@ -98,6 +98,8 @@
   std::vector<double*> xchg;
   std::vector<size_t> xchg_cap;
   int enqueue = HH_MGPU_ENQUEUE_THREADS;
+  int kernel_ms = 1;
+  std::vector<const double*> slot;
   std::vector<std::unique_ptr<hh_worker>> workers;
   const std::function<int(int)>* job = nullptr;
   std::vector<int> rcs;
@@ -362,27 +364,39 @@
                                             "collective (HH_MGPU_RCCL does not fall back): create a new one"));
   int rc = ensure_acc(mg, n_acc);
   if (rc) return drain(mg, rc);
+  const bool deliver = mg->mode == HH_MGPU_REDUCE_HOST && (!basket || multi);
+  const uint32_t n_vec = (uint32_t)(n_acc / HH_ACC_LEN);
+  std::vector<char> timed(mg->n, 0);
+  for (int g = 0; g < mg->n; ++g) timed[g] = mg->kernel_ms != 0 || mg->ctx[g]->timing;
+  const bool fenced = mg->mode == HH_MGPU_REDUCE_RCCL;
   const auto t_enq = clk::now();
   rc = for_each_device(mg, [&](int g) -> int {
     const auto t0 = clk::now();
     hh_ctx* c = mg->ctx[g];
-    HH_DHIP(mg, g, hipSetDevice(mg->devices[g]));
-    HH_DHIP(mg, g, hipEventRecord(c->ev0, c->stream));
+    HH_DHIP(mg, g, set_device(mg->devices[g]));
+    DeliverSlot slot{};
+    if (deliver) {
+      std::lock_guard<std::recursive_mutex> lock__(c->mu);
+      slot = take_deliver_slot(c, n_vec);
+    }
+    mg->slot[g] = slot.host;
+    if (timed[g]) HH_DHIP(mg, g, hipEventRecord(c->ev0, c->stream));
     if (cfgs[g].n_paths == 0) {
-      HH_DHIP(mg, g, hipMemsetAsync(mg->acc[g], 0, n_acc * sizeof(double), c->stream));
+      if (deliver) std::memset(slot.host, 0, n_acc * sizeof(double));
+      else HH_DHIP(mg, g, hipMemsetAsync(mg->acc[g], 0, n_acc * sizeof(double), c->stream));
     } else {
       double* term = terminals ? terminals[g] : nullptr;
-      const int r = multi    ? hh_mc_accumulate_multi(c, m, basket->n_models, &cfgs[g], mg->acc[g], nullptr)
+      const int r = multi    ? hh_accumulate_multi_delivered(c, m, basket->n_models, &cfgs[g], mg->acc[g], nullptr, slot.dev)
                     : basket ? hh_mc_accumulate_basket(c, m, &cfgs[g], basket->strikes, basket->cps,
                                                        basket->n_payoffs, mg->acc[g], term)
-                             : hh_mc_accumulate(c, m, &cfgs[g], mg->acc[g], term);
+                             : hh_accumulate_delivered(c, m, &cfgs[g], mg->acc[g], term, slot.dev);
       if (r) {
         snprintf(mg->derr[g].data(), mg->derr[g].size(), "%s", hh_last_error(c));
         return r;
       }
     }
-    HH_DHIP(mg, g, hipEventRecord(c->ev1, c->stream));
-    mg->fence[g] = c->ev1;
+    if (timed[g] || fenced) HH_DHIP(mg, g, hipEventRecord(c->ev1, c->stream));
+    mg->fence[g] = fenced ? c->ev1 : nullptr;
     mg->enq_us[g] = us_since(t0);
     return HH_OK;
   });
@@ -392,7 +406,7 @@
   if (mg->mode == HH_MGPU_REDUCE_RCCL) {
     const int e = all_reduce_group(mg, mg->acc.data(), mg->red.data(), n_acc);
     if (e == kNcclSuccess) {
-      HH_MHIP_DRAIN(mg, hipSetDevice(mg->devices[0]));
+      HH_MHIP_DRAIN(mg, set_device(mg->devices[0]));
       HH_MHIP_DRAIN(mg, hipMemcpyAsync(mg->host, mg->red[0], n_acc * sizeof(double), hipMemcpyDeviceToHost,
                                        mg->ctx[0]->stream));
       reduced = true;
@@ -406,27 +420,33 @@
       }
     }
   }
-  if (!reduced) {
+  if (!reduced && !deliver) {
     for (int g = 0; g < mg->n; ++g) {
-      HH_MHIP_DRAIN(mg, hipSetDevice(mg->devices[g]));
+      HH_MHIP_DRAIN(mg, set_device(mg->devices[g]));
       HH_MHIP_DRAIN(mg, hipMemcpyAsync(mg->host + (size_t)g * n_acc, mg->acc[g], n_acc * sizeof(double),
                                        hipMemcpyDeviceToHost, mg->ctx[g]->stream));
     }
   }
-  for (int g = 0; g < mg->n; ++g) {
-    HH_MHIP_DRAIN(mg, hipSetDevice(mg->devices[g]));
+  double worst = 0.0;
+  for (int g = 0; g < mg->n; ++g) {
+    HH_MHIP_DRAIN(mg, set_device(mg->devices[g]));
     HH_MHIP_DRAIN(mg, hipStreamSynchronize(mg->ctx[g]->stream));
+    if (!timed[g]) continue;
+    float ms = 0.f;
+    HH_MHIP_DRAIN(mg, hipEventElapsedTime(&ms, mg->ctx[g]->ev0, mg->ctx[g]->ev1));
+    if (ms > worst) worst = ms;
   }
   if (!reduced) {
+    if (deliver) {
+      for (int g = 0; g < mg->n; ++g) {
+        if (cfgs[g].n_paths != 0 && !delivered(mg->slot[g], n_vec))
+          return mfail(mg, HH_ERR_HIP, "shard %d (device %d): the solve's kernels ran and left no sums in the context's host slot",
+                       g, mg->devices[g]);
+        std::memcpy(mg->host + (size_t)g * n_acc, mg->slot[g], n_acc * sizeof(double));
+      }
+    }
     for (int g = 1; g < mg->n; ++g)
       for (size_t i = 0; i < n_acc; ++i) mg->host[i] += mg->host[(size_t)g * n_acc + i];
-  }
-  double worst = 0.0;
-  for (int g = 0; g < mg->n; ++g) {
-    float ms = 0.f;
-    HH_MHIP(mg, hipSetDevice(mg->devices[g]));
-    HH_MHIP(mg, hipEventElapsedTime(&ms, mg->ctx[g]->ev0, mg->ctx[g]->ev1));
-    if (ms > worst) worst = ms;
   }
   *kernel_ms = worst;
   return HH_OK;
@@ -471,6 +491,7 @@
   mg->enq_us.assign(n_devices, 0.0);
   mg->pre.assign(n_devices, nullptr);
   mg->fence.assign(n_devices, nullptr);
+  mg->slot.assign(n_devices, nullptr);
   for (int g = 0; g < n_devices; ++g) {
     int rc = hh_ctx_create(&mg->ctx[g], device_ids[g]);
     if (!rc && hipEventCreateWithFlags(&mg->pre[g], hipEventDisableTiming) != hipSuccess) rc = HH_ERR_HIP;
@@ -630,6 +651,11 @@
         return mfail(mg, HH_ERR_INVALID, "HH_MGPU_OPT_ENQUEUE: 0 (one shard after the other) or 1 (a thread per device)");
       if (value == HH_MGPU_ENQUEUE_SERIAL) stop_workers(mg);
       mg->enqueue = (int)value;
+      return HH_OK;
+    case HH_MGPU_OPT_KERNEL_MS:
+      if (value != 0 && value != 1)
+        return mfail(mg, HH_ERR_INVALID, "HH_MGPU_OPT_KERNEL_MS: 1 (out->kernel_ms is measured) or 0 (no events, kernel_ms = 0)");
+      mg->kernel_ms = (int)value;
       return HH_OK;
     default:
       return mfail(mg, HH_ERR_INVALID, "unknown option %d", option);
diff --git a/hedgehog.jl_amd/csrc/hh_reduce.h b/hedgehog.jl_amd/csrc/hh_reduce.h
--- a/hedgehog.jl_amd/csrc/hh_reduce.h
+++ b/hedgehog.jl_amd/csrc/hh_reduce.h
@@ -4,6 +4,10 @@
 #include "hh_kernels.h"
 
 namespace hh {
+
+__device__ __forceinline__ void deliver_store(double* p, double v) {
+  __hip_atomic_store(p, v, __ATOMIC_RELAXED, __HIP_MEMORY_SCOPE_SYSTEM);
+}
 
 __device__ __forceinline__ double tree256(const double* __restrict__ p) {
   const int l = threadIdx.x & 63;
diff --git a/hedgehog.jl_amd/csrc/hh_sim.h b/hedgehog.jl_amd/csrc/hh_sim.h
--- a/hedgehog.jl_amd/csrc/hh_sim.h
+++ b/hedgehog.jl_amd/csrc/hh_sim.h
@@ -439,7 +439,9 @@
     }
     if (slot == HH_ACC_NPATHS) out = n_paths;
     const bool dirty = scalar_load_end(state_in_flight) != 0u;
-    accum[slot] = (gave_up || dirty) ? __longlong_as_double(0x7FF8000000000000ll) : out;
+    const double sum = (gave_up || dirty) ? __longlong_as_double(0x7FF8000000000000ll) : out;
+    accum[slot] = sum;
+    if (a.host_accum) deliver_store(a.host_accum + slot, sum);
     if (slot == 0 && gave_up) __hip_atomic_store(a.finish_state, 1u, __ATOMIC_RELAXED, __HIP_MEMORY_SCOPE_AGENT);
   }
 }
diff --git a/include/hedgehog_mc.h b/include/hedgehog_mc.h
--- a/include/hedgehog_mc.h
+++ b/include/hedgehog_mc.h
@@ -104,7 +104,7 @@
 const char* hh_last_error(const hh_ctx* ctx);
 enum hh_option { HH_OPT_LSM_FORM = 1, HH_OPT_BK_TERM_CACHE = 2, HH_OPT_GRID_FORM = 3, HH_OPT_LSM_SPIN_TICKS = 4,
                  HH_OPT_FUSE_REDUCE = 5, HH_OPT_GRID_ORDER = 6, HH_OPT_FINISH_SPIN_TICKS = 7,
-                 HH_OPT_FINISH_TILE_FIRST = 8 };
+                 HH_OPT_FINISH_TILE_FIRST = 8, HH_OPT_SOLVE_KERNEL_MS = 9 };
 enum hh_grid_form { HH_GRID_FORM_PER_DATE = 0, HH_GRID_FORM_BATCHED = 1 };
 enum hh_lsm_form { HH_LSM_FORM_PER_DATE = 0, HH_LSM_FORM_PERSISTENT = 1, HH_LSM_FORM_AUTO = 2 };
 int hh_ctx_set_option(hh_ctx* ctx, int32_t option, int64_t value);
@@ -135,7 +135,7 @@
 int hh_mgpu_reduce_mode(const hh_mgpu* mg);
 int hh_mgpu_selftest(hh_mgpu* mg, int32_t* ranks_out, int32_t* reduce_mode_out );
 int hh_mgpu_rccl_info(const hh_mgpu* mg, char* path_out, size_t cap, int32_t* version_out, int32_t* from_env_out);
-enum hh_mgpu_option { HH_MGPU_OPT_ENQUEUE = 1 };
+enum hh_mgpu_option { HH_MGPU_OPT_ENQUEUE = 1, HH_MGPU_OPT_KERNEL_MS = 2 };
 enum hh_mgpu_enqueue { HH_MGPU_ENQUEUE_SERIAL = 0, HH_MGPU_ENQUEUE_THREADS = 1  };
 int hh_mgpu_set_option(hh_mgpu* mg, int32_t option, int64_t value);
 int hh_mgpu_enqueue_stats(hh_mgpu* mg, double* shard_us, double* phase_us);
```

Result: no change. 430.7 billion (-0.0%).
